# fixstars/cuda-bundle-adjustment

Hardware: AMD Instinct MI355X
Metric: edges/sec (edge-iterations/s = E x LM iterations / wall, graph resident in HBM, every timed 10-iteration run from its own perturbed start) + 10-iter LM wall-clock (contract_wall: initialize()+optimize(10) after warm-up, C++ API) on KITTI-00-shaped graph; per-iter chi2 vs g2o-faithful oracle (higher is better)
Workload: dtype f64

## Files before the change

cuda-bundle-adjustment_amd/capi.py:

```python
from __future__ import annotations

import atexit
import ctypes as C
import os
import subprocess
import weakref

import numpy as np

_HERE = os.path.dirname(os.path.abspath(__file__))
CSRC = os.path.join(_HERE, "csrc")
LIB_PATH = os.path.join(CSRC, "libcuba_hip.so")
LIB_PATH_F32 = os.path.join(CSRC, "libcuba_hip_f32.so")
HEADER = os.path.join(os.path.dirname(_HERE), "include", "cuba_hip.h")

_dp = C.POINTER(C.c_double)
_ip = C.POINTER(C.c_int32)
_u8p = C.POINTER(C.c_uint8)

ARRAY_IDS = dict(bp=0, bsc=1, xp=2, xl=3, lm_sys=4, hsc=5, state=6)
PROFILE_KEYS = (
    "0: Initialize Optimizer", "1: Build Structure", "2: Compute Error", "3: Build System",
    "4: Schur Complement", "5: Symbolic Decomposition", "6: Numerical Decomposition", "7: Update Solution")


class CubaHipError(RuntimeError):
    pass


def build_library(force=False):
    srcs = [os.path.join(CSRC, f) for f in os.listdir(CSRC) if f.endswith((".hip", ".hpp"))] + [HEADER]
    stale = not os.path.exists(LIB_PATH) or any(os.path.getmtime(s) > os.path.getmtime(LIB_PATH) for s in srcs)
    if force or stale or not os.path.exists(LIB_PATH_F32):
        subprocess.check_call(["make", "-C", CSRC, "-s", "all"])
    return LIB_PATH


_libs = {}


def load_library(precision="f64"):
    path = {"f64": LIB_PATH, "f32": LIB_PATH_F32}[precision]
    path = os.environ.get("CUBA_HIP_LIB_" + precision.upper(), path)
    if path in _libs:
        return _libs[path]
    if not os.path.exists(path):
        raise CubaHipError(f"{path} is missing: run __graft_entry__.build() (hipcc --offload-arch=gfx950)")
    if os.environ.get("CUBA_HIP_NO_TORCH") != "1":
        try:
            import torch
        except Exception:
            pass
    lib = C.CDLL(path)
    H = C.c_void_p
    sig = {
        "cuba_hip_create": [C.c_int, C.POINTER(H)],
        "cuba_hip_destroy": [H],
        "cuba_hip_set_stream": [H, C.c_void_p],
        "cuba_hip_set_option": [H, C.c_char_p, C.c_double],
        "cuba_hip_set_graph": [H, C.c_int, C.c_int, C.c_int, C.c_int, _dp, _dp, _dp, _dp, C.c_int, _ip, _ip, _u8p, _dp, _dp],
        "cuba_hip_set_graph_begin": [H, C.c_int, C.c_int, C.c_int, C.c_int, _dp, _dp, _dp, _dp, C.c_int, _ip, _ip, _u8p, _dp, _dp],
        "cuba_hip_set_graph_end": [H],
        "cuba_hip_set_graph_partition": [H, C.c_int, C.c_int, C.c_int, C.c_int, _dp, _dp, _dp, _dp, C.c_int, _ip, _ip, _u8p, _dp, _dp, C.c_int, C.c_int],
        "cuba_hip_set_robust_kernel": [H, C.c_int, C.c_int, C.c_double],
        "cuba_hip_build_structure": [H],
        "cuba_hip_compute_errors": [H, _dp],
        "cuba_hip_build_system": [H],
        "cuba_hip_max_diagonal": [H, _dp],
        "cuba_hip_set_lambda": [H, C.c_double],
        "cuba_hip_restore_diagonal": [H],
        "cuba_hip_schur": [H],
        "cuba_hip_schur_parts": [H, C.POINTER(C.c_int)],
        "cuba_hip_schur_part": [H, C.c_int, C.POINTER(C.c_size_t)],
# ... 721 lines not shown
```

cuda-bundle-adjustment_amd/csrc/ba_kernels.hpp:

```cpp
#pragma once

#include <hip/hip_runtime.h>
#include <cstdint>
#include <vector>

#include "ba_math.hpp"

namespace cubahip
{

constexpr int PCG_SETUP_POSES = 64;
constexpr int NSLOT = 16;
constexpr int WAVE = 64;
constexpr int LIN_BLOCK = 256;
constexpr int STEREO_BIT = 0x40000000;

struct DeviceGraph
{
	int Pt = 0, Pf = 0, Lt = 0, Lf = 0, E = 0;
	int e_begin = 0, e_end = 0;
	Scalar *q = nullptr, *t = nullptr, *cam = nullptr, *Xw = nullptr;
	int *e_pose = nullptr, *e_lm = nullptr;
	Scalar *e_mu = nullptr, *e_mv = nullptr, *e_mr = nullptr, *e_w = nullptr;
	int* lm_ptr = nullptr;
	RobustKernel rk[2] = { { 0, 0 }, { 0, 0 } };
};

constexpr int BP_HEAVY = 64;

struct DeviceStructure
{
	int nWaves = 0;
	int* wave_lm = nullptr;
	int nBig = 0;
	int* big_lm = nullptr;
	int nblk = 0;
	int *hsc_rowptr = nullptr, *hsc_colind = nullptr;
	int *adj_ptr = nullptr, *adj_blk = nullptr, *adj_col = nullptr;
	int2* ell = nullptr;
	int ell_m = 0, ell_over = 0;
	int* hsc_blkrow = nullptr;
	int nOd = 0;
	int nDiagProd = 0;
	int* od_blocks = nullptr;
	int inv_rows8 = 1;
	int nHeavy = 0;
	int *prod_ea = nullptr, *prod_eb = nullptr;
	const int *prod_beg = nullptr, *prod_end = nullptr, *pe_beg = nullptr, *pe_end = nullptr;
	int* prod_lm = nullptr;
	int* pe_edge = nullptr;
	int nCb = 0;
	int *cb_I = nullptr, *cb_J = nullptr, *cb_ptr = nullptr, *cb_blk = nullptr;
	Scalar *cb_wi = nullptr, *cb_wj = nullptr;
	Scalar* e_rec = nullptr;
	int mixed = 0;
};

int spmv_rows_for(int Pf);

struct DeviceSystem
{
	Scalar* hsc = nullptr;
	Scalar* bsc = nullptr;
	Scalar* bp = nullptr;
	Scalar* lm_sys = nullptr;
	Scalar* lm_inv = nullptr;
	Scalar* xp = nullptr;
	Scalar* xl = nullptr;
	Scalar* parts = nullptr;
	Scalar* slots = nullptr;
	unsigned long long* maxdiag = nullptr;
	int* fail = nullptr;
	Scalar *minv = nullptr, *r = nullptr, *z = nullptr, *p0 = nullptr, *p1 = nullptr, *ap = nullptr;
	Scalar *rz = nullptr, *pq = nullptr;
	int rzStride = 0, pqStride = 0;
	int nrz0 = 0, nrz = 0, npq = 0;
	int* done = nullptr;
	int* iters = nullptr;
	int* host_flags = nullptr;
	int* ticket = nullptr;
	int* kbase = nullptr;
	int agg = 0;
	int nc = 0;
	Scalar inv_agg = 0;
	int cl = 1;
	Scalar* acinv = nullptr;
	float* acinv32 = nullptr;
	Scalar* gj_pivots = nullptr;
	Scalar* rc = nullptr;
	Scalar* hrow = nullptr;
	int spmv_rows = 2;
	Scalar* qpart = nullptr;
	Scalar* r2 = nullptr;
// ... 28 lines not shown
	int nActive = 0;
	int nBlocks = 0;
	int nPoses = 0;
	const int *pose_i = nullptr, *pose_j = nullptr;
	const int* blk_ptr = nullptr;
	const int* blk_id = nullptr;
	const int* blk_shared = nullptr;
	const int* pose_ptr = nullptr;
	const int* pose_id = nullptr;
	const int* pose_item = nullptr;
	const Scalar* info = nullptr;
	Scalar* rec = nullptr;
	Scalar* chi = nullptr;
	const int* rk_kind = nullptr;
	const Scalar* rk_delta = nullptr;
};
constexpr int REL_REC = 90;
struct DeviceRelPoses : DevicePosePairs { const Scalar *q = nullptr, *t = nullptr; };
constexpr int PRNG_REC = 14;
struct DevicePoseRanges : DevicePosePairs
{
	const Scalar *arm_i = nullptr, *arm_j = nullptr;
	const Scalar* range = nullptr;
};

struct DeviceLandmarkPriors
{
	int n = 0;
	const int* lm_ptr = nullptr;
	const int* lm = nullptr;
	const Scalar* xbar = nullptr;
	const Scalar* info = nullptr;
	const int* rk_kind = nullptr;
	const Scalar* rk_delta = nullptr;
	Scalar* chi = nullptr;
};

enum { FACTOR_PRIORS = 0, FACTOR_REL, FACTOR_LMP, FACTOR_POS, FACTOR_DIR, FACTOR_RNG, FACTOR_PRNG, FACTOR_KINDS };
struct DeviceFactors
{
	DevicePriors priors; DeviceRelPoses rel; DeviceLandmarkPriors lmp; DevicePositionFactors pos; DeviceDirectionFactors dir; DeviceRangeFactors rng;
	DevicePoseRanges prng;
	template <class F> void each(F&& f) const { f(priors); f(rel); f(lmp); f(pos); f(dir); f(rng); f(prng); }
};
void launch_pose_factor_linearize(const DeviceGraph& g, const DeviceStructure& st, const DeviceSystem& sys, const DeviceFactors& pf, int mode, hipStream_t s);
void launch_factor_chi2(const DeviceGraph& g, const DeviceFactors& pf, Scalar* parts, hipStream_t s, int only = -1);
int factor_chi2_parts(const DeviceFactors* pf);

void launch_residual_chi2(const DeviceGraph& g, Scalar* parts, Scalar* slots, Scalar* per_edge, hipStream_t st, const DeviceFactors* pf = nullptr);

struct BlockPassRange { int begin, end, heavy; };
void launch_linearize_dm(const DeviceGraph& g, const DeviceStructure& st, const DeviceSystem& sys, int mode, Scalar lambda, hipStream_t s,
	Scalar* backupSrc = nullptr, Scalar* backupDst = nullptr, size_t backupCount = 0, const BlockPassRange* range = nullptr, const double* restoreFlag = nullptr,
	const DeviceLandmarkPriors* lp = nullptr);
void launch_block_pass(const DeviceGraph& g, const DeviceStructure& st, const DeviceSystem& sys, const BlockPassRange& range, hipStream_t s);

void launch_pose_maxdiag(const DeviceGraph& g, const DeviceStructure& st, const DeviceSystem& sys, hipStream_t s);

void launch_back_substitute(const DeviceGraph& g, const DeviceStructure& st, const DeviceSystem& sys, Scalar lambda, hipStream_t s);

void launch_pose_scale(const DeviceGraph& g, const DeviceSystem& sys, Scalar lambda, Scalar* slots, hipStream_t s);
struct LmDevice;
void launch_trial_tail_fused(const DeviceGraph& g, const DeviceStructure& st, const DeviceSystem& sys, Scalar lambda, const Scalar* old, hipStream_t s,
	const LmDevice* decide = nullptr, const DeviceFactors* pf = nullptr, int publish = 1);
size_t trial_tail_parts(const DeviceGraph& g, const DeviceStructure& st, int factorParts = 0);
constexpr int LM_REC = 8, LM_RING = 64;
struct LmDevice { double* state = nullptr; Scalar* lam = nullptr; double* ring = nullptr; };
void launch_lm_run_init(const Scalar* chiSlots, const unsigned long long* maxdiag, const LmDevice& lm, double tau, double tagBase, int maxq, hipStream_t s);
void launch_lm_decide_failed(const DeviceSystem& sys, const LmDevice& lm, hipStream_t s);
void launch_reduce_report(const DeviceSystem& sys, const Scalar* pA, int nA, Scalar* oA, const Scalar* pB, int nB, Scalar* oB, const Scalar* pC, int nC, Scalar* oC,
	const LmDevice* decide, int publish, hipStream_t s);
void launch_restore_if_rejected(Scalar* state, const Scalar* backup, size_t count, const LmDevice& lm, hipStream_t s);
void launch_landmark_scale(const DeviceGraph& g, const DeviceSystem& sys, Scalar lambda, Scalar* slots, hipStream_t s);

void launch_update_state(const DeviceGraph& g, const DeviceSystem& sys, hipStream_t s);

void launch_pcg_setup(const DeviceGraph& g, const DeviceStructure& st, const DeviceSystem& sys, Scalar lambda, hipStream_t s);
void launch_pcg_spmv(const DeviceGraph& g, const DeviceStructure& st, const DeviceSystem& sys, int k, int maxIter, Scalar tol2, hipStream_t s);
void launch_pcg_update(const DeviceGraph& g, const DeviceStructure& st, const DeviceSystem& sys, int k, int maxIter, Scalar tol2, hipStream_t s);
Scalar* launch_coarse_setup(const DeviceGraph& g, const DeviceStructure& st, const DeviceSystem& sys, Scalar* work0, Scalar* work1, hipStream_t s, hipEvent_t assembled = nullptr);
Scalar* launch_dense_inverse(Scalar* work0, Scalar* work1, int n, Scalar* pivots, hipStream_t s);
void launch_coarse_finish(const Scalar* swept, Scalar* dst, int n, hipStream_t s);
struct GjJob { Scalar* buf[2]; Scalar* piv[2]; int n, tiles; };
void launch_coarse_assemble(const DeviceGraph& g, const DeviceStructure& st, const DeviceSystem& sys, Scalar* work0, hipStream_t s);
void launch_dense_inverse_batch(const GjJob* jobs, int m, int nMax, hipStream_t s);
void launch_pcg2_fused(const DeviceGraph& g, const DeviceSystem& sys, int k, int kOut, int maxIter, Scalar tol2, int doUpdate, hipStream_t s);
int spmv_upper_grid(int Pf);
int pcg_rows_max_aggregate();
int pcg_rows_entries_per_thread(const DeviceSystem& sys);
void launch_build_lowpos(const DeviceGraph& g, const DeviceStructure& st, int* lowpos, hipStream_t s);
void launch_pcg_upper_iteration(const DeviceGraph& g, const DeviceStructure& st, const DeviceSystem& sys, int k, int maxIter, Scalar tol2, hipStream_t s, int which = 7);
void launch_pcg_advance(const DeviceSystem& sys, int n, hipStream_t s, Scalar tol2 = Scalar(-1));
void launch_coarse_to_fp32(const Scalar* swept, float* dst, int n, hipStream_t s);
void launch_pcg_iteration(const DeviceGraph& g, const DeviceStructure& st, const DeviceSystem& sys, int k, int maxIter, Scalar tol2, hipStream_t s);

struct LmDevice;
struct BatchTrial
{
	unsigned lmGroups = 0, lmGrid = 0; const Scalar* backupSrc = nullptr; Scalar* backupDst = nullptr; size_t backupCount = 0;
	int poseGroups = 0; unsigned schurGrid = 0;
	int nSetup = 0; size_t expandTotal = 0; unsigned nExpand = 0; const Scalar* copySrc = nullptr; Scalar* copyDst = nullptr; size_t copyPairs = 0; unsigned setupGrid = 0;
	int fusedOn = 0;
	const Scalar* old = nullptr; Scalar *scParts = nullptr, *chiParts = nullptr, *scaleParts = nullptr; int nLm = 0, poseBlocks = 0, nScale = 0; unsigned tailGrid = 0; int nA = 0;
	double* lmState = nullptr; Scalar* lmLam = nullptr; double* lmRing = nullptr; int reportOn = 0;
	Scalar* state = nullptr; size_t stateCount = 0; unsigned restoreGrid = 0;
};
struct BatchEntry
{
	DeviceGraph g; DeviceStructure st; DeviceSystem sys;
	int maxIter = 0;
	int gridSpmv = 0;
	BatchTrial t;
};
void batch_fill_linearize(const DeviceGraph& g, const DeviceStructure& st, const Scalar* backupSrc, Scalar* backupDst, size_t backupCount, BatchTrial& t);
void launch_batch_linearize(const BatchEntry* tab, int n, unsigned lmGridMax, unsigned schurGridMax, bool mixed, hipStream_t s);
void batch_fill_setup(const DeviceGraph& g, const DeviceStructure& st, const DeviceSystem& sys, const Scalar* copySrc, Scalar* copyDst, size_t copyCount, BatchTrial& t);
void launch_batch_setup(const BatchEntry* tab, int n, unsigned gridMax, hipStream_t s);
void launch_batch_first_precond(const BatchEntry* tab, int n, const DeviceSystem& sys0, int ncMax, size_t ldsMax, Scalar tol2, hipStream_t s);
void batch_fill_tail(const DeviceGraph& g, const DeviceStructure& st, const DeviceSystem& sys, const Scalar* old, const LmDevice& lm, Scalar* state, size_t stateCount, BatchTrial& t);
void launch_batch_tail(const BatchEntry* tab, int n, unsigned tailGridMax, unsigned restoreGridMax, hipStream_t s);
int batch_kernel_class(const DeviceGraph& g, const DeviceSystem& sys);
size_t batch_pcg2_lds_bytes(const DeviceSystem& sys);
void launch_pcg_batch_iteration(const BatchEntry* tab, int n, const DeviceGraph& g0, const DeviceSystem& sys0, int gridSpmvMax, int ncMax, size_t ldsMax, int k, Scalar tol2, hipStream_t s);
void launch_pcg_batch_advance(const BatchEntry* tab, int n, int iters, hipStream_t s, Scalar tol2);

hipError_t graph_add_pcg_chunk(hipGraph_t graph, const DeviceGraph& g, const DeviceStructure& st, const DeviceSystem& sys, int chunk, int maxIter, Scalar tol2, int report);

void launch_hsc_expand(const DeviceGraph& g, const DeviceStructure& st, const DeviceSystem& sys, hipStream_t s);
void launch_pcg_setup_expand(const DeviceGraph& g, const DeviceStructure& st, const DeviceSystem& sys, Scalar lambda, hipStream_t s,
	const Scalar* copySrc = nullptr, Scalar* copyDst = nullptr, size_t copyCount = 0);

constexpr int SC_T = 32;
constexpr int SC_TP = 5;
constexpr int SC_TT = SC_T * SC_T;

struct SparseCholPlan
{
	int Pf = 0, T = 0, nTiles = 0, nLevels = 0, slack = 0;
	std::vector<int> posOfSeg, segOfPos;
	std::vector<int> colPtr;
	std::vector<int> rowIdx, colOfTile;
	std::vector<int> gPtr;
	std::vector<int> gather;
	std::vector<int> wgRec;
	std::vector<int> lvlPtr, lvlTiles;
	std::vector<int> lvlColPtr, lvlCols;
	std::vector<int> blkTile;
	long long entries = 0;
	size_t tileBytes() const { return sizeof(Scalar) * (size_t)SC_TT * ((size_t)2 * nTiles + 1); }
	double secondsEstimate() const;
};
bool sparse_chol_plan(int Pf, const int* rowptr, const int* colind, int slack, size_t maxTiles, SparseCholPlan& out);

struct SparseChol
{
	Scalar* tiles = nullptr;
	Scalar* tilesT = nullptr;
	Scalar* y = nullptr;
	Scalar* rinv = nullptr;
	const int *colPtr = nullptr, *rowIdx = nullptr, *colOfTile = nullptr, *gPtr = nullptr, *gather = nullptr;
	const int *wgRec = nullptr, *lvlCols = nullptr, *blkTile = nullptr, *posOfSeg = nullptr;
	int* fail = nullptr;
	int T = 0, Pf = 0, nTiles = 0;
};
void launch_sparse_chol_fill(const DeviceStructure& st, const DeviceSystem& sys, const SparseChol& d, hipStream_t s);
void launch_sparse_chol_solve(const SparseChol& d, const SparseCholPlan& plan, Scalar* x, hipStream_t s);
void launch_sparse_chol_factor(const SparseChol& d, const SparseCholPlan& plan, hipStream_t s);

struct SelInvPlan
{
	int nLevels = 0;
	std::vector<int> stepPtr;
	std::vector<int> offRec;
	std::vector<int> colStepPtr, cols;
	std::vector<int> gather;
	long long products = 0;
	size_t sigmaBytes() const;
	int nTiles = 0;
};
bool selinv_plan(const SparseCholPlan& p, SelInvPlan& out);

struct SelInv
// ... 70 lines not shown
```

cuda-bundle-adjustment_amd/csrc/ba_linearize.hip:

```cpp

#include "ba_device.hpp"

namespace cubahip
{

constexpr int REC = 8;

__device__ __forceinline__ double tag_encode(int tag, double) { return __longlong_as_double((long long)tag); }
__device__ __forceinline__ float tag_encode(int tag, float) { return __int_as_float(tag); }
__device__ __forceinline__ int tag_decode(double v) { return (int)__double_as_longlong(v); }
__device__ __forceinline__ int tag_decode(float v) { return __float_as_int(v); }
__device__ __forceinline__ bool sign_flag(double v) { return __double_as_longlong(v) < 0; }
__device__ __forceinline__ bool sign_flag(float v) { return __float_as_int(v) < 0; }
__device__ __forceinline__ double abs_value(double v) { return __builtin_fabs(v); }
__device__ __forceinline__ float abs_value(float v) { return __builtin_fabsf(v); }

template <typename ET>
__device__ __forceinline__ void write_record(Scalar* base, size_t e, const Scalar Xc[3], Scalar wr, const Scalar r[3], int il, bool stereo)
{
	ET* rec = reinterpret_cast<ET*>(base) + REC * e;
	const ET w = (ET)wr;
	rec[0] = (ET)Xc[0]; rec[1] = (ET)Xc[1]; rec[2] = (ET)Xc[2]; rec[3] = stereo ? -w : w;
	rec[4] = (ET)r[0]; rec[5] = (ET)r[1]; rec[6] = (ET)r[2];
	rec[7] = tag_encode(il, ET());
// ... 342 lines not shown
template <int MODE, typename ET>
__global__ __launch_bounds__(256) void pose_pass_kernel(DeviceGraph g, DeviceStructure st, DeviceSystem sys)
{
	pose_pass_body<MODE, ET>(g, st, sys, blockIdx.x);
}

template <typename ET>
struct ProductOperand { ET X[3]; ET M[3][3]; };

template <typename ET>
__device__ __forceinline__ void product_operand(const ET* rec, const Rot3T<ET>& R, const ET cam[5], ProductOperand<ET>& o)
{
	CameraFrameEdge<ET> c;
	camera_frame_edge<ET>(rec, cam, c);
	o.X[0] = c.X[0]; o.X[1] = c.X[1]; o.X[2] = c.X[2];
	camera_frame_m<ET>(c, R, o.M);
}

template <typename ET>
__device__ __forceinline__ void product_accumulate(const ProductOperand<ET>& A, const ProductOperand<ET>& B, const ET inv[6], ET (&T)[6][6])
{
	ET P[3][3], W[3][6];
#pragma unroll
	for (int i = 0; i < 3; i++)
#pragma unroll
		for (int k = 0; k < 3; k++)
			P[i][k] = A.M[i][0] * inv[sym3_idx(0, k)] + A.M[i][1] * inv[sym3_idx(1, k)] + A.M[i][2] * inv[sym3_idx(2, k)];
#pragma unroll
	for (int i = 0; i < 3; i++)
	{
#pragma unroll
		for (int j = 0; j < 3; j++) W[i][3 + j] = P[i][0] * B.M[j][0] + P[i][1] * B.M[j][1] + P[i][2] * B.M[j][2];
		W[i][0] = B.X[1] * W[i][5] - B.X[2] * W[i][4];
		W[i][1] = B.X[2] * W[i][3] - B.X[0] * W[i][5];
		W[i][2] = B.X[0] * W[i][4] - B.X[1] * W[i][3];
	}
#pragma unroll
	for (int c = 0; c < 6; c++)
	{
		T[0][c] += A.X[1] * W[2][c] - A.X[2] * W[1][c];
		T[1][c] += A.X[2] * W[0][c] - A.X[0] * W[2][c];
		T[2][c] += A.X[0] * W[1][c] - A.X[1] * W[0][c];
		T[3][c] += W[0][c]; T[4][c] += W[1][c]; T[5][c] += W[2][c];
	}
}

template <typename ET, int GROUP>
__device__ __forceinline__ void block_pass_group(const DeviceGraph& g, const DeviceStructure& st, const DeviceSystem& sys, int grp, int gl)
{
	const int blk0 = grp >= 0 ? st.od_blocks[grp] : -1;
	const bool on = blk0 >= 0;
	const int blk = on ? blk0 : 0;
	const int a = on ? st.hsc_blkrow[blk] : 0, b = on ? st.hsc_colind[blk] : 0;
	ET qa[4], cama[5], qb[4], camb[5];
	load_pose_as<ET>(g, a, qa, cama);
	load_pose_as<ET>(g, b, qb, camb);
	const Rot3T<ET> Ra = quat_to_rot(qa[0], qa[1], qa[2], qa[3]);
	const Rot3T<ET> Rb = quat_to_rot(qb[0], qb[1], qb[2], qb[3]);
	ET T[6][6];
#pragma unroll
	for (int r = 0; r < 6; r++)
#pragma unroll
		for (int c = 0; c < 6; c++) T[r][c] = 0;
	const ET* recs = reinterpret_cast<const ET*>(st.e_rec);
	const int p1 = on ? st.prod_end[blk] : 0;
	for (int p = (on ? st.prod_beg[blk] : 0) + gl; p < p1; p += GROUP)
	{
		const ET* ra = recs + REC * (size_t)st.prod_ea[p];
		const ET* rb = recs + REC * (size_t)st.prod_eb[p];
		const Scalar* li = st.inv_rows8 ? sys.lm_inv + 8 * (size_t)st.prod_lm[p] : sys.lm_sys + 9 * (size_t)st.prod_lm[p];
		ET inv[6];
#pragma unroll
		for (int k = 0; k < 6; k++) inv[k] = (ET)li[k];
		ProductOperand<ET> A, B;
		product_operand<ET>(ra, Ra, cama, A);
		product_operand<ET>(rb, Rb, camb, B);
		product_accumulate<ET>(A, B, inv, T);
	}
	Scalar Ts[6][6];
#pragma unroll
	for (int r = 0; r < 6; r++)
#pragma unroll
		for (int c = 0; c < 6; c++)
		{
			Scalar v = (Scalar)T[r][c];
			if (GROUP == 64) v = wave_sum(v);
			else { v += __shfl_xor(v, 1); v += __shfl_xor(v, 2); v += __shfl_xor(v, 4); v += __shfl_xor(v, 8); }
			Ts[r][c] = v;
		}
	if (!on) return;
	Scalar* dst = sys.hsc + 36 * (size_t)blk;
	if (a != b)
	{
#pragma unroll
		for (int c = 0; c < 6; c++)
#pragma unroll
			for (int r = 0; r < 6; r++)
				if (GROUP == 64 ? (c * 6 + r) == gl : (c * 6 + r) % GROUP == gl) dst[c * 6 + r] = -Ts[r][c];
	}
	else if (gl == 0)
	{
#pragma unroll
		for (int c = 0; c < 6; c++)
#pragma unroll
			for (int r = 0; r <= c; r++) dst[c * 6 + r] -= Ts[r][c] + Ts[c][r];
	}
}

__host__ __device__ __forceinline__ int block_pass_heavy_groups(int nHeavy) { return (nHeavy + 3) / 4; }
__host__ __device__ __forceinline__ int block_pass_groups(int nOd, int nHeavy) { return block_pass_heavy_groups(nHeavy) + ((nOd - nHeavy) * BP_GROUP + 255) / 256; }

template <typename ET>
__device__ __forceinline__ void block_pass_body(const DeviceGraph& g, const DeviceStructure& st, const DeviceSystem& sys, int bid)
{
	const int nh = block_pass_heavy_groups(st.nHeavy);
	if (bid < nh)
	{
		const int grp = bid * 4 + (threadIdx.x >> 6);
		block_pass_group<ET, 64>(g, st, sys, grp < st.nHeavy ? grp : -1, threadIdx.x & 63);
	}
	else
	{
		const int grp = st.nHeavy + ((bid - nh) * 256 + threadIdx.x) / BP_GROUP;
		block_pass_group<ET, BP_GROUP>(g, st, sys, grp < st.nOd ? grp : -1, threadIdx.x & (BP_GROUP - 1));
	}
}

template <typename ET>
__global__ __launch_bounds__(256) void block_pass_kernel(DeviceGraph g, DeviceStructure st, DeviceSystem sys)
{
	block_pass_body<ET>(g, st, sys, blockIdx.x);
}

template <typename ET>
__global__ __launch_bounds__(256) void schur_pass_kernel(DeviceGraph g, DeviceStructure st, DeviceSystem sys, int nPoseGroups)
{
	if ((int)blockIdx.x < nPoseGroups) pose_pass_body<1, ET>(g, st, sys, blockIdx.x);
	else block_pass_body<ET>(g, st, sys, blockIdx.x - nPoseGroups);
}

template <typename ET>
__global__ __launch_bounds__(256) void schur_pass_batch_kernel(const BatchEntry* __restrict__ tab)
{
	const BatchEntry& e = tab[blockIdx.y];
	if (blockIdx.x >= e.t.schurGrid) return;
	if ((int)blockIdx.x < e.t.poseGroups) pose_pass_body<1, ET>(e.g, e.st, e.sys, blockIdx.x);
	else block_pass_body<ET>(e.g, e.st, e.sys, blockIdx.x - e.t.poseGroups);
}

static DeviceStructure block_pass_view(const DeviceStructure& st, const BlockPassRange& r)
{
	DeviceStructure v = st;
	v.od_blocks = st.od_blocks + r.begin; v.nOd = r.end - r.begin; v.nHeavy = r.heavy;
	return v;
}

struct LandmarkGrid
{
	unsigned groups, nCopy;
	LandmarkGrid(const DeviceStructure& st, const Scalar* backupSrc, size_t backupCount)
		: groups((st.nWaves + (LIN_BLOCK / WAVE) - 1) / (LIN_BLOCK / WAVE)),
		nCopy(backupSrc ? (unsigned)std::min<size_t>(512, (backupCount + LIN_BLOCK - 1) / LIN_BLOCK) : 0) {}
	unsigned grid() const { return groups + nCopy; }
};

template <typename ET>
static void launch_linearize_dm_t(const DeviceGraph& g, const DeviceStructure& stAll, const DeviceSystem& sys, int mode, Scalar lambda, hipStream_t s,
	Scalar* backupSrc, Scalar* backupDst, size_t backupCount, const BlockPassRange* range, const double* restoreFlag, const DeviceLandmarkPriors* lp)
{
	const DeviceStructure st = range ? block_pass_view(stAll, *range) : stAll;
	if (st.nWaves > 0)
	{
		const LandmarkGrid L(st, backupSrc, backupCount);
		const double* flag = L.nCopy ? restoreFlag : nullptr;
		if (lp)
			hipLaunchKernelGGL((mode == 0 ? lm_pass_prior_kernel<0, ET> : lm_pass_prior_kernel<1, ET>), dim3(L.grid()), dim3(LIN_BLOCK), 0, s,
				g, st, sys, lambda, L.groups, backupSrc, backupDst, backupCount, flag, *lp);
		else
			hipLaunchKernelGGL((mode == 0 ? lm_pass_kernel<0, ET> : lm_pass_kernel<1, ET>), dim3(L.grid()), dim3(LIN_BLOCK), 0, s,
				g, st, sys, lambda, L.groups, backupSrc, backupDst, backupCount, flag);
	}
	else if (backupSrc && backupCount)
		(void)hipMemcpyAsync(backupDst, backupSrc, backupCount * sizeof(Scalar), hipMemcpyDeviceToDevice, s);
	if (st.nBig > 0)
	{
		const auto big = lp ? (mode == 0 ? big_lm_pass_kernel<0, ET, true> : big_lm_pass_kernel<1, ET, true>)
			: (mode == 0 ? big_lm_pass_kernel<0, ET, false> : big_lm_pass_kernel<1, ET, false>);
		hipLaunchKernelGGL(big, dim3(st.nBig), dim3(256), 0, s, g, st, sys, lambda, lp ? *lp : DeviceLandmarkPriors());
	}
	const int nbp = block_pass_groups(st.nOd, st.nHeavy);
	if (mode == 1 && g.Pf > 0 && st.nOd > 0 && st.nDiagProd == 0)
	{
		const int np = (g.Pf + 3) / 4;
		hipLaunchKernelGGL((schur_pass_kernel<ET>), dim3(np + nbp), dim3(256), 0, s, g, st, sys, np);
		return;
	}
	if (g.Pf > 0)
	{
		if (mode == 0) hipLaunchKernelGGL((pose_pass_kernel<0, ET>), dim3((g.Pf + 3) / 4), dim3(256), 0, s, g, st, sys);
		else hipLaunchKernelGGL((pose_pass_kernel<1, ET>), dim3((g.Pf + 3) / 4), dim3(256), 0, s, g, st, sys);
	}
	if (mode == 1 && st.nOd > 0)
		hipLaunchKernelGGL((block_pass_kernel<ET>), dim3(nbp), dim3(256), 0, s, g, st, sys);
}

void launch_linearize_dm(const DeviceGraph& g, const DeviceStructure& st, const DeviceSystem& sys, int mode, Scalar lambda, hipStream_t s,
	Scalar* backupSrc, Scalar* backupDst, size_t backupCount, const BlockPassRange* range, const double* restoreFlag, const DeviceLandmarkPriors* lp)
{
	if (lp && lp->n == 0) lp = nullptr;
	if (st.mixed && sizeof(Scalar) == 8) launch_linearize_dm_t<float>(g, st, sys, mode, lambda, s, backupSrc, backupDst, backupCount, range, restoreFlag, lp);
	else launch_linearize_dm_t<Scalar>(g, st, sys, mode, lambda, s, backupSrc, backupDst, backupCount, range, restoreFlag, lp);
}

void batch_fill_linearize(const DeviceGraph& g, const DeviceStructure& st, const Scalar* backupSrc, Scalar* backupDst, size_t backupCount, BatchTrial& t)
{
	const LandmarkGrid L(st, backupSrc, backupCount);
	t.lmGroups = L.groups;
	t.lmGrid = L.grid();
	t.backupSrc = backupSrc; t.backupDst = backupDst; t.backupCount = backupCount;
	t.poseGroups = (g.Pf + 3) / 4;
	t.schurGrid = (unsigned)(t.poseGroups + block_pass_groups(st.nOd, st.nHeavy));
}

void launch_batch_linearize(const BatchEntry* tab, int n, unsigned lmGridMax, unsigned schurGridMax, bool mixed, hipStream_t s)
{
	if (mixed && sizeof(Scalar) == 8)
	{
		hipLaunchKernelGGL((lm_pass_batch_kernel<float>), dim3(lmGridMax, n), dim3(LIN_BLOCK), 0, s, tab);
		hipLaunchKernelGGL((schur_pass_batch_kernel<float>), dim3(schurGridMax, n), dim3(256), 0, s, tab);
	}
	else
	{
		hipLaunchKernelGGL((lm_pass_batch_kernel<Scalar>), dim3(lmGridMax, n), dim3(LIN_BLOCK), 0, s, tab);
		hipLaunchKernelGGL((schur_pass_batch_kernel<Scalar>), dim3(schurGridMax, n), dim3(256), 0, s, tab);
	}
}

void launch_block_pass(const DeviceGraph& g, const DeviceStructure& stAll, const DeviceSystem& sys, const BlockPassRange& range, hipStream_t s)
{
	if (range.end <= range.begin) return;
	const DeviceStructure st = block_pass_view(stAll, range);
	const int nbp = block_pass_groups(st.nOd, st.nHeavy);
	if (st.mixed && sizeof(Scalar) == 8) hipLaunchKernelGGL((block_pass_kernel<float>), dim3(nbp), dim3(256), 0, s, g, st, sys);
	else hipLaunchKernelGGL((block_pass_kernel<Scalar>), dim3(nbp), dim3(256), 0, s, g, st, sys);
}

__global__ __launch_bounds__(256) void pose_maxdiag_kernel(DeviceGraph g, DeviceStructure st, DeviceSystem sys)
{
	const int i = blockIdx.x * 256 + threadIdx.x;
	Scalar m = 0;
	if (i < g.Pf * 6)
	{
		const int p = i / 6, k = i % 6;
		m = sys.hsc[36 * (size_t)st.hsc_rowptr[p] + k * 7];
	}
	m = wave_max(m);
	if ((threadIdx.x & 63) == 0) atomic_max_nonneg(sys.maxdiag, m);
}

void launch_pose_maxdiag(const DeviceGraph& g, const DeviceStructure& st, const DeviceSystem& sys, hipStream_t s)
{
	if (g.Pf <= 0) return;
	hipLaunchKernelGGL(pose_maxdiag_kernel, dim3((g.Pf * 6 + 255) / 256), dim3(256), 0, s, g, st, sys);
}
// ... 3 lines not shown
```

cuda-bundle-adjustment_amd/csrc/ba_lm.hip:

```cpp
#include "ba_solver.hpp"

using namespace cubahip;

void cuba_hip_solver::graphWorker()
{
	(void)hipSetDevice(device);
	std::unique_lock<std::mutex> lk(gb.m);
	for (;;)
	{
		gb.cv.wait(lk, [&] { return gb.stop || !gb.jobs.empty() || !gb.trash.empty(); });
		if (gb.stop) return;
		if (gb.jobs.empty())
		{
			std::vector<hipGraphExec_t> t; t.swap(gb.trash);
			gb.busy = true;
			lk.unlock();
			for (hipGraphExec_t e : t) (void)hipGraphExecDestroy(e);
			lk.lock();
			gb.busy = false;
			gb.cv.notify_all();
			continue;
		}
		GraphJob j = gb.jobs.front(); gb.jobs.pop_front();
		gb.busy = true;
// ... 68 lines not shown
{
	volatile int* flags = (volatile int*)((char*)h_pinned + 1024);
	{
		const auto t0 = Clock::now();
		for (long spins = 0; flags[3] != expectedTicket; spins++)
			if ((spins & 0xfff) == 0xfff && std::chrono::duration<double>(Clock::now() - t0).count() > 2.0) break;
		if (flags[3] == expectedTicket)
		{
			std::atomic_thread_fence(std::memory_order_acquire);
			return;
		}
	}
	sync();
	std::atomic_thread_fence(std::memory_order_acquire);
	expectedTicket = flags[3];
}

void cuba_hip_solver::downloadAsDouble(const Scalar* dsrc, double* hdst, size_t n)
{
	if (!n) return;
	if (sizeof(Scalar) == sizeof(double))
	{
		HIP_TRY(hipMemcpyAsync(hdst, dsrc, n * sizeof(double), hipMemcpyDeviceToHost, stream));
		sync();
		return;
	}
	std::vector<Scalar> tmp(n);
	HIP_TRY(hipMemcpyAsync(tmp.data(), dsrc, n * sizeof(Scalar), hipMemcpyDeviceToHost, stream));
	sync();
	for (size_t i = 0; i < n; i++) hdst[i] = (double)tmp[i];
}

void cuba_hip_solver::uploadFromDouble(Scalar* ddst, const double* hsrc, size_t n)
{
	if (!n) return;
	std::vector<Scalar> tmp(hsrc, hsrc + n);
	HIP_TRY(hipMemcpyAsync(ddst, tmp.data(), n * sizeof(Scalar), hipMemcpyHostToDevice, stream));
	sync();
}

double cuba_hip_solver::computeErrors()
{
	need();
	StageTimer tm(this, 2);
	launch_residual_chi2(g, d_parts.data(), slotsDev, nullptr, stream, factors());
	return readSlots(0);
}

void cuba_hip_solver::linearize(int mode, double lam, bool withBackup)
{
	waitAssembled();
	const bool parts = mode == 1 && !redParts.empty();
	launch_linearize_dm(g, st, sys, mode, lam, stream, withBackup ? d_state.data() : nullptr, d_backup.data(), d_state.size(), parts ? &redParts[0].od : nullptr,
		withBackup ? lmRestoreFlag : nullptr, landmarkPriors());
	if (parts && !partsByCaller)
		for (size_t c = 1; c < redParts.size(); c++) launch_block_pass(g, st, sys, redParts[c].od, stream);
	if (factors()) launch_pose_factor_linearize(g, st, sys, pf, mode, stream);
}

void cuba_hip_solver::schurPart(int part, size_t ranges[4])
{
	need();
	if (part < 0 || part >= schurParts()) throw ArgError{ "cuba_hip_schur_part: no such part" };
	if (part == 0)
	{
		StageTimer tm(this, 4);
		zeroReduced();
		partsByCaller = true;
		try { linearize(1, lambda, false); } catch (...) { partsByCaller = false; throw; }
		partsByCaller = false;
	}
	else
	{
		StageTimer tm(this, 4);
		launch_block_pass(g, st, sys, redParts[part].od, stream);
	}
	const size_t nblk = (size_t)st.nblk;
	ranges[0] = redParts.empty() ? 0 : 36 * redParts[part].blkBegin;
	ranges[1] = redParts.empty() ? 36 * nblk : 36 * (redParts[part].blkEnd - redParts[part].blkBegin);
	ranges[2] = part == 0 ? 36 * nblk : 0;
	ranges[3] = part == 0 ? d_red.size() - 36 * nblk : 0;
}

void cuba_hip_solver::assemble()
{
	need();
	StageTimer tm(this, 3);
	zeroReduced(true);
	d_maxdiag.zero(stream);
	linearize(0, 0.0);
}

void cuba_hip_solver::maxDiagonalParts(double* posePart, double* lmPart)
{
	need();
	const double* hD = (const double*)hostStage();
	HIP_TRY(hipMemcpyAsync(hostStage(), d_maxdiag.data(), 8 * 64, hipMemcpyDeviceToHost, stream));
	sync();
	double v = 0;
	for (int i = 0; i < 64; i++) v = std::max(v, hD[i]);
	*lmPart = v;
	d_maxdiag.zero(stream);
	launch_pose_maxdiag(g, st, sys, stream);
	HIP_TRY(hipMemcpyAsync(hostStage(), d_maxdiag.data(), 8 * 64, hipMemcpyDeviceToHost, stream));
	sync();
	v = 0;
	for (int i = 0; i < 64; i++) v = std::max(v, hD[i]);
	*posePart = v;
}

void cuba_hip_solver::scaleParts(double lam, double* posePart, double* lmPart)
{
	need();
	launch_pose_scale(g, sys, lam, slotsDev + 3 * NSLOT, stream);
	launch_landmark_scale(g, sys, lam, slotsDev + 2 * NSLOT, stream);
	sync();
	double a = 0, b = 0;
	for (int i = 0; i < NSLOT; i++) { b += slot(2 * NSLOT + i); a += slot(3 * NSLOT + i); }
	*posePart = a; *lmPart = b;
}

double cuba_hip_solver::maxDiagonal()
{
	need();
	StageTimer tm(this, 3);
	zeroReduced(true);
	d_maxdiag.zero(stream);
	linearize(0, 0.0);
	launch_pose_maxdiag(g, st, sys, stream);
	HIP_TRY(hipMemcpyAsync(hostStage(), d_maxdiag.data(), 8 * 64, hipMemcpyDeviceToHost, stream));
	sync();
	double v = 0;
	for (int i = 0; i < 64; i++) v = std::max(v, ((const double*)hostStage())[i]);
	return v;
}

void cuba_hip_solver::schur(bool withBackup)
{
	need();
	StageTimer tm(this, 4);
	zeroReduced();
	linearize(1, lambda, withBackup);
}

bool cuba_hip_solver::solveReduced() { return retryWithFp64Inverse(solveReducedOnce()); }

bool cuba_hip_solver::retryWithFp64Inverse(bool ok)
{
	if (ok || !lastSolveBrokeDown || lastFailCode != 2 || !fp32Inverse() || sys.agg <= 0) return ok;
	precondFp32 = false; sys.acinv32 = nullptr;
	dropPcgGraph();
	coarseValid = false; firstInvValid = false; firstInvPending = false;
	cntFp32Fallbacks++;
	if (std::getenv("CUBA_HIP_DEBUG")) std::fprintf(stderr, "[cuba_hip] PCG broke down with the fp32-stored coarse inverse: repeating the solve with fp64 storage\n");
	const int64_t directBefore = cntDirect;
	const bool ok2 = solveReducedOnce();
	if (!ok2 || cntDirect != directBefore)
	{
		precondFp32 = true; sys.acinv32 = d_coarse32[0].data();
		dropPcgGraph();
		coarseValid = false; firstInvValid = false; firstInvPending = false;
	}
	return ok2;
}

int cuba_hip_solver::pcgBudget(int maxIter) const
{
	const int it = directAfter > 0 ? directAfter : std::min(384, std::max(128, Pf / 4));
	return std::min(maxIter, std::max(4, it / 4 * 4));
}

bool cuba_hip_solver::ensureDirectPlan()
{
	if (directPlanValid) return !directRefused;
	const auto t0 = Clock::now();
	ensureHostPattern();
	if (!sparse_chol_plan(Pf, h_rowptr.data(), h_colind.data(), directSlack, (size_t)std::max(1, directMaxTiles), directPlan))
	{
		directPlanValid = true; directRefused = true;
		char buf[200];
		std::snprintf(buf, sizeof buf, "exact reduced solve unavailable: the factor of the %d-pose reduced matrix needs more than direct_max_tiles = %d tiles", Pf, directMaxTiles);
		lastError = buf;
		return false;
	}
	const SparseCholPlan& p = directPlan;
	{
		size_t freeB = 0, totalB = 0;
		const size_t have = sizeof(Scalar) * (d_scTiles.size() + d_scTilesT.size());
		if (hipMemGetInfo(&freeB, &totalB) == hipSuccess && p.tileBytes() > have && p.tileBytes() - have > freeB)
		{
			directPlanValid = true; directRefused = true;
			char buf[200];
			std::snprintf(buf, sizeof buf, "exact reduced solve unavailable: the factor of the %d-pose reduced matrix needs %.1f MB, %.1f MB of device memory are free",
				Pf, p.tileBytes() / 1e6, freeB / 1e6);
// ... 3 lines not shown
		(void)hipGetLastError();
	}
	std::vector<int> ints;
	auto put = [&](const std::vector<int>& v) { const size_t o = ints.size(); ints.insert(ints.end(), v.begin(), v.end()); while (ints.size() % 4) ints.push_back(0); return o; };
	const size_t oColPtr = put(p.colPtr), oRowIdx = put(p.rowIdx), oColOf = put(p.colOfTile), oGPtr = put(p.gPtr), oGather = put(p.gather),
		oWgRec = put(p.wgRec), oLvlCols = put(p.lvlCols), oBlkTile = put(p.blkTile), oPos = put(p.posOfSeg);
	d_scInts.upload(ints, stream);
	d_scTiles.resize((size_t)SC_TT * ((size_t)p.nTiles + 1)); d_scTilesT.resize((size_t)SC_TT * std::max(1, p.nTiles));
	d_scY.resize((size_t)SC_T * p.T); d_scRinv.resize((size_t)SC_T * p.T); d_scFail.resize(1);
	sync();
	SparseChol& d = directDev;
	d.tiles = d_scTiles.data(); d.tilesT = d_scTilesT.data(); d.y = d_scY.data(); d.rinv = d_scRinv.data(); d.fail = d_scFail.data();
	const int* base = d_scInts.data();
	d.colPtr = base + oColPtr; d.rowIdx = base + oRowIdx; d.colOfTile = base + oColOf; d.gPtr = base + oGPtr; d.gather = base + oGather;
	d.wgRec = base + oWgRec; d.lvlCols = base + oLvlCols; d.blkTile = base + oBlkTile; d.posOfSeg = base + oPos;
	d.T = p.T; d.Pf = Pf; d.nTiles = p.nTiles;
	directPlanValid = true;
	directPlanBuilds++;
	directPlanSeconds = std::chrono::duration<double>(Clock::now() - t0).count();
	if (std::getenv("CUBA_HIP_DEBUG"))
		std::fprintf(stderr, "[cuba_hip] exact reduced solve, symbolic phase: %d poses -> %d tile columns, %d tiles (%.1f MB), %d levels, %lld tile products, slack %d, %.2f ms\n",
			Pf, p.T, p.nTiles, p.tileBytes() / 1e6, p.nLevels, p.entries, p.slack, 1e3 * directPlanSeconds);
	return true;
}

bool cuba_hip_solver::solveDirect()
{
	if (!ensureDirectPlan()) return false;
	const auto t0 = Clock::now();
	launch_sparse_chol_fill(st, sys, directDev, stream);
	launch_sparse_chol_solve(directDev, directPlan, sys.xp, stream);
	int* hflag = (int*)hostStage();
	HIP_TRY(hipMemcpyAsync(hflag, directDev.fail, sizeof(int), hipMemcpyDeviceToHost, stream));
	sync();
	directSeconds = std::chrono::duration<double>(Clock::now() - t0).count();
	cntDirect++;
	directSticky = true;
	coarseValid = false;
	if (std::getenv("CUBA_HIP_DEBUG"))
		std::fprintf(stderr, "[cuba_hip] exact reduced solve: %d unknowns, %.3f ms, lambda %.3e%s\n", 6 * Pf, 1e3 * directSeconds, lambda, *hflag ? " -- NON-POSITIVE PIVOT" : "");
	if (*hflag)
	{
		cntDirectFailed++;
		lastError = "exact reduced solve: non-positive pivot (the damped reduced matrix is not positive definite)";
		return false;
	}
	return true;
}

bool cuba_hip_solver::solveBegin(SolveCtx& sc)
{
	lastSolveBrokeDown = false;
	need();
	if (Pf == 0) { sc.result = true; return true; }
	const int maxIter = sc.maxIter = maxIterAlloc;
	const Scalar tol2 = sc.tol2 = pcgTol * pcgTol;
	if (failDirty) { d_fail.zero(stream); failDirty = false; }
	const bool twoLevel = sc.twoLevel = sys.agg > 0;
	const bool direct = sc.direct = directUsable();
	if (direct && (directSticky || directAlways))
	{
		launch_pcg_setup(g, st, sys, lambda, stream);
		failDirty = true;
		coarseValid = false;
		notePcgHistory(0);
		sc.result = solveDirect();
		return true;
	}
	sc.budget = direct && !acceptUnconverged ? pcgBudget(maxIter) : maxIter;
	const size_t invCount = (size_t)36 * sys.cl * sys.cl * sys.nc * sys.nc;
	bool takeInverse = false;
	if (twoLevel && coarseValid && pendingInv >= 0)
	{
		HIP_TRY(hipStreamWaitEvent(stream, evInverse, 0));
		takeInverse = true; pendingInv = -1;
	}
	const bool deferred = sc.deferLaunch && twoLevel && coarseValid;
	{
		const bool f32 = fp32Inverse();
		const Scalar* cpSrc = !takeInverse ? nullptr : f32 ? reinterpret_cast<const Scalar*>(d_coarse32[1].data()) : d_coarse[0].data();
		Scalar* cpDst = f32 ? reinterpret_cast<Scalar*>(d_coarse32[0].data()) : d_coarse[2].data();
		const size_t cpCount = f32 ? inv32Count() / 2 : invCount;
		if (deferred) { sc.deferred = true; sc.copySrc = cpSrc; sc.copyDst = cpDst; sc.copyCount = cpCount; }
		else launch_pcg_setup_expand(g, st, sys, lambda, stream, cpSrc, cpDst, cpCount);
	}
	if (twoLevel)
	{
		const int gjSteps = (6 * sys.cl * sys.nc + 31) / 32, first = gjSteps & 1;
		{
			ensureOverlapObjects();
			const size_t invBytes = sizeof(Scalar) * (size_t)36 * sys.cl * sys.cl * sys.nc * sys.nc;
			if (!coarseValid && heuristics && firstInvValid)
			{
				HIP_TRY(hipStreamWaitEvent(stream, evFirstInv, 0));
				if (fp32Inverse()) HIP_TRY(hipMemcpyAsync(d_coarse32[0].data(), d_firstInv32.data(), inv32Count() * sizeof(float), hipMemcpyDeviceToDevice, stream));
				else HIP_TRY(hipMemcpyAsync(d_coarse[2].data(), d_firstInv.data(), invBytes, hipMemcpyDeviceToDevice, stream));
				pendingInv = -1;
				coarseValid = true; sideAge = overlapPeriod(); firstInvPending = true;
			}
			else if (!coarseValid)
			{
				drainInversion();
				(void)launch_coarse_setup(g, st, sys, d_coarse[first].data(), d_coarse[1 - first].data(), stream);
				if (fp32Inverse()) launch_coarse_to_fp32(d_coarse[0].data(), d_coarse32[0].data(), 6 * sys.cl * sys.nc, stream);
				else launch_coarse_finish(d_coarse[0].data(), d_coarse[2].data(), 6 * sys.cl * sys.nc, stream);
				coarseValid = true; cntCoarseRefresh++; cntCoarseInline++; sideAge = 0;
				if (heuristics)
				{
					if (fp32Inverse()) d_firstInv32.resize(inv32Count()); else d_firstInv.resize(invCount);
					sideAge = overlapPeriod(); firstInvPending = true;
				}
			}
			sys.acinv = d_coarse[2].data();
			const bool regular = ++sideAge >= overlapPeriod();
			if (regular) sideAge = 0;
			if (regular)
			{
				if (!deferred) HIP_TRY(hipEventRecord(evSetup, stream));
				if (sc.deferCoarse)
				{
					sc.deferCoarse->push_back(CoarseJob{ this, first, firstInvPending, !deferred });
					if (firstInvPending) { firstInvPending = false; firstInvValid = true; }
				}
				else if (sc.sideLater) sc.sideFirst = first;
				else enqueueCoarseSide(first);
				pendingInv = 0;
				assemblePending = true; cntCoarseRefresh++;
			}
		}
		if (!deferred) launch_pcg2_fused(g, sys, 0, 0, maxIter, tol2, 0, stream);
	}
	const bool graphs = sc.graphs = useGraph && !sc.batched && g_liveHandles.load(std::memory_order_relaxed) <= 1;
	if (useGraph && !graphs && (!pcgGraphs.empty() || graphsOrderedFor)) dropPcgGraph();
	if (graphs && pcgGraphs.empty() && graphsOrderedFor != (const void*)sys.acinv)
	{
		for (int c = 64; c >= 4; c /= 2) (void)pcgGraphIfReady(c, maxIter, tol2);
		graphsOrderedFor = (const void*)sys.acinv;
	}
	sc.hInts = (volatile int*)((char*)h_pinned + 1024);
	sc.tSolve0 = Clock::now();
	int predicted = 32;
	if (runIters.size() >= 2)
	{
		const double a = runIters[runIters.size() - 2], b = runIters.back();
		const double lin = b + std::max(0.0, b - a), geo = b * std::min(1.35, std::max(1.0, b / std::max(1.0, a)));
		predicted = (int)std::max(lin, geo) + 1;
	}
	else if (runIters.size() == 1) predicted = (int)(1.35 * runIters[0]) + 2;
	else if (firstSolveIters > 0) predicted = firstSolveIters + 1;
	{
		const size_t k = runIters.size();
		if (heuristics && k < prevRunIters.size() && std::equal(runIters.begin(), runIters.end(), prevRunIters.begin())) predicted = prevRunIters[k];
	}
	sc.predicted = predicted;
	return false;
}

void cuba_hip_solver::enqueueCoarseSide(int first)
{
	HIP_TRY(hipStreamWaitEvent(gjStream, evSetup, 0));
	(void)launch_coarse_setup(g, st, sys, d_coarse[first].data(), d_coarse[1 - first].data(), gjStream, evAssembled);
	enqueueInversionTail(gjStream, firstInvPending);
	if (firstInvPending) { firstInvPending = false; firstInvValid = true; }
}

void cuba_hip_solver::enqueueInversionTail(hipStream_t side, bool firstInvCopy)
{
	const int Nc = 6 * sys.cl * sys.nc;
	if (fp32Inverse()) launch_coarse_to_fp32(d_coarse[0].data(), d_coarse32[1].data(), Nc, side);
	else launch_coarse_finish(d_coarse[0].data(), d_coarse[0].data(), Nc, side);
	if (firstInvCopy)
	{
		if (fp32Inverse()) HIP_TRY(hipMemcpyAsync(d_firstInv32.data(), d_coarse32[1].data(), inv32Count() * sizeof(float), hipMemcpyDeviceToDevice, side));
		else HIP_TRY(hipMemcpyAsync(d_firstInv.data(), d_coarse[0].data(), sizeof(Scalar) * (size_t)Nc * Nc, hipMemcpyDeviceToDevice, side));
		HIP_TRY(hipEventRecord(evFirstInv, side));
	}
	HIP_TRY(hipEventRecord(evInverse, side));
}

bool cuba_hip_solver::solveBrokeDown(SolveCtx& sc)
{
	lastSolveBrokeDown = true; lastFailCode = sc.hInts[0];
	cntPcgIters += sc.hInts[1]; coarseValid = false; firstInvValid = false; firstInvPending = false; failDirty = true;
	if (sc.direct && lastFailCode != 1 && !(lastFailCode == 2 && fp32Inverse() && sc.twoLevel))
	{
		notePcgHistory(-sc.hInts[1]);
		d_fail.zero(stream); failDirty = false;
		return solveDirect();
	}
	return false;
}

static int pcgFirstTarget(int predicted) { return (predicted + 3) / 4 * 4; }
static int pcgNextTarget(int k0, int looks) { return k0 + ((looks == 0 && k0 <= 96) ? 4 : std::max(8, k0 / 8 / 4 * 4)); }
static int pcgBatchLength(int target, int budget, int k0) { return std::max(4, std::min(target, budget) - k0); }

bool cuba_hip_solver::solveReducedOnce()
{
	StageTimer tm(this, 6);
	SolveCtx sc;
	sc.sideLater = coarseSideLater;
	if (solveBegin(sc)) return sc.result;
	const int maxIter = sc.maxIter; const Scalar tol2 = sc.tol2; const bool graphs = sc.graphs; const int predicted = sc.predicted;
	bool converged = false;
	int k0 = 0, looks = 0, eagerIters = 0;
	int target = pcgFirstTarget(predicted);
	while (k0 < sc.budget && !converged)
	{
		int todo = pcgBatchLength(target, sc.budget, k0);
		while (todo > 0)
		{
			int c = graphs ? 256 : todo;
			for (; graphs && c > 4 && c > todo; c >>= 1) {}
			if (graphs && todo > c && todo % 4 == 0 && todo <= 128 && pcgGraphMaxIter == maxIter && pcgGraphTol2 == tol2)
			{
				if ((pcgGraphs.count(std::make_pair(todo, (const Scalar*)sys.acinv)) || ++batchRequests[todo] >= 2) && pcgGraphIfReady(todo, maxIter, tol2)) c = todo;
			}
			hipGraphExec_t exec = graphs ? pcgGraphIfReady(c, maxIter, tol2) : nullptr;
			if (exec) { HIP_TRY(hipGraphLaunch(exec, stream)); noteReport(); }
			else
			{
				for (int k = 0; k < c; k++) enqueuePcgIteration(k, maxIter, tol2, stream);
				launch_pcg_advance(sys, c, stream, tol2); noteReport();
				if (graphs) { eagerIters += c; cntPcgPlain += c; }
			}
			k0 += c; todo -= c;
			if (sc.sideFirst >= 0) { enqueueCoarseSide(sc.sideFirst); sc.sideFirst = -1; }
		}
		waitReport();
		if (sc.hInts[0] != 0) return solveBrokeDown(sc);
		if (sc.hInts[2] == 1 || sc.hInts[1] < std::min(k0, maxIter)) converged = true;
		target = pcgNextTarget(k0, looks);
		looks++; cntPcgLooks++; cntHostLooks++;
	}
	sc.converged = converged; sc.k0 = k0; sc.looks = looks; sc.eagerIters = eagerIters;
	return solveEnd(sc);
}

bool cuba_hip_solver::solveEnd(SolveCtx& sc)
{
	const int maxIter = sc.maxIter; const bool direct = sc.direct; const bool converged = sc.converged;
	const int k0 = sc.k0, looks = sc.looks, eagerIters = sc.eagerIters, predicted = sc.predicted;
	const auto tSolve1 = Clock::now();
	if (std::getenv("CUBA_HIP_DEBUG"))
	{
		std::vector<Scalar> part((size_t)std::max(1, sys.nrz0));
		HIP_TRY(hipMemcpyAsync(part.data(), sys.rz, sizeof(Scalar) * part.size(), hipMemcpyDeviceToHost, stream));
		sync();
		double rz0 = 0; for (Scalar v : part) rz0 += (double)v;
		std::fprintf(stderr, "[cuba_hip] PCG: %d iterations, %d enqueued (%d as plain launches), %d host looks (prediction %d), lambda %.3e, r0.z0 %.6e, solve %.3f ms, graphs built so far %lld\n",
			sc.hInts[1], k0, eagerIters, looks, predicted, lambda, rz0, 1e3 * std::chrono::duration<double>(tSolve1 - sc.tSolve0).count(), (long long)gb.builds.load());
	}
	const int itersDone = sc.itersDone >= 0 ? sc.itersDone : sc.hInts[1];
	cntPcgIters += itersDone; cntPcgEnqueued += k0;
	if (runIters.empty()) firstSolveIters = itersDone;
// ... 95 lines not shown
		if (!r.absorb(rec)) throw StateError{ "the device's decision record of an LM trial never arrived" };
	}
}

bool cuba_hip_solver::lmBeforeTrial(LmRun& r)
{
	if (r.stop) return false;
	if (r.enq > r.seen)
	{
		const bool safe = r.done + 1 < r.niter && r.rejRun + 1 < LmRun::maxq;
		if (!safe) { waitReport(); cntHostLooks++; lmAbsorb(r, r.enq); if (r.stop) return false; }
	}
	cntTrials++;
	lambda = -1.0;
	return true;
}

bool cuba_hip_solver::lmAfterSolveHost(LmRun& r)
{
	lmAbsorb(r, r.enq);
	if (r.stop) { cntTrials--; return false; }
	return true;
}

bool cuba_hip_solver::lmAfterSolve(LmRun& r, bool ok)
{
	if (!lmAfterSolveHost(r)) return false;
	const bool waited = !r.chain || !(r.done + 1 < r.niter && r.rejRun + 1 < LmRun::maxq);
	const bool publish = waited || !ok;
	if (ok) launch_trial_tail_fused(g, st, sys, (Scalar)-1, d_backup.data(), stream, &r.lm, factors(), publish ? 1 : 0);
	else launch_lm_decide_failed(sys, r.lm, stream);
	if (publish) noteReport();
	r.restoreInPass = !publish && st.nWaves > 0;
	if (!r.restoreInPass) launch_restore_if_rejected(d_state.data(), d_backup.data(), d_state.size(), r.lm, stream);
	r.enq++;
	(void)hipStreamQuery(stream);
	return true;
}

int cuba_hip_solver::lmRunEnd(LmRun& r)
{
	if (r.seen < r.enq) { waitReport(); cntHostLooks++; lmAbsorb(r, r.enq); }
	lambda = r.lam;
	return r.done;
}

int cuba_hip_solver::optimizeDeviceDecision(int niter, double* chi2Out)
{
	LmRun r;
	lmRunBegin(r, niter, chi2Out, true);
	while (lmBeforeTrial(r))
	{
		lmRestoreFlag = r.restoreInPass ? r.lm.state + 5 : nullptr;
		try { schur(true); } catch (...) { lmRestoreFlag = nullptr; throw; }
		lmRestoreFlag = nullptr;
		coarseSideLater = true;
		bool ok = false;
		try { ok = solveReduced(); } catch (...) { coarseSideLater = false; throw; }
		coarseSideLater = false;
		if (!lmAfterSolve(r, ok)) break;
	}
	return lmRunEnd(r);
}

bool cuba_hip_solver::fullyBatchable() const
{
	return batchable() && st.nBig == 0 && st.nDiagProd == 0 && st.nOd > 0 && st.nWaves > 0 && redParts.empty() && !factors();
}

bool cuba_hip_solver::batchable() const
{
	return !profile && partHi < 0 && Pf > 0 && Lf > 0 && E > 0 && trial_tail_parts(g, st, factorParts()) <= d_parts.size() && batch_kernel_class(g, sys) >= 0;
}

void cuba_hip_solver::launchCoarseJobs(std::vector<CoarseJob>& jobs, hipEvent_t common)
{
	if (jobs.empty()) return;
	ensureOverlapObjects();
	hipStream_t side = gjStream;
	const int m = (int)jobs.size();
	if (!h_gjTab) { HIP_TRY(hipHostMalloc((void**)&h_gjTab, sizeof(GjJob) * CUBA_HIP_BATCH_MAX, hipHostMallocDefault)); HIP_TRY(hipEventCreateWithFlags(&evGjTab, hipEventDisableTiming)); HIP_TRY(hipEventRecord(evGjTab, side)); }
	d_gjTab.resize(sizeof(GjJob) * CUBA_HIP_BATCH_MAX);
	HIP_TRY(hipEventSynchronize(evGjTab));
	int nMax = 0;
	for (int a = 0; a < m; a++)
	{
		cuba_hip_solver* h = jobs[a].h;
		const int Nc = 6 * h->sys.cl * h->sys.nc;
		HIP_TRY(hipStreamWaitEvent(side, jobs[a].ownEvent || !common ? h->evSetup : common, 0));
		launch_coarse_assemble(h->g, h->st, h->sys, h->d_coarse[jobs[a].first].data(), side);
		GjJob& j = h_gjTab[a];
		j.buf[0] = h->d_coarse[jobs[a].first].data(); j.buf[1] = h->d_coarse[1 - jobs[a].first].data();
		j.piv[0] = h->sys.gj_pivots; j.piv[1] = h->sys.gj_pivots + 32 * 32;
		j.n = Nc; j.tiles = (Nc + 31) / 32;
		nMax = std::max(nMax, Nc);
	}
	for (int a = 0; a < m; a++) HIP_TRY(hipEventRecord(jobs[a].h->evAssembled, side));
	HIP_TRY(hipMemcpyAsync(d_gjTab.data(), h_gjTab, sizeof(GjJob) * m, hipMemcpyHostToDevice, side));
	HIP_TRY(hipEventRecord(evGjTab, side));
	launch_dense_inverse_batch(reinterpret_cast<const GjJob*>(d_gjTab.data()), m, nMax, side);
	for (int a = 0; a < m; a++) jobs[a].h->enqueueInversionTail(side, jobs[a].firstInvCopy);
	jobs.clear();
}

void cuba_hip_solver::ensureBatchTables()
{
	if (!h_batchTab) HIP_TRY(hipHostMalloc((void**)&h_batchTab, sizeof(BatchEntry) * CUBA_HIP_BATCH_MAX * 3, hipHostMallocDefault));
	d_batchTab.resize(sizeof(BatchEntry) * CUBA_HIP_BATCH_MAX * 3);
// ... 71 lines not shown
};
}

static int optimizeBatch(cuba_hip_solver** hs, int n, int niter, double* chi2, int* nDone, bool full)
{
	typedef cuba_hip_solver::SolveCtx SolveCtx;
	cuba_hip_solver* lead = hs[0];
	hipStream_t bs = lead->stream;
	struct StreamGuard
	{
		cuba_hip_solver** hs; int n; std::vector<hipStream_t> own;
		StreamGuard(cuba_hip_solver** h, int m, hipStream_t s) : hs(h), n(m), own((size_t)m)
		{
			for (int i = 0; i < n; i++) { own[i] = hs[i]->stream; (void)hipStreamSynchronize(own[i]); hs[i]->stream = s; }
		}
		~StreamGuard() { if (n > 0) (void)hipStreamSynchronize(hs[0]->stream); for (int i = 0; i < n; i++) hs[i]->stream = own[i]; }
	} streamGuard(hs, full ? n : 0, bs);
	std::vector<hipEvent_t>& evJoin = lead->batchEvents;
	while (!full && (int)evJoin.size() < n + 1) { hipEvent_t e; HIP_TRY(hipEventCreateWithFlags(&e, hipEventDisableTiming)); evJoin.push_back(e); }
	const hipEvent_t evFork = full ? nullptr : evJoin[n];
	lead->ensureBatchTables();
	lead->ensureOverlapObjects();
	BatchEntry* hTab[3]; const BatchEntry* dTab[3];
	for (int k = 0; k < 3; k++) { hTab[k] = lead->h_batchTab + (size_t)k * CUBA_HIP_BATCH_MAX; dTab[k] = reinterpret_cast<const BatchEntry*>(lead->d_batchTab.data()) + (size_t)k * CUBA_HIP_BATCH_MAX; }
	auto upload = [&](int k, int m) { HIP_TRY(hipMemcpyAsync(const_cast<BatchEntry*>(dTab[k]), hTab[k], sizeof(BatchEntry) * m, hipMemcpyHostToDevice, bs)); };
	const int pcgTab = full ? 1 : 0;
	std::vector<cuba_hip_solver::LmRun> runs((size_t)n);
	std::vector<SolveCtx> ctx((size_t)n);
	std::vector<cuba_hip_solver::CoarseJob> coarseJobs;
	for (int i = 0; i < n; i++) hs[i]->lmRunBegin(runs[i], niter, chi2 ? chi2 + (size_t)i * niter : nullptr);
	const bool mixed = lead->st.mixed != 0;
	const int cls0 = batch_kernel_class(lead->g, lead->sys);
	std::vector<int> act;
	std::vector<char> okv((size_t)n);
	int batchSolves = 0;
	for (;;)
	{
		act.clear();
		for (int i = 0; i < n; i++) if (hs[i]->lmBeforeTrial(runs[i])) act.push_back(i);
		if (act.empty()) break;
		const int m = (int)act.size();
		(full ? lead->cntBatchFullTrials : lead->cntBatchIterTrials)++;
		if (full)
		{
			unsigned lmMax = 0, schurMax = 0;
			for (int a = 0; a < m; a++)
			{
				cuba_hip_solver* h = hs[act[a]];
				h->zeroReduced();
				BatchEntry& e = hTab[0][a];
				e = BatchEntry();
				e.g = h->g; e.st = h->st; e.sys = h->sys;
				batch_fill_linearize(h->g, h->st, h->d_state.data(), h->d_backup.data(), h->d_state.size(), e.t);
				lmMax = std::max(lmMax, e.t.lmGrid); schurMax = std::max(schurMax, e.t.schurGrid);
			}
			upload(0, m);
			launch_batch_linearize(dTab[0], m, lmMax, schurMax, mixed, bs);
		}
		BatchPcg pcg(hs, ctx, bs);
		unsigned setupMax = 0; int nFused = 0;
		for (int a = 0; a < m; a++)
		{
			const int i = act[a];
			cuba_hip_solver* h = hs[i];
			if (!full) h->schur(true);
			ctx[i] = SolveCtx(); ctx[i].batched = true; ctx[i].deferCoarse = &coarseJobs; ctx[i].deferLaunch = full;
			const bool alone = batch_kernel_class(h->g, h->sys) != cls0;
			const bool finished = alone || h->solveBegin(ctx[i]);
			if (finished) okv[i] = alone ? h->solveReduced() : ctx[i].result;
			BatchEntry& e = hTab[pcgTab][full ? a : pcg.count()];
			if (!finished)
			{
				pcg.add(i, e);
				if (ctx[i].deferred) { batch_fill_setup(h->g, h->st, h->sys, ctx[i].copySrc, ctx[i].copyDst, ctx[i].copyCount, e.t); e.t.fusedOn = 1; nFused++; }
				setupMax = std::max(setupMax, e.t.setupGrid);
			}
			else if (full) { e = BatchEntry(); e.g = h->g; e.st = h->st; e.sys = h->sys; }
		}
		if (!full || pcg.count() == 0) lead->launchCoarseJobs(coarseJobs);
		if (pcg.count() > 0)
		{
			const int mTab = full ? m : pcg.count();
			if (full)
			{
				upload(1, m);
				if (nFused > 0) launch_batch_setup(dTab[1], m, setupMax, bs);
				HIP_TRY(hipEventRecord(lead->evSetup, bs));
				lead->launchCoarseJobs(coarseJobs, lead->evSetup);
				if (nFused > 0) launch_batch_first_precond(dTab[1], m, pcg.kh->sys, pcg.ncMax, pcg.ldsMax, pcg.tol2, bs);
			}
			else
			{
				for (int a = 0; a < mTab; a++)
				{
					cuba_hip_solver* h = hs[pcg.who[a]];
					if (h != lead) { HIP_TRY(hipEventRecord(evJoin[a], h->stream)); HIP_TRY(hipStreamWaitEvent(bs, evJoin[a], 0)); }
				}
				upload(0, mTab);
			}
			pcg.iterate(dTab[pcgTab], mTab);
			if (!full) HIP_TRY(hipEventRecord(evFork, bs));
			pcg.finish(okv, evFork);
			batchSolves++;
		}
		if (full)
		{
// ... 218 lines not shown
```

cuda-bundle-adjustment_amd/csrc/ba_pcg.hip:

```cpp

#include "ba_device.hpp"

namespace cubahip
{

template <bool ROWCOPY>
__device__ __forceinline__ void pcg_setup_body(const DeviceGraph& g, const DeviceStructure& st, const DeviceSystem& sys, Scalar lambda, int bid, int nb)
{
	const int i = threadIdx.x < PCG_SETUP_POSES ? bid * PCG_SETUP_POSES + (int)threadIdx.x : g.Pf;
	lambda = launch_lambda(sys, lambda);
	Scalar rz = 0;
	if (i < g.Pf)
	{
		Scalar* blk = sys.hsc + 36 * (size_t)st.hsc_rowptr[i];
		Scalar A[36], Ai[36];
#pragma unroll
		for (int c = 0; c < 6; c++)
#pragma unroll
			for (int r = 0; r <= c; r++)
			{
				Scalar v = blk[c * 6 + r];
				if (r == c) v += lambda;
				A[c * 6 + r] = v;
				A[r * 6 + c] = v;
			}
#pragma unroll
		for (int k = 0; k < 36; k++) blk[k] = A[k];
		if (ROWCOPY && !sys.upper)
		{
			const int pos = (st.adj_ptr[i + 1] - st.adj_ptr[i]) - (st.hsc_rowptr[i + 1] - st.hsc_rowptr[i]);
			if (pos < 20 * st.ell_m)
			{
				Scalar* dst = sys.hrow + 36 * ((size_t)i * st.ell_m * 20 + pos);
#pragma unroll
				for (int k = 0; k < 36; k++) dst[k] = A[k];
			}
		}
		if (!spd6_inverse(A, Ai)) *sys.fail = 1;
#pragma unroll
		for (int k = 0; k < 36; k++) sys.minv[36 * (size_t)i + k] = Ai[k];
		Scalar rr[6];
#pragma unroll
		for (int k = 0; k < 6; k++) rr[k] = sys.bsc[6 * (size_t)i + k];
#pragma unroll
		for (int r = 0; r < 6; r++)
		{
			Scalar z = 0;
#pragma unroll
			for (int c = 0; c < 6; c++) z += Ai[c * 6 + r] * rr[c];
			sys.r[6 * (size_t)i + r] = rr[r];
			sys.z[6 * (size_t)i + r] = z;
			sys.xp[6 * (size_t)i + r] = 0;
			sys.p0[6 * (size_t)i + r] = 0;
			sys.p1[6 * (size_t)i + r] = 0;
			rz += rr[r] * z;
		}
	}
	rz = wave_sum(rz);
	if (sys.agg == 0)
	{
		if (threadIdx.x == 0)
		{
			const Scalar s2 = rz;
			sys.rz[bid] = s2;
			sys.rz[sys.rzStride + bid] = s2;
		}
		for (int t = nb + bid * 256 + threadIdx.x; t < sys.nrz; t += nb * 256) sys.rz[sys.rzStride + t] = 0;
	}
	if (bid == 0 && threadIdx.x == 0) { *sys.iters = 0; *sys.done = 0; *sys.kbase = 0; }
}

__global__ __launch_bounds__(256) void pcg_setup_kernel(DeviceGraph g, DeviceStructure st, DeviceSystem sys, Scalar lambda)
{
	pcg_setup_body<false>(g, st, sys, lambda, blockIdx.x, gridDim.x);
}

void launch_pcg_setup(const DeviceGraph& g, const DeviceStructure& st, const DeviceSystem& sys, Scalar lambda, hipStream_t s)
{
	if (g.Pf > 0) hipLaunchKernelGGL(pcg_setup_kernel, dim3((g.Pf + PCG_SETUP_POSES - 1) / PCG_SETUP_POSES), dim3(256), 0, s, g, st, sys, lambda);
}

__device__ __forceinline__ void pcg_raise_done(const DeviceSystem& sys, bool atLimit, Scalar rzk)
{
	if (*sys.done == 0) *sys.done = atLimit ? 2 : 1;
	if (!(rzk == rzk)) *sys.fail = 3;
}

__device__ __forceinline__ bool pcg_active(const DeviceSystem& sys, int k, int maxIter, Scalar tol2, int lane, Scalar& rzk)
{
	if (*sys.done) return false;
	rzk = wave_sum(load_parts(rz_slot(sys, k), rz_count(sys, k), lane));
	const Scalar rz0 = wave_sum(load_parts(sys.rz, sys.nrz0, lane));
	const bool on = k < maxIter && *sys.fail == 0 && rzk > tol2 * rz0 && rzk == rzk;
	if (!on && blockIdx.x == 0 && threadIdx.x == 0) pcg_raise_done(sys, k >= maxIter, rzk);
	return on;
}

__device__ __forceinline__ void spmv_entry(const DeviceStructure& st, const DeviceSystem& sys, const Scalar* pold, int a, int rr,
	Scalar& accz, Scalar& accp)
{
	const int bi = st.adj_blk[a];
	const int j = st.adj_col[a];
	const Scalar* B = sys.hsc + 36 * (size_t)(bi & 0x7fffffff);
	const int sr = bi < 0 ? 6 : 1, sc = bi < 0 ? 1 : 6;
	Scalar av[6], zv[6], pv[6];
#pragma unroll
	for (int c = 0; c < 6; c++)
	{
		av[c] = B[rr * sr + c * sc];
		zv[c] = sys.z[6 * (size_t)j + c];
		pv[c] = pold[6 * (size_t)j + c];
	}
#pragma unroll
	for (int c = 0; c < 6; c++) { accz += av[c] * zv[c]; accp += av[c] * pv[c]; }
}

typedef Scalar Scalar2 __attribute__((ext_vector_type(2)));

template <bool FUSED>
__device__ __forceinline__ void hsc_expand_body(const DeviceStructure& st, const DeviceSystem& sys, size_t total, size_t bid)
{
	const size_t t = bid * 256 + threadIdx.x;
	if (t >= total) return;
	const size_t slot = t / 36;
	const int e = (int)(t - 36 * slot);
	const int2 en = st.ell[slot];
	if (en.y < 0) return;
	const int rr = e / 6, c = e - 6 * rr;
	const Scalar* B = sys.hsc + 36 * (size_t)(en.x & 0x7fffffff);
	if (FUSED && en.y == (int)(slot / ((size_t)st.ell_m * 20))) return;
	sys.hrow[t] = B[en.x < 0 ? rr * 6 + c : c * 6 + rr];
}

__global__ __launch_bounds__(256) void hsc_expand_kernel(DeviceStructure st, DeviceSystem sys, size_t total)
{
	hsc_expand_body<false>(st, sys, total, blockIdx.x);
}

__global__ __launch_bounds__(256) void pcg_setup_expand_kernel(DeviceGraph g, DeviceStructure st, DeviceSystem sys, Scalar lambda, int nSetup, size_t total,
	unsigned nExpand, const Scalar2* __restrict__ copySrc, Scalar2* __restrict__ copyDst, size_t copyPairs)
{
	if ((int)blockIdx.x < nSetup) pcg_setup_body<true>(g, st, sys, lambda, blockIdx.x, nSetup);
	else if (blockIdx.x < nSetup + nExpand) hsc_expand_body<true>(st, sys, total, blockIdx.x - nSetup);
	else
	{
		const size_t stride = (size_t)(gridDim.x - nSetup - nExpand) * 256;
		for (size_t i = (size_t)(blockIdx.x - nSetup - nExpand) * 256 + threadIdx.x; i < copyPairs; i += stride) copyDst[i] = copySrc[i];
	}
}

__global__ __launch_bounds__(256) void pcg_setup_expand_batch_kernel(const BatchEntry* __restrict__ tab)
{
	const BatchEntry& e = tab[blockIdx.y];
	const BatchTrial& t = e.t;
	if (blockIdx.x >= t.setupGrid) return;
	if ((int)blockIdx.x < t.nSetup) pcg_setup_body<true>(e.g, e.st, e.sys, Scalar(-1), blockIdx.x, t.nSetup);
	else if (blockIdx.x < t.nSetup + t.nExpand) hsc_expand_body<true>(e.st, e.sys, t.expandTotal, blockIdx.x - t.nSetup);
	else
	{
		const Scalar2* __restrict__ src = reinterpret_cast<const Scalar2*>(t.copySrc);
		Scalar2* __restrict__ dst = reinterpret_cast<Scalar2*>(t.copyDst);
		const size_t stride = (size_t)(t.setupGrid - t.nSetup - t.nExpand) * 256;
		for (size_t i = (size_t)(blockIdx.x - t.nSetup - t.nExpand) * 256 + threadIdx.x; i < t.copyPairs; i += stride) dst[i] = src[i];
	}
}

void launch_hsc_expand(const DeviceGraph& g, const DeviceStructure& st, const DeviceSystem& sys, hipStream_t s)
{
	const size_t total = (size_t)g.Pf * st.ell_m * 20 * 36;
	if (total) hipLaunchKernelGGL(hsc_expand_kernel, dim3((unsigned)((total + 255) / 256)), dim3(256), 0, s, st, sys, total);
}

void launch_pcg_setup_expand(const DeviceGraph& g, const DeviceStructure& st, const DeviceSystem& sys, Scalar lambda, hipStream_t s,
	const Scalar* copySrc, Scalar* copyDst, size_t copyCount)
{
	if (g.Pf <= 0) return;
	const size_t total = sys.upper ? 0 : (size_t)g.Pf * st.ell_m * 20 * 36;
	const int nSetup = (g.Pf + PCG_SETUP_POSES - 1) / PCG_SETUP_POSES;
	const unsigned nExpand = (unsigned)((total + 255) / 256);
	const size_t pairs = copySrc ? copyCount / 2 : 0;
	const unsigned nCopy = pairs ? (unsigned)std::min<size_t>(1024, (pairs + 255) / 256) : 0;
	hipLaunchKernelGGL(pcg_setup_expand_kernel, dim3(nSetup + nExpand + nCopy), dim3(256), 0, s, g, st, sys, lambda, nSetup, total, nExpand,
		reinterpret_cast<const Scalar2*>(copySrc), reinterpret_cast<Scalar2*>(copyDst), pairs);
}

void batch_fill_setup(const DeviceGraph& g, const DeviceStructure& st, const DeviceSystem& sys, const Scalar* copySrc, Scalar* copyDst, size_t copyCount, BatchTrial& t)
{
	t.expandTotal = sys.upper ? 0 : (size_t)g.Pf * st.ell_m * 20 * 36;
	t.nSetup = (g.Pf + PCG_SETUP_POSES - 1) / PCG_SETUP_POSES;
	t.nExpand = (unsigned)((t.expandTotal + 255) / 256);
	t.copyPairs = copySrc ? copyCount / 2 : 0;
	const unsigned nCopy = t.copyPairs ? (unsigned)std::min<size_t>(1024, (t.copyPairs + 255) / 256) : 0;
	t.copySrc = copySrc; t.copyDst = copyDst;
	t.setupGrid = t.nSetup + t.nExpand + nCopy;
}

void launch_batch_setup(const BatchEntry* tab, int n, unsigned gridMax, hipStream_t s)
{
	if (gridMax) hipLaunchKernelGGL(pcg_setup_expand_batch_kernel, dim3(gridMax, n), dim3(256), 0, s, tab);
}

template <int N>
__device__ __forceinline__ void spmv_batch(const DeviceSystem& sys, const Scalar* pold, const int2 (&e)[3], const Scalar* Arow, int rr, Scalar& accz, Scalar& accp)
{
	Scalar2 av[N][3], zv[N][3], pv[N][3];
#pragma unroll
	for (int n = 0; n < N; n++)
	{
		const size_t j = e[n].y >= 0 ? e[n].y : 0;
		const Scalar2* A2 = reinterpret_cast<const Scalar2*>(Arow + (size_t)n * (20 * 36) + 6 * rr);
		const Scalar2* z2 = reinterpret_cast<const Scalar2*>(sys.z + 6 * j);
		const Scalar2* p2 = reinterpret_cast<const Scalar2*>(pold + 6 * j);
		const bool on = e[n].y >= 0;
#pragma unroll
		for (int c = 0; c < 3; c++) { av[n][c] = on ? A2[c] : Scalar2{ 0, 0 }; zv[n][c] = z2[c]; pv[n][c] = p2[c]; }
	}
#pragma unroll
	for (int n = 0; n < N; n++)
	{
#pragma unroll
		for (int c = 0; c < 3; c++)
		{
			const Scalar a0 = av[n][c].x, a1 = av[n][c].y;
			accz += a0 * zv[n][c].x; accp += a0 * pv[n][c].x;
			accz += a1 * zv[n][c].y; accp += a1 * pv[n][c].y;
		}
	}
}

template <int ROWS>
// ... 555 lines not shown
		Scalar s2 = 0;
#pragma unroll
		for (int w = 0; w < PCG2_T / 64; w++) s2 += wsum[24 + w];
		rz_slot_w(sys, kOut)[blockIdx.x] = s2;
		if (!doUpdate) sys.rz[blockIdx.x] = s2;
		if (doUpdate && blockIdx.x == 0) *sys.iters = kabs + 1;
	}
	TRACE_MARK();
	if (doUpdate) TRACE_FLUSH(1, blockIdx.x * (PCG2_T / 64) + wv);
}

template <int CL, int AC, int AC2, int W, bool PRE = false>
__global__ __launch_bounds__(PCG2_T) void pcg2_fused_kernel(DeviceGraph g, DeviceSystem sys, int k, int kOut, int maxIter, Scalar tol2, int doUpdate)
{
	pcg2_fused_body<CL, AC, AC2, W, PRE>(g, sys, k, kOut, maxIter, tol2, doUpdate);
}

template <int CL, int AC, int AC2, int W>
__global__ __launch_bounds__(PCG2_T) void pcg2_fused_batch_kernel(const BatchEntry* __restrict__ tab, int k, int kOut, Scalar tol2, int doUpdate)
{
	const BatchEntry& e = tab[blockIdx.y];
	if ((int)blockIdx.x >= e.sys.nc || e.gridSpmv == 0 || (doUpdate == 0 && e.t.fusedOn == 0)) return;
	pcg2_fused_body<CL, AC, AC2, W, false>(e.g, e.sys, k, kOut, e.maxIter, tol2, doUpdate);
}

template <bool PRE>
static void* pcg2_kernel_sel(const DeviceSystem& sys)
{
	const int Nc = 6 * sys.cl * sys.nc;
	if (sys.acinv32 && sizeof(Scalar) == 8)
	{
		if (sys.cl == 2) return Nc <= 768 ? (void*)pcg2_fused_kernel<2, 3, 0, 4, PRE> : Nc <= 1536 ? (void*)pcg2_fused_kernel<2, 6, 0, 4, PRE> : (void*)pcg2_fused_kernel<2, 6, 3, 4, PRE>;
		return Nc <= 768 ? (void*)pcg2_fused_kernel<1, 3, 0, 4, PRE> : Nc <= 1536 ? (void*)pcg2_fused_kernel<1, 6, 0, 4, PRE> : (void*)pcg2_fused_kernel<1, 6, 3, 4, PRE>;
	}
	const bool small = Nc <= 768;
	if (sys.cl == 2) return small ? (void*)pcg2_fused_kernel<2, 6, 0, 2, PRE> : (void*)pcg2_fused_kernel<2, 12, 6, 2, PRE>;
	return small ? (void*)pcg2_fused_kernel<1, 6, 0, 2, PRE> : (void*)pcg2_fused_kernel<1, 12, 6, 2, PRE>;
}
static void* pcg2_kernel_for(const DeviceSystem& sys, bool precondOnly = false) { return precondOnly ? pcg2_kernel_sel<true>(sys) : pcg2_kernel_sel<false>(sys); }

static size_t pcg2_lds_bytes(const DeviceSystem& sys)
{
	const size_t cd = 6 * (size_t)sys.cl;
	const size_t ncp = (cd * sys.nc + 3) & ~(size_t)3;
	return sizeof(Scalar) * (2 * ncp + 8 * cd + cd + 32 + 12 * (size_t)sys.agg);
}

void launch_pcg2_fused(const DeviceGraph& g, const DeviceSystem& sys, int k, int kOut, int maxIter, Scalar tol2, int doUpdate, hipStream_t s)
{
	const size_t lds = pcg2_lds_bytes(sys);
	hipLaunchKernelGGL((void (*)(DeviceGraph, DeviceSystem, int, int, int, Scalar, int))pcg2_kernel_for(sys), dim3(sys.nc), dim3(PCG2_T), lds, s, g, sys, k, kOut, maxIter, tol2, doUpdate);
}

__device__ __forceinline__ Scalar half_wave_sum(Scalar v, bool upperHalf)
{
	v += dpp_shift<0x111, 0xf>(v);
	v += dpp_shift<0x112, 0xf>(v);
	v += dpp_shift<0x114, 0xf>(v);
	v += dpp_shift<0x118, 0xf>(v);
	v += dpp_shift<0x142, 0xa>(v);
	union { Scalar s; int w[sizeof(Scalar) / 4]; } u, lo, hi;
	u.s = v;
#pragma unroll
	for (int i = 0; i < (int)(sizeof(Scalar) / 4); i++) { lo.w[i] = __builtin_amdgcn_readlane(u.w[i], 31); hi.w[i] = __builtin_amdgcn_readlane(u.w[i], 63); }
	return upperHalf ? hi.s : lo.s;
}

template <int NS>
__device__ __forceinline__ void upper_steps(const DeviceStructure& st, const DeviceSystem& sys, const Scalar* pold, int s0, int b0, int b1, int grp, int c,
	Scalar beta, const Scalar (&pi)[6], Scalar (&acc)[6], Scalar& dotT)
{
	int bb[NS], j[NS], lp[NS]; bool on[NS];
	Scalar2 v[NS][3]; Scalar zj[NS], pjo[NS];
#pragma unroll
	for (int s = 0; s < NS; s++)
	{
		const int b = s0 + 5 * s + grp;
		on[s] = grp < 5 && b < b1;
		bb[s] = on[s] ? b : b0;
	}
#pragma unroll
	for (int s = 0; s < NS; s++) { j[s] = st.hsc_colind[bb[s]]; lp[s] = sys.lowpos[bb[s]]; }
#pragma unroll
	for (int s = 0; s < NS; s++)
	{
		const Scalar2* B2 = reinterpret_cast<const Scalar2*>(sys.hsc + (36 * (size_t)bb[s] + 6 * c));
		v[s][0] = B2[0]; v[s][1] = B2[1]; v[s][2] = B2[2];
	}
#pragma unroll
	for (int s = 0; s < NS; s++) { zj[s] = sys.z[6 * (size_t)j[s] + c]; pjo[s] = pold[6 * (size_t)j[s] + c]; }
#pragma unroll
	for (int s = 0; s < NS; s++)
	{
		const Scalar pj = on[s] ? zj[s] + beta * pjo[s] : Scalar(0);
		const Scalar Bc[6] = { v[s][0].x, v[s][0].y, v[s][1].x, v[s][1].y, v[s][2].x, v[s][2].y };
		Scalar t = 0;
#pragma unroll
		for (int r = 0; r < 6; r++) { acc[r] += Bc[r] * pj; t += Bc[r] * pi[r]; }
		if (on[s] && bb[s] != b0)
		{
			sys.tq[6 * (size_t)lp[s] + c] = t;
			dotT += pj * t;
		}
	}
}

// ... 396 lines not shown
```

cuda-bundle-adjustment_amd/csrc/ba_setup.hip:

```cpp
#include "ba_solver.hpp"

using namespace cubahip;

void cuba_hip_solver::finishValues()
{
	if (!valuesPending) return;
	valuesPending = false;
	HIP_TRY(hipStreamWaitEvent(stream, evValues, 0));
	gatherSortedValues();
	valuesStamp++;
}

void cuba_hip_solver::gatherSortedValues()
{
	sizeSortedValues();
	topo::launch_gather_edges(d_perm.data(), d_rawEp.data(), d_rawEl.data(), d_rawDim.data(), d_rawMeas.data(), d_rawOmega.data(), E,
		nullptr, nullptr, d_mu.data(), d_mv.data(), d_mr.data(), d_w.data(), stream);
	sortedValuesValid = true;
}

UploadFacts cuba_hip_solver::uploadFacts() const
{
	static const bool noCache = std::getenv("CUBA_HIP_NO_STRUCTURE_CACHE") != nullptr;
	UploadFacts f{};
// ... 419 lines not shown
		int maxCnt = 0;
		for (int k = 0; k < nblk; k++) maxCnt = std::max(maxCnt, prodPtr[k + 1] - prodPtr[k]);
		std::vector<int> start(maxCnt + 2, 0);
		for (int k = 0; k < nblk; k++) { const int c = prodPtr[k + 1] - prodPtr[k]; if (c > 0) start[maxCnt - c + 1]++; }
		for (int c = 0; c <= maxCnt; c++) start[c + 1] += start[c];
		odBlocks.resize(start[maxCnt + 1]);
		for (int k = 0; k < nblk; k++) { const int c = prodPtr[k + 1] - prodPtr[k]; if (c > 0) odBlocks[start[maxCnt - c]++] = k; }
		if (rowGroupedBlocks(nprodLocal))
		{
			std::vector<int> cntOf(nblk);
			for (int k = 0; k < nblk; k++) cntOf[k] = prodPtr[k + 1] - prodPtr[k];
			odBlocks = rowGroupedOrder(blkRow.data(), h_colind.data(), cntOf.data(), nblk);
		}
	}
	lap("structure: product lists");
	std::vector<int> pePtr(Pf + 1, 0), peEdge;
	const bool wholeGraph = g.e_begin == 0 && g.e_end == E;
	if (!wholeGraph)
	{
		for (int i = g.e_begin; i < g.e_end; i++) if (h_epose[i] < Pf) pePtr[h_epose[i] + 1]++;
		for (int i = 0; i < Pf; i++) pePtr[i + 1] += pePtr[i];
		peEdge.resize(pePtr[Pf]);
		std::vector<int> cur(pePtr.begin(), pePtr.end() - 1);
		for (int i = g.e_begin; i < g.e_end; i++) if (h_epose[i] < Pf) peEdge[cur[h_epose[i]]++] = i;
	}
	lap("structure: pose edge lists");
	std::vector<int> waveLm, bigLm;
	{
		int start = -1, cnt = 0;
		auto flush = [&](int end) { if (start >= 0 && cnt > 0) { waveLm.push_back(start); waveLm.push_back(end); } start = -1; cnt = 0; };
		for (int l = lo; l < hi; l++)
		{
			if ((l - lo) % topo::WAVE_CHUNK == 0) flush(l);
			const int n = h_lmptr[l + 1] - h_lmptr[l];
			if (n > WAVE)
			{
				flush(l);
				bigLm.push_back(l);
				continue;
			}
			if (n == 0) continue;
			if (start >= 0 && cnt + n > WAVE) flush(l);
			if (start < 0) start = l;
			cnt += n;
		}
		flush(hi);
	}

	lap("structure: wave list");
	d_waveLm.upload(waveLm, stream); d_bigLm.upload(bigLm, stream);
	d_rowptr.upload(h_rowptr, stream); d_colind.upload(h_colind, stream);
	d_adjPtr.upload(adjPtr, stream); d_adjBlk.upload(adjBlk, stream); d_adjCol.upload(adjCol, stream);
	int ellM = 0, ellOver = 0;
	{
		int maxRow = 0;
		for (int i = 0; i < Pf; i++) maxRow = std::max(maxRow, adjPtr[i + 1] - adjPtr[i]);
		const int M = std::min(3, (maxRow + 19) / 20);
		ellM = M; ellOver = maxRow > 20 * M;
		std::vector<int2> ell((size_t)Pf * M * 20, int2{ 0, -1 });
		for (int i = 0; i < Pf; i++)
		{
			const int n = std::min(adjPtr[i + 1] - adjPtr[i], 20 * M);
			for (int e = 0; e < n; e++) ell[(size_t)i * M * 20 + e] = int2{ adjBlk[adjPtr[i] + e], adjCol[adjPtr[i] + e] };
		}
		d_ell.upload(ell, stream);
	}
	d_blkrow.upload(blkRow, stream); d_odBlocks.upload(odBlocks, stream); d_prodPtr.upload(prodPtr, stream);
	d_prodEa.upload(prodEa, stream); d_prodEb.upload(prodEb, stream); d_pePtr.upload(wholeGraph ? peAllPtr : pePtr, stream); d_peEdge.upload(wholeGraph ? peAll : peEdge, stream);
	const CoarseCfg cc = coarseConfig();
	allocSystem(nblk, cc);
	const int agg = cc.agg, cl = cc.cl, nc = cc.nc;
	lap("structure: uploads + allocs");
	std::vector<int> cbI, cbJ, cbPtr(1, 0), cbBlk, adjRow(adjBlk.size());
	std::vector<Scalar> cbWi, cbWj;
	auto weight = [&](int pose) {
		if (pose == Pf - 1 && Pf % agg == 1) return Scalar(0);
		return Scalar(2 * (pose % agg) + 1 - agg) / Scalar(agg);
	};
	for (int i = 0; i < Pf; i++) for (int a = adjPtr[i]; a < adjPtr[i + 1]; a++) adjRow[a] = i;
	if (nc > 0)
	{
		std::vector<uint64_t> ck; ck.reserve(adjBlk.size());
		for (int i = 0; i < Pf; i++)
			for (int a = adjPtr[i]; a < adjPtr[i + 1]; a++)
				ck.push_back(((uint64_t)((size_t)(i / agg) * nc + adjCol[a] / agg) << 32) | (uint32_t)a);
		std::sort(ck.begin(), ck.end());
		for (size_t x = 0; x < ck.size(); x++)
		{
			const int cbid = (int)(ck[x] >> 32);
			if (x == 0 || cbid != (int)(ck[x - 1] >> 32))
			{
				if (x) cbPtr.push_back((int)cbBlk.size());
				cbI.push_back(cbid / nc); cbJ.push_back(cbid % nc);
			}
			cbBlk.push_back(adjBlk[(uint32_t)ck[x]]);
			if (cl == 2) { cbWi.push_back(weight(adjRow[(uint32_t)ck[x]])); cbWj.push_back(weight(adjCol[(uint32_t)ck[x]])); }
		}
		cbPtr.push_back((int)cbBlk.size());
	}
	d_cbI.upload(cbI, stream); d_cbJ.upload(cbJ, stream); d_cbPtr.upload(cbPtr, stream); d_cbBlk.upload(cbBlk, stream); d_cbWi.upload(cbWi, stream); d_cbWj.upload(cbWj, stream);
	sync();
	lap("structure: coarse lists + sync");
	diagProdBlocks = 0; for (int k : odBlocks) diagProdBlocks += k >= 0 && blkRow[k] == h_colind[k];
	heavyBlocks = 0;
	if (!rowGroupedBlocks(nprodLocal))
		for (int k : odBlocks) heavyBlocks += prodPtr[k + 1] - prodPtr[k] > BP_HEAVY;
	publishStructure(nblk, (int)waveLm.size() / 2, (int)bigLm.size(), (int)odBlocks.size(), (int)cbI.size(), ellM, ellOver, cc);
	hostPatternValid = true;
	const double dt = std::chrono::duration<double>(Clock::now() - t0).count();
	prof[1] += 0.5 * dt; prof[5] += 0.5 * dt;
}

cuba_hip_solver::CoarseCfg cuba_hip_solver::coarseConfig() const
{
	int agg = pcgAggregate;
	const int cl = coarseLinear ? 2 : 1;
	const int ncMax = std::min(180, std::max(115, (Pf + 31) / 32));
	if (agg < 0) agg = cl == 2 ? (Pf >= 1320 ? std::max(16, (Pf + ncMax - 1) / ncMax) : std::max(6, (Pf + 27) / 55)) : std::max(12, (Pf + 159) / 160);
	const int spmvRows = spmv_rows_for(Pf);
	if (agg > 0) agg = (agg + spmvRows - 1) / spmvRows * spmvRows;
	int nc = agg > 0 ? (Pf + agg - 1) / agg : 0;
	int clOut = cl;
	const int aggMax = 600 / spmvRows * spmvRows;
	auto ncOf = [&](int a) { return (Pf + a - 1) / a; };
	auto fits = [&](int c, int a) { const int n = ncOf(a); return c * n <= 600 && sizeof(Scalar) * (12 * (size_t)c * n + 12 * (size_t)a + 200) <= 60 * 1024; };
	if (agg > aggMax) agg = aggMax;
	if (agg > 0)
	{
		bool ok = false;
		for (int c = cl; c >= 1 && !ok; c--)
		{
			int a = agg;
			while (a < aggMax && !fits(c, a)) a = std::min(aggMax, 2 * a);
			if (!fits(c, a))
			{
				int m = ((int)std::ceil(std::sqrt((double)c * Pf)) + spmvRows - 1) / spmvRows * spmvRows;
				m = std::min(aggMax, std::max(agg, m));
				if (fits(c, m)) a = m;
			}
			if (fits(c, a)) { agg = a; clOut = c; ok = true; }
		}
		if (!ok) agg = 0;
	}
	nc = agg > 0 ? ncOf(agg) : 0;
	if (nc < 2) { agg = 0; nc = 0; }
	return CoarseCfg{ agg, agg > 0 ? clOut : cl, nc, spmvRows };
}

void cuba_hip_solver::allocSystem(int nblk, const CoarseCfg& c)
{
	directRefused = false; directSticky = false; directPlanValid = false;
	d_red.resize((size_t)36 * nblk + (size_t)12 * Pf);
	d_lmSys.resize((size_t)9 * Lf); d_lmInv.resize((size_t)8 * std::max(Lf, 1)); d_erec.resize((size_t)8 * E); d_xp.resize((size_t)6 * Pf); d_xl.resize((size_t)3 * Lf);
	d_minv.resize((size_t)36 * Pf);
	d_r.resize((size_t)6 * Pf); d_z.resize((size_t)6 * Pf); d_p0.resize((size_t)6 * Pf); d_p1.resize((size_t)6 * Pf); d_ap.resize((size_t)6 * Pf);
	d_red.zero(stream); d_lmSys.zero(stream); d_lmInv.zero(stream); d_xp.zero(stream); d_xl.zero(stream);
	reducedZeroed = true;
	for (auto& b : d_coarse) b.resize((size_t)36 * c.cl * c.cl * c.nc * c.nc);
	{
		const size_t n = (size_t)6 * c.cl * c.nc;
		for (auto& b : d_coarse32) b.resize(fp32Inverse() ? n * ((n + 3) & ~(size_t)3) : 0);
	}
	d_rc.resize((size_t)12 * c.cl * c.nc); d_r2.resize((size_t)6 * Pf);
// ... 60 lines not shown
	std::stable_sort(byLen.begin(), byLen.end(), [](const std::pair<int, int>& x, const std::pair<int, int>& y) { return x.first < y.first; });
	std::vector<int> od(nChunks * 16, -1);
	for (size_t o = 0; o < nChunks; o++)
	{
		const size_t c = (size_t)byLen[o].second;
		if (c < nWhole) for (int x = 0; x < 16; x++) od[o * 16 + x] = val[chunkStart[c] + x];
		else
		{
			const size_t b = (size_t)chunkStart[c] - n, e = std::min(rest.size(), b + 16);
			for (size_t x = b; x < e; x++) od[o * 16 + (x - b)] = rest[x];
		}
	}
	return od;
}

void cuba_hip_solver::publishStructure(int nblk, int nWaves, int nBig, int nOd, int nCb, int ellM, int ellOver, const CoarseCfg& c)
{
	const int agg = c.agg, cl = c.cl, nc = c.nc, spmvRows = c.spmvRows;
	const int gridSetup = (Pf + PCG_SETUP_POSES - 1) / PCG_SETUP_POSES, gridUpd = (Pf + 39) / 40, gridSpmv = (Pf + spmvRows - 1) / spmvRows;
	st = DeviceStructure();
	st.nWaves = nWaves; st.wave_lm = d_waveLm.data();
	st.nBig = nBig; st.big_lm = d_bigLm.data();
	st.nblk = nblk; st.hsc_rowptr = d_rowptr.data(); st.hsc_colind = d_colind.data();
	st.adj_ptr = d_adjPtr.data(); st.adj_blk = d_adjBlk.data(); st.adj_col = d_adjCol.data();
	st.ell = d_ell.data(); st.ell_m = ellM; st.ell_over = ellOver;
	st.hsc_blkrow = d_blkrow.data(); st.nOd = nOd; st.nDiagProd = diagProdBlocks; st.od_blocks = d_odBlocks.data(); st.nHeavy = std::min(heavyBlocks, nOd);
	if (d_prodEa.size() > ((size_t)1 << 19)) st.nHeavy = 0;
	st.inv_rows8 = Lf >= 250000;
	st.prod_ea = d_prodEa.data(); st.prod_eb = d_prodEb.data();
	if (!localRanges) fillProdLm();
	st.prod_lm = d_prodLm.data();
	st.prod_beg = localRanges ? d_prodBeg.data() : d_prodPtr.data(); st.prod_end = localRanges ? d_prodEnd.data() : d_prodPtr.data() + 1;
	st.pe_beg = localRanges ? d_peBeg.data() : d_pePtr.data(); st.pe_end = localRanges ? d_peEnd.data() : d_pePtr.data() + 1;
	st.pe_edge = d_peEdge.data(); st.e_rec = d_erec.data();
	st.nCb = nCb; st.cb_I = d_cbI.data(); st.cb_J = d_cbJ.data(); st.cb_ptr = d_cbPtr.data(); st.cb_blk = d_cbBlk.data(); st.cb_wi = d_cbWi.data(); st.cb_wj = d_cbWj.data();
	sys = DeviceSystem();
	sys.hsc = d_red.data(); sys.bsc = d_red.data() + (size_t)36 * nblk; sys.bp = sys.bsc + (size_t)6 * Pf;
	sys.lm_sys = d_lmSys.data(); sys.lm_inv = d_lmInv.data(); sys.xp = d_xp.data(); sys.xl = d_xl.data(); sys.slots = slotsDev; sys.host_flags = flagsDev; sys.parts = d_parts.data();
	sys.maxdiag = d_maxdiag.data(); sys.fail = d_fail.data();
	sys.minv = d_minv.data(); sys.r = d_r.data(); sys.z = d_z.data(); sys.p0 = d_p0.data(); sys.p1 = d_p1.data(); sys.ap = d_ap.data();
	sys.rz = d_rz.data(); sys.pq = d_pq.data(); sys.iters = d_iters.data(); sys.kbase = d_kbase.data(); sys.ticket = d_ticket.data();
	dropPcgGraph();
	firstInvValid = false; firstInvPending = false; prevRunIters.clear();
	sys.rzStride = rzStrideCfg; sys.pqStride = pqStrideCfg; sys.npq = gridSpmv;
	sys.nrz0 = agg > 0 ? nc : gridSetup; sys.nrz = agg > 0 ? nc : gridUpd; sys.done = d_done.data();
	coarseValid = false;
	d_qpart.resize(agg > 0 ? (size_t)(agg / spmvRows) * 6 * cl * nc : 1); d_gjPivots.resize(2 * 32 * 32); sys.gj_pivots = d_gjPivots.data();
	sys.qpart = d_qpart.data();
	d_qpart.zero(stream);
	d_lamS.resize(1); d_lmState.resize(32); sys.lam_dev = d_lamS.data();
	sys.upper = agg > 0 && agg <= pcg_rows_max_aggregate() && (spmvUpper < 0 ? spmvRows == 4 : spmvUpper != 0) ? 1 : 0;
	if (sys.upper)
	{
		d_tq.resize((size_t)6 * nblk); sys.tq = d_tq.data(); d_hrow.release(); sys.hrow = nullptr;
		d_lowpos.resize((size_t)nblk); sys.lowpos = d_lowpos.data();
		DeviceGraph gg; gg.Pf = Pf;
		launch_build_lowpos(gg, st, d_lowpos.data(), stream);
		sys.npq = spmv_upper_grid(Pf);
	}
	else
	{
		d_hrow.resize((size_t)36 * 20 * ellM * Pf); sys.hrow = d_hrow.data();
		d_hrow.zero(stream);
	}
	sys.spmv_rows = spmvRows;
	sys.agg = agg; sys.nc = nc; sys.cl = agg > 0 ? cl : 1; sys.inv_agg = agg > 0 ? Scalar(1) / Scalar(agg) : Scalar(0); sys.acinv = d_coarse[0].data(); sys.rc = d_rc.data(); sys.r2 = d_r2.data();
	sys.acinv32 = fp32Inverse() && agg > 0 ? d_coarse32[0].data() : nullptr;
	cutReductionParts();
	haveStructure = true;
	structRelPairs = h_relPairs; cntStructureBuilds++;
}

void cuba_hip_solver::cutReductionParts()
{
	redParts.clear();
	if (partHi < 0 || st.nblk <= 0 || st.nOd <= 0 || Pf <= 0) return;
	const size_t matrixBytes = (size_t)36 * st.nblk * sizeof(Scalar);
	const int want = redChunks > 0 ? redChunks : (int)std::min<size_t>(8, matrixBytes >> 23);
	if (want <= 1) return;
	std::vector<int> rowptr((size_t)Pf + 1), od((size_t)st.nOd);
	HIP_TRY(hipMemcpyAsync(rowptr.data(), d_rowptr.data(), sizeof(int) * rowptr.size(), hipMemcpyDeviceToHost, stream));
	HIP_TRY(hipMemcpyAsync(od.data(), d_odBlocks.data(), sizeof(int) * od.size(), hipMemcpyDeviceToHost, stream));
	sync();
	std::vector<int> cut{ 0 };
	for (int c = 1; c < want; c++)
	{
		const int target = (int)((long long)st.nblk * c / want);
		const int b = *std::lower_bound(rowptr.begin(), rowptr.end(), target);
		if (b > cut.back() && b < st.nblk) cut.push_back(b);
	}
	if (cut.size() < 2) return;
	cut.push_back(st.nblk);
	const int C = (int)cut.size() - 1;
	std::vector<std::vector<int>> lists(C);
	std::vector<int> heavy(C, 0);
	int c = 0;
	for (int i = 0; i < st.nOd; i++)
	{
		if (od[i] >= 0) c = (int)(std::upper_bound(cut.begin() + 1, cut.end(), od[i]) - (cut.begin() + 1));
		lists[c].push_back(od[i]);
		if (i < st.nHeavy) heavy[c]++;
	}
	od.clear();
	for (int k = 0; k < C; k++)
	{
		RedPart p;
		p.od.begin = (int)od.size(); od.insert(od.end(), lists[k].begin(), lists[k].end()); p.od.end = (int)od.size(); p.od.heavy = heavy[k];
// ... 322 lines not shown
	d_k32a.resize(n32); d_k32b.resize(n32); d_v32a.resize(n32); d_v32b.resize(n32);
	sortTemp(n32);
	d_odBlocks.resize(nblk);
	if (localRanges)
	{
		fillProdLm();
		d_prodBeg.resize(nblk); d_prodEnd.resize(nblk);
		topo::launch_segment_subrange(d_prodPtr.data(), nblk, d_prodLm.data(), lo, hi, d_prodBeg.data(), d_prodEnd.data(), stream);
	}
	topo::launch_od_keys(localRanges ? d_prodBeg.data() : d_prodPtr.data(), localRanges ? d_prodEnd.data() : d_prodPtr.data() + 1,
		d_blkrow.data(), d_colind.data(), nblk, farOffset(), BP_HEAVY, d_k32a.data(), d_v32a.data(), cnt, stream);
	if (nblk) HIP_TRY(topo::sort_u32_u32(d_topoTemp.data(), d_topoTemp.size(), d_k32a.data(), d_k32b.data(), d_v32a.data(), d_v32b.data(), nblk, 32, stream));
	topo::launch_copy_u32_to_int(d_v32b.data(), d_odBlocks.data(), nblk, stream);
	const int nAdj = std::max(0, 2 * nblk - Pf);
	d_lowerPtr.resize((size_t)Pf + 1); d_adjPtr.resize((size_t)Pf + 1); d_adjBlk.resize(nAdj); d_adjCol.resize(nAdj); d_adjRow.resize(nAdj);
	d_tmpI0.resize(std::max(std::max((size_t)nblk, (size_t)nAdj), d_tmpI0.size())); d_tmpI1.resize(std::max((size_t)nAdj, d_tmpI1.size()));
	d_k64a.resize(std::max((size_t)nblk, d_k64a.size())); d_k64b.resize(std::max((size_t)nblk, d_k64b.size()));
	topo::launch_transpose_keys(d_colind.data(), d_blkrow.data(), nblk, d_k64a.data(), d_v32a.data(), stream);
	if (nblk) HIP_TRY(topo::sort_u64_u32(d_topoTemp.data(), d_topoTemp.size(), d_k64a.data(), d_k64b.data(), d_v32a.data(), d_v32b.data(), nblk, 64, stream));
	topo::launch_keys_hi(d_k64b.data(), nblk, Pf, d_tmpI0.data(), stream);
	topo::launch_segment_ptr(d_tmpI0.data(), nblk, Pf, d_lowerPtr.data(), stream);
	topo::launch_adj_ptr(d_rowptr.data(), d_lowerPtr.data(), Pf, d_adjPtr.data(), cnt, stream);
	topo::launch_adj_fill(d_rowptr.data(), d_colind.data(), d_blkrow.data(), d_lowerPtr.data(), d_k64b.data(), d_v32b.data(), nblk, d_adjPtr.data(),
		d_adjBlk.data(), d_adjCol.data(), d_adjRow.data(), stream);
	const CoarseCfg cc = coarseConfig();
	d_cbI.resize(nAdj); d_cbJ.resize(nAdj); d_cbPtr.resize((size_t)nAdj + 1); d_cbBlk.resize(nAdj);
	d_cbWi.resize(cc.cl == 2 ? nAdj : 0); d_cbWj.resize(cc.cl == 2 ? nAdj : 0);
	if (cc.nc > 0 && nAdj > 0)
	{
		topo::launch_coarse_keys(d_adjRow.data(), d_adjCol.data(), nAdj, cc.agg, cc.nc, d_k32a.data(), d_v32a.data(), stream);
		HIP_TRY(topo::sort_u32_u32(d_topoTemp.data(), d_topoTemp.size(), d_k32a.data(), d_k32b.data(), d_v32a.data(), d_v32b.data(), nAdj, bitsFor((long long)cc.nc * cc.nc), stream));
		topo::launch_heads_u32(d_k32b.data(), nAdj, d_tmpI0.data(), stream);
		HIP_TRY(topo::inclusive_scan_i32(d_topoTemp.data(), d_topoTemp.size(), d_tmpI0.data(), d_tmpI1.data(), nAdj, stream));
		topo::launch_coarse_lists(d_k32b.data(), d_v32b.data(), d_tmpI1.data(), d_adjBlk.data(), d_adjRow.data(), d_adjCol.data(), nAdj, cc.agg, cc.nc, Pf, cc.cl,
			d_cbI.data(), d_cbJ.data(), d_cbPtr.data(), d_cbBlk.data(), d_cbWi.data(), d_cbWj.data(), cnt, stream);
	}
	allocSystem(nblk, cc);
	HIP_TRY(hipMemcpyAsync(hc, cnt, sizeof hc, hipMemcpyDeviceToHost, stream));
	std::vector<int> earlyOd;
	if (earlyTiles)
	{
		HIP_TRY(hipEventSynchronize(evTileInputs));
		const int* pp = h_tileStage + 2 * (size_t)nblk;
		std::vector<int> len(nblk);
		for (int k = 0; k < nblk; k++) len[k] = pp[k + 1] - pp[k];
		earlyOd = rowGroupedOrder(h_tileStage, h_tileStage + nblk, len.data(), nblk);
	}
	sync();
	lap("structure (device): adjacency, coarse lists, allocations");
	const int maxRow = hc[topo::CNT_MAXROW];
	const int ellM = std::min(3, (maxRow + 19) / 20), ellOver = maxRow > 20 * ellM;
	d_ell.resize((size_t)Pf * ellM * 20);
	topo::launch_ell(d_adjPtr.data(), d_adjBlk.data(), d_adjCol.data(), Pf, ellM, d_ell.data(), stream);
	if (!reorderActive && !reorderTried && tryReorder(nblk, hc[topo::CNT_FARBLOCKS]))
	{
		reorderTried = true;
		buildStructureDevice();
		return;
	}
	reorderTried = false;
	diagProdBlocks = hc[topo::CNT_DIAGPROD]; heavyBlocks = hc[topo::CNT_NHEAVY];
	int nOdList = hc[topo::CNT_NOD];
	if (earlyTiles)
	{
		d_odBlocks.upload(earlyOd, stream);
		sync();
		nOdList = (int)earlyOd.size(); heavyBlocks = 0;
	}
	else if (rowGroupedBlocks(npairs) && nblk > 0)
	{
		std::vector<int> hRow(nblk), hBeg(nblk), hEnd(nblk), hCol;
		hCol.resize(nblk); HIP_TRY(hipMemcpyAsync(hCol.data(), d_colind.data(), sizeof(int) * nblk, hipMemcpyDeviceToHost, stream));
		HIP_TRY(hipMemcpyAsync(hRow.data(), d_blkrow.data(), sizeof(int) * nblk, hipMemcpyDeviceToHost, stream));
		HIP_TRY(hipMemcpyAsync(hBeg.data(), localRanges ? d_prodBeg.data() : d_prodPtr.data(), sizeof(int) * nblk, hipMemcpyDeviceToHost, stream));
		HIP_TRY(hipMemcpyAsync(hEnd.data(), localRanges ? d_prodEnd.data() : d_prodPtr.data() + 1, sizeof(int) * nblk, hipMemcpyDeviceToHost, stream));
		sync();
		for (int k = 0; k < nblk; k++) hEnd[k] -= hBeg[k];
		const std::vector<int> od = rowGroupedOrder(hRow.data(), hCol.data(), hEnd.data(), nblk);
		d_odBlocks.upload(od, stream);
		sync();
		nOdList = (int)od.size(); heavyBlocks = 0;
	}
	lap("structure (device): block order of the Schur pass");
	publishStructure(nblk, nWaves, nBig, nOdList, cc.nc > 0 ? hc[topo::CNT_NCB] : 0, ellM, ellOver, cc);
	hostPatternValid = false;
	lap("structure (device): published");
	if (std::getenv("CUBA_HIP_DEBUG")) std::fprintf(stderr, "[cuba_hip] structure (device): nblk %d products %lld waves %d big %d od %d coarse blocks %d max row %d\n",
		nblk, npairs, nWaves, nBig, hc[topo::CNT_NOD], hc[topo::CNT_NCB], maxRow);
	const double dt = std::chrono::duration<double>(Clock::now() - t0).count();
	prof[1] += 0.5 * dt; prof[5] += 0.5 * dt;
}

std::vector<cuba_hip_solver::CallerBlock> cuba_hip_solver::callerBlocks()
{
	ensureHostPattern();
	std::vector<CallerBlock> b; b.reserve(h_colind.size());
	for (int i = 0; i < Pf; i++)
		for (int k = h_rowptr[i]; k < h_rowptr[i + 1]; k++)
		{
			int r = poseOldOfNew[i], c = poseOldOfNew[h_colind[k]];
			const bool tr = r > c;
			if (tr) std::swap(r, c);
			b.push_back(CallerBlock{ ((uint64_t)(uint32_t)r << 32) | (uint32_t)c, k, tr });
		}
	std::sort(b.begin(), b.end(), [](const CallerBlock& x, const CallerBlock& y) { return x.key < y.key; });
	return b;
// ... 12 lines not shown
```

cuda-bundle-adjustment_amd/csrc/ba_solver.hip:

```cpp
#include "ba_solver.hpp"

using namespace cubahip;


namespace cubahip_host
{
std::atomic<int> g_liveHandles{ 0 };
}

namespace
{
std::string g_createError;

template <typename F>
int guarded(cuba_hip_solver* s, F&& f)
{
	if (!s) return CUBA_HIP_ERR_INVALID_ARGUMENT;
	try
	{
		if (hipSetDevice(s->device) != hipSuccess) { s->lastError = "hipSetDevice failed"; return CUBA_HIP_ERR_RUNTIME; }
		f();
		return CUBA_HIP_OK;
	}
	catch (const HipError& e)
// ... 72 lines not shown
	g_liveHandles.fetch_sub(1, std::memory_order_relaxed);
	return CUBA_HIP_OK;
}

const char* cuba_hip_last_error(const cuba_hip_solver* s) { return s ? s->lastError.c_str() : "null solver handle"; }

int cuba_hip_set_stream(cuba_hip_solver* s, void* hip_stream)
{
	return guarded(s, [&] {
		s->sync();
		if (s->ownStream && s->stream) { HIP_TRY(hipStreamDestroy(s->stream)); s->ownStream = false; }
		s->stream = (hipStream_t)hip_stream;
	});
}

int cuba_hip_set_option(cuba_hip_solver* s, const char* key, double value)
{
	return guarded(s, [&] {
		if (!key) throw ArgError{ "null key" };
		const std::string k(key);
		if (k == "pcg_tol") s->pcgTol = value;
		else if (k == "pcg_max_iter") { s->pcgMaxIter = (int)value; s->haveStructure = false; }
		else if (k == "heuristics") { s->heuristics = value != 0; s->firstInvValid = false; s->firstInvPending = false; }
		else if (k == "precond_fp32") { s->precondFp32 = value != 0; s->haveStructure = false; s->coarseValid = false; s->dropPcgGraph(); }
		else if (k == "pose_reorder") { s->poseReorder = value != 0; s->haveStructure = false; }
		else if (k == "device_setup") { s->deviceSetup = value != 0; s->haveStructure = false; }
		else if (k == "mixed_precision") s->mixedPrecision = value != 0 && sizeof(Scalar) == 8;
		else if (k == "pcg_accept_unconverged") s->acceptUnconverged = value != 0;
		else if (k == "direct_fallback") { s->directFallback = value != 0; s->directSticky = false; }
		else if (k == "direct_after") s->directAfter = (int)value;
		else if (k == "direct_max_tiles") { s->directMaxTiles = (int)value; s->directRefused = false; s->directPlanValid = false; }
		else if (k == "direct_slack") { s->directSlack = (int)value; s->directRefused = false; s->directPlanValid = false; }
		else if (k == "reduced_solver")
		{
			if (value != 0 && value != 1) throw ArgError{ "reduced_solver: 0 = block PCG with the exact solver as fallback, 1 = exact sparse Cholesky for every solve" };
			s->directAlways = value != 0;
		}
		else if (k == "pcg_aggregate") { s->pcgAggregate = (int)value; s->haveStructure = false; }
		else if (k == "coarse_linear") { s->coarseLinear = value != 0; s->haveStructure = false; }
		else if (k == "covariance_workspace_mb")
		{
			if (value < 0 || value > (double)(1 << 30)) throw ArgError{ "covariance_workspace_mb must lie in 0 .. 2^30 (0 = automatic)" };
			s->covWorkspaceMb = value;
		}
		else if (k == "landmark_reorder") s->lmReorder = value != 0;
		else if (k == "reduction_chunks")
		{
			if (value < 0 || value > 64) throw ArgError{ "reduction_chunks must lie in 0 .. 64" };
			s->redChunks = (int)value; s->haveStructure = false;
		}
		else if (k == "spmv_upper") { s->spmvUpper = (int)value; s->haveStructure = false; s->dropPcgGraph(); }
		else if (k == "pcg_graph") { s->useGraph = value != 0; s->dropPcgGraph(); }
		else if (k == "profile") s->profile = value != 0;
		else throw ArgError{ "unknown option: " + k };
	});
}


int cuba_hip_hint_unchanged(cuba_hip_solver* s, int same_edges, int same_values)
{
	return guarded(s, [&] { s->hintSameEdges = same_edges != 0; s->hintSameValues = same_edges != 0 && same_values != 0; });
}

int cuba_hip_set_graph(cuba_hip_solver* s, int Pt, int Pf, int Lt, int Lf, const double* q, const double* t, const double* cam,
	const double* Xw, int E, const int32_t* edge_pose, const int32_t* edge_landmark, const uint8_t* edge_dim,
	const double* meas, const double* omega)
{
	return guarded(s, [&] { s->setGraph(Pt, Pf, Lt, Lf, q, t, cam, Xw, E, edge_pose, edge_landmark, edge_dim, meas, omega); });
}

int cuba_hip_set_graph_begin(cuba_hip_solver* s, int Pt, int Pf, int Lt, int Lf, const double* q, const double* t, const double* cam,
	const double* Xw, int E, const int32_t* edge_pose, const int32_t* edge_landmark, const uint8_t* edge_dim,
	const double* meas, const double* omega)
{
	return guarded(s, [&] { s->setGraph(Pt, Pf, Lt, Lf, q, t, cam, Xw, E, edge_pose, edge_landmark, edge_dim, meas, omega, true); });
}

int cuba_hip_set_graph_partition(cuba_hip_solver* s, int Pt, int Pf, int Lt, int Lf,
	const double* q, const double* t, const double* cam, const double* Xw,
	int E, const int32_t* edge_pose, const int32_t* edge_landmark, const uint8_t* edge_dim,
	const double* meas, const double* omega, int landmark_begin, int landmark_end)
{
	return guarded(s, [&] {
		if (landmark_end < 0) throw ArgError{ "bad landmark range" };
		s->setGraph(Pt, Pf, Lt, Lf, q, t, cam, Xw, E, edge_pose, edge_landmark, edge_dim, meas, omega, false, landmark_begin, landmark_end);
	});
}

int cuba_hip_set_graph_end(cuba_hip_solver* s)
{
	return guarded(s, [&] {
		if (!s->haveGraph) throw StateError{ "set_graph_begin must be called first" };
		if (s->upStream) HIP_TRY(hipStreamSynchronize(s->upStream));
		s->finishValues();
	});
}

int cuba_hip_set_robust_kernel(cuba_hip_solver* s, int edge_type, int kind, double delta)
{
	return guarded(s, [&] {
		if (edge_type < 0 || edge_type > 1 || kind < 0 || kind > 2) throw ArgError{ "bad robust kernel" };
		s->rk[edge_type] = RobustKernel{ kind, (Scalar)delta };
	});
}

int cuba_hip_build_structure(cuba_hip_solver* s) { return guarded(s, [&] { s->buildStructure(); s->sync(); }); }
// ... 137 lines not shown

int cuba_hip_chi_squares_end(cuba_hip_solver* s)
{
	return guarded(s, [&] { s->sync(); });
}

int cuba_hip_gate_edges(cuba_hip_solver* s, const double chi2_max[2], int require_positive_depth, int mode, int64_t counts[6], double* chi2_per_edge)
{
	return guarded(s, [&] { s->gateEdges(chi2_max, require_positive_depth != 0, mode, counts, chi2_per_edge); });
}

int cuba_hip_set_edge_active(cuba_hip_solver* s, const uint8_t* active) { return guarded(s, [&] { s->setEdgeActive(active); }); }
int cuba_hip_get_edge_active(cuba_hip_solver* s, uint8_t* active) { return guarded(s, [&] { s->getEdgeActive(active); }); }
int cuba_hip_landmark_active_edges(cuba_hip_solver* s, int32_t* per_landmark) { return guarded(s, [&] { s->landmarkActiveEdges(per_landmark); }); }

int cuba_hip_get_profile(cuba_hip_solver* s, double seconds[CUBA_HIP_PROFILE_ITEMS])
{
	return guarded(s, [&] { for (int i = 0; i < CUBA_HIP_PROFILE_ITEMS; i++) seconds[i] = s->prof[i]; });
}

int cuba_hip_get_counters(cuba_hip_solver* s, int64_t c[8])
{
	return guarded(s, [&] {
		c[0] = s->cntPcgIters; c[1] = s->cntTrials; c[2] = s->st.nblk; c[3] = s->nmul;
		c[4] = s->cntCoarseRefresh; c[5] = s->cntPcgLooks; c[6] = s->cntPcgEnqueued; c[7] = 6 * (int64_t)s->sys.cl * s->sys.nc;
	});
}

int cuba_hip_get_counter(cuba_hip_solver* s, const char* name, int64_t* value)
{
	return guarded(s, [&] {
		if (!name || !value) throw ArgError{ "null argument" };
		const std::string k(name);
		if (k == "pcg_iterations") *value = s->cntPcgIters;
		else if (k == "lm_trials") *value = s->cntTrials;
		else if (k == "coarse_refreshes") *value = s->cntCoarseRefresh;
		else if (k == "coarse_inline_inversions") *value = s->cntCoarseInline;
		else if (k == "pcg_host_looks") *value = s->cntPcgLooks;
		else if (k == "pcg_iterations_enqueued") *value = s->cntPcgEnqueued;
		else if (k == "pcg_unconverged_solves") *value = s->cntPcgUnconverged;
		else if (k == "pcg_graph_instantiations") *value = s->gb.builds.load();
		else if (k == "precond_fp32_fallbacks") *value = s->cntFp32Fallbacks;
		else if (k == "pcg_iterations_plain_launches") *value = s->cntPcgPlain;
		else if (k == "batch_full_trials") *value = s->cntBatchFullTrials;
		else if (k == "batch_iteration_trials") *value = s->cntBatchIterTrials;
		else if (k == "host_looks") *value = s->cntHostLooks;
		else if (k == "exact_solve_fallbacks") *value = s->cntDirect;
		else if (k == "exact_solve_failures") *value = s->cntDirectFailed;
		else if (k == "graph_uploads") *value = s->cntUploads;
		else if (k == "structure_builds") *value = s->cntStructureBuilds;
		else if (k == "value_bytes_uploaded") *value = s->cntValueBytes;
		else if (k == "edge_sorts") *value = s->cntEdgeSorts;
		else if (k == "late_decision_records") *value = s->cntLateRecords;
		else if (k == "covariance_ns") *value = (int64_t)(1e9 * s->covSeconds);
		else if (k == "covariance_pairs_ns") *value = (int64_t)(1e9 * s->covPairsSeconds);
		else if (k == "covariance_pairs_chunks") *value = s->covPairChunks;
		else throw ArgError{ "unknown counter: " + k };
	});
}

int cuba_hip_get_pcg_history(cuba_hip_solver* s, int32_t* iterations, int capacity, int* n_solves, int64_t* n_unconverged)
{
	return guarded(s, [&] {
		const int n = (int)s->pcgHistory.size();
		if (n_solves) *n_solves = n;
		if (n_unconverged) *n_unconverged = s->cntPcgUnconverged;
		if (iterations) for (int i = 0; i < std::min(n, capacity); i++) iterations[i] = s->pcgHistory[i];
	});
}

int cuba_hip_get_hsc_structure(cuba_hip_solver* s, int32_t* row_ptr, int32_t* col_ind, int* nblk)
{
	return guarded(s, [&] {
		s->need();
		s->ensureHostPattern();
		if (nblk) *nblk = (int)s->h_colind.size();
		if (!s->reorderActive)
		{
			if (row_ptr) std::memcpy(row_ptr, s->h_rowptr.data(), sizeof(int) * s->h_rowptr.size());
			if (col_ind) std::memcpy(col_ind, s->h_colind.data(), sizeof(int) * s->h_colind.size());
			return;
		}
		const auto blocks = s->callerBlocks();
		if (row_ptr)
		{
			for (int i = 0; i <= s->Pf; i++) row_ptr[i] = 0;
			for (const auto& b : blocks) row_ptr[(int)(b.key >> 32) + 1]++;
			for (int i = 0; i < s->Pf; i++) row_ptr[i + 1] += row_ptr[i];
		}
		if (col_ind) for (size_t k = 0; k < blocks.size(); k++) col_ind[k] = (int)(uint32_t)blocks[k].key;
	});
}

int cuba_hip_get_array(cuba_hip_solver* s, int which, double* out, size_t* count)
{
	return guarded(s, [&] {
		s->need();
		const Scalar* src = nullptr; size_t n = 0;
		switch (which)
		{
		case CUBA_HIP_ARRAY_BP: src = s->sys.bp; n = (size_t)6 * s->Pf; break;
		case CUBA_HIP_ARRAY_BSC: src = s->sys.bsc; n = (size_t)6 * s->Pf; break;
		case CUBA_HIP_ARRAY_XP: src = s->sys.xp; n = (size_t)6 * s->Pf; break;
		case CUBA_HIP_ARRAY_XL: src = s->sys.xl; n = (size_t)3 * s->Lf; break;
		case CUBA_HIP_ARRAY_LM_SYS: src = s->sys.lm_sys; n = (size_t)9 * s->Lf; break;
		case CUBA_HIP_ARRAY_HSC: src = s->sys.hsc; n = (size_t)36 * s->st.nblk; break;
		default: throw ArgError{ "unknown array id" };
		}
		if (count) *count = n;
		if (out && n)
		{
			if (which == CUBA_HIP_ARRAY_XL) src = s->landmarkRowsForCaller(src, s->Lf, 3);
			else if (which == CUBA_HIP_ARRAY_LM_SYS) src = s->landmarkRowsForCaller(src, s->Lf, 9);
			s->downloadAsDouble(src, out, n);
			if (s->reorderActive)
			{
				if (which == CUBA_HIP_ARRAY_BP || which == CUBA_HIP_ARRAY_BSC || which == CUBA_HIP_ARRAY_XP) s->permutePoseArray(out, 6, false);
				else if (which == CUBA_HIP_ARRAY_HSC)
				{
					const std::vector<double> v(out, out + n);
					const auto blocks = s->callerBlocks();
					for (size_t k = 0; k < blocks.size(); k++)
					{
						const double* src36 = v.data() + 36 * (size_t)blocks[k].src;
						double* dst = out + 36 * k;
						for (int c = 0; c < 6; c++)
							for (int r = 0; r < 6; r++) dst[c * 6 + r] = blocks[k].transposed ? src36[r * 6 + c] : src36[c * 6 + r];
					}
				}
			}
		}
	});
}

int cuba_hip_compute_covariance(cuba_hip_solver* s, double* pose_cov, double* landmark_cov, int* not_positive_definite)
{
	return guarded(s, [&] {
		const bool ok = s->computeCovariance(pose_cov, landmark_cov);
		if (!ok) s->lastError = "marginal covariances: non-positive pivot (the undamped reduced matrix is not positive definite)";
		if (not_positive_definite) *not_positive_definite = ok ? 0 : 1;
	});
}

int cuba_hip_get_covariance_blocks(cuba_hip_solver* s, double* values)
{
	return guarded(s, [&] { s->covarianceBlocks(values); });
}

int cuba_hip_compute_covariance_pairs(cuba_hip_solver* s, int n, const int32_t* kind_a, const int32_t* index_a, const int32_t* kind_b,
	const int32_t* index_b, double* out, int* not_positive_definite)
{
	return guarded(s, [&] {
		const bool ok = s->computeCovariancePairs(n, kind_a, index_a, kind_b, index_b, out);
		if (!ok) s->lastError = "covariance pairs: non-positive pivot (the undamped reduced matrix is not positive definite)";
		if (not_positive_definite) *not_positive_definite = ok ? 0 : 1;
	});
}

static int factor_chi_squares(cuba_hip_solver* s, int kind, double* out)
{
	return guarded(s, [&] {
		if (!s->haveGraph) throw StateError{ "set_graph must be called first" };
// ... 630 lines not shown
```

cuda-bundle-adjustment_amd/csrc/ba_solver.hpp:

```cpp
#pragma once

#include <algorithm>
#include <chrono>
#include <cmath>
#include <cstdarg>
#include <cstdio>
#include <cstdlib>
#include <cstring>
#include <numeric>
#include <string>
#include <thread>
#include <atomic>
#include <functional>
#include <condition_variable>
#include <deque>
#include <map>
#include <mutex>
#include <vector>

#include "../../include/cuba_hip.h"
#include "ba_kernels.hpp"
#include "host_pool.hpp"
#include "ba_structure.hpp"
#include "ba_upload_plan.hpp"

using namespace cubahip;
static_assert(UPLOAD_POSE_LIMIT == STEREO_BIT, "the upload plan refuses the poses a sorted edge cannot name");

namespace cubahip_host
{

struct HipError { hipError_t code; const char* what; const char* file; int line; };

#define HIP_TRY(expr)                                                    \
	do {                                                                 \
		hipError_t err__ = (expr);                                       \
		if (err__ != hipSuccess) throw HipError{ err__, #expr, __FILE__, __LINE__ }; \
	} while (0)

struct StateError { std::string msg; };
struct ArgError { std::string msg; };

template <typename T>
class DevBuf
{
public:
	DevBuf() = default;
	DevBuf(const DevBuf&) = delete;
	DevBuf& operator=(const DevBuf&) = delete;
	~DevBuf() { release(); }
	void release()
	{
		if (ptr_) (void)hipFree(ptr_);
		ptr_ = nullptr; size_ = cap_ = 0;
	}
	void resize(size_t n)
// ... 562 lines not shown
	bool directRefused = false;
	bool directPlanValid = false;
	double directSeconds = 0, directPlanSeconds = 0;
	SparseCholPlan directPlan;
	SparseChol directDev;
	DevBuf<Scalar> d_scTiles, d_scTilesT, d_scY, d_scRinv;
	DevBuf<int> d_scInts, d_scFail;
	int64_t cntDirect = 0, cntDirectFailed = 0;
	int64_t directPlanBuilds = 0;
	bool directUsable() const { return directFallback && !directRefused && Pf > 0; }
	int pcgBudget(int maxIter) const;
	bool ensureDirectPlan();
	bool solveDirect();

	SelInvPlan selPlan;
	int64_t selPlanFor = -1;
	SelInv selDev;
	DevBuf<int> d_selInts;
	DevBuf<Scalar> d_sigma, d_covW, d_covPose, d_covBlk, d_covLm;
	bool covBlocksValid = false;
	double covSeconds = 0;
	bool computeCovariance(double* poseCov, double* lmCov);
	void covarianceBlocks(double* out);
	double covWorkspaceMb = 0;
	double covPairsSeconds = 0;
	int covPairChunks = 0;
	PairWork covPairWork;
	DevBuf<Scalar> d_pairOut;
	bool computeCovariancePairs(int n, const int32_t* kindA, const int32_t* indexA, const int32_t* kindB, const int32_t* indexB, double* out);

	struct CoarseJob { cuba_hip_solver* h; int first; bool firstInvCopy; bool ownEvent; };
	void launchCoarseJobs(std::vector<CoarseJob>& jobs, hipEvent_t common = nullptr);
	GjJob* h_gjTab = nullptr; DevBuf<unsigned char> d_gjTab; hipEvent_t evGjTab = nullptr;
	struct SolveCtx
	{
		int maxIter = 0, budget = 0, predicted = 32, k0 = 0, looks = 0, eagerIters = 0;
		int itersDone = -1;
		Scalar tol2 = 0;
		bool twoLevel = false, direct = false, graphs = false, converged = false, result = false;
		bool batched = false;
		std::vector<CoarseJob>* deferCoarse = nullptr;
		bool deferLaunch = false;
		bool deferred = false;
		bool sideLater = false;
		int sideFirst = -1;
		const Scalar* copySrc = nullptr; Scalar* copyDst = nullptr; size_t copyCount = 0;
		volatile int* hInts = nullptr;
		Clock::time_point tSolve0;
	};
	bool solveBegin(SolveCtx& sc);
	void enqueueCoarseSide(int first);
	void enqueueInversionTail(hipStream_t side, bool firstInvCopy);
	bool coarseSideLater = false;
	bool solveBrokeDown(SolveCtx& sc);
	bool solveEnd(SolveCtx& sc);
	bool solveReducedOnce();
	bool retryWithFp64Inverse(bool ok);

	void backSubstitute();

	bool solve();

	void update();

	double computeScale(double lam);

	void push() { need(); HIP_TRY(hipMemcpyAsync(d_backup.data(), d_state.data(), d_state.size() * sizeof(Scalar), hipMemcpyDeviceToDevice, stream)); }
	void pop() { need(); HIP_TRY(hipMemcpyAsync(d_state.data(), d_backup.data(), d_state.size() * sizeof(Scalar), hipMemcpyDeviceToDevice, stream)); }

	int optimize(int niter, double* chi2Out);
	int optimizeDeviceDecision(int niter, double* chi2Out);
	struct LmRun
	{
		static constexpr int maxq = 10;
		int niter = 0, enq = 0, seen = 0, done = 0, rejRun = 0;
		bool stop = false;
		bool chain = false;
		bool restoreInPass = false;
		double lam = 0, F = 0, tagBase = 0;
		double* chi2Out = nullptr;
		LmDevice lm;
		bool absorb(const volatile double* rec)
		{
			if (rec[7] != tagBase + (double)(seen + 1)) return false;
			const bool acc = rec[5] != 0.0;
			const double rho = rec[2];
			lam = rec[3]; F = rec[4];
			seen++;
			if (acc) rejRun = 0; else rejRun++;
			const bool iterationEnds = acc || rejRun == maxq || !(rho < 0);
			if (!iterationEnds) return true;
			if (chi2Out) chi2Out[done] = F;
			done++;
			if (done == niter || rejRun == maxq || rho <= 0 || !std::isfinite(lam)) stop = true;
			rejRun = 0;
			return true;
		}
	};
	void lmRunBegin(LmRun& r, int niter, double* chi2Out, bool chain = false);
	const double* lmRestoreFlag = nullptr;
	void lmAbsorb(LmRun& r, int upto);
	bool lmBeforeTrial(LmRun& r);
	bool lmAfterSolveHost(LmRun& r);
	bool lmAfterSolve(LmRun& r, bool ok);
	bool fullyBatchable() const;
	int lmRunEnd(LmRun& r);
// ... 19 lines not shown
```

cuda-bundle-adjustment_amd/csrc/ba_structure.hip:

```cpp
#include "ba_structure.hpp"

#include <cstring>

#include <rocprim/rocprim.hpp>

#include "ba_kernels.hpp"

namespace cubahip
{
namespace topo
{

size_t sort_temp_bytes(size_t n)
{
	size_t b = 0;
	(void)rocprim::radix_sort_pairs(nullptr, b, (const uint64_t*)nullptr, (uint64_t*)nullptr, (const uint64_t*)nullptr, (uint64_t*)nullptr, n, 0, 64, (hipStream_t)0);
	return b + 256;
}

size_t scan_temp_bytes(size_t n)
{
	size_t b = 0;
	(void)rocprim::exclusive_scan(nullptr, b, (const long long*)nullptr, (long long*)nullptr, 0LL, n, rocprim::plus<long long>(), (hipStream_t)0);
	return b + 256;
// ... 231 lines not shown
{
	const int k = blockIdx.x * T + threadIdx.x;
	if (k >= nblk) return;
	const int r = blkrow[k], c = colind[k];
	keys[k] = r == c ? KEY_MAX : (((uint64_t)(uint32_t)c << 32) | (uint32_t)r);
	vals[k] = (uint32_t)k;
}

__global__ __launch_bounds__(T) void keys_hi_kernel(const uint64_t* keys, int n, int limit, int* hi)
{
	const int i = blockIdx.x * T + threadIdx.x;
	if (i < n) hi[i] = (int)min((uint64_t)limit, keys[i] >> 32);
}

__global__ __launch_bounds__(T) void adj_ptr_kernel(const int* rowptr, const int* lowerPtr, int Pf, int* adjPtr, int* counters)
{
	const int i = blockIdx.x * T + threadIdx.x;
	int len = 0;
	if (i <= Pf)
	{
		adjPtr[i] = lowerPtr[i] + rowptr[i];
		if (i < Pf) len = (lowerPtr[i + 1] + rowptr[i + 1]) - (lowerPtr[i] + rowptr[i]);
	}
#pragma unroll
	for (int o = 32; o > 0; o >>= 1) len = max(len, __shfl_xor(len, o));
	if ((threadIdx.x & 63) == 0 && len) atomicMax(&counters[CNT_MAXROW], len);
}

__global__ __launch_bounds__(T) void adj_fill_kernel(const int* rowptr, const int* colind, const int* blkrow, const int* lowerPtr, const uint64_t* tKeys,
	const uint32_t* tBlk, int nblk, const int* adjPtr, int* adjBlk, int* adjCol, int* adjRow)
{
	const int t = blockIdx.x * T + threadIdx.x;
	if (t >= nblk) return;
	const uint64_t key = tKeys[t];
	if (key != KEY_MAX)
	{
		const int c = (int)(key >> 32), r = (int)(uint32_t)key;
		const int a = adjPtr[c] + (t - lowerPtr[c]);
		adjBlk[a] = (int)tBlk[t] | (int)0x80000000; adjCol[a] = r; adjRow[a] = c;
	}
	const int i = blkrow[t];
	const int a = adjPtr[i] + (lowerPtr[i + 1] - lowerPtr[i]) + (t - rowptr[i]);
	adjBlk[a] = t; adjCol[a] = colind[t]; adjRow[a] = i;
}

__global__ __launch_bounds__(T) void ell_kernel(const int* adjPtr, const int* adjBlk, const int* adjCol, int Pf, int M, int2* ell)
{
	const size_t x = (size_t)blockIdx.x * T + threadIdx.x;
	const int W = 20 * M;
	if (x >= (size_t)Pf * W) return;
	const int i = (int)(x / W), e = (int)(x - (size_t)i * W);
	const int a0 = adjPtr[i], n = adjPtr[i + 1] - a0;
	ell[x] = e < n ? int2{ adjBlk[a0 + e], adjCol[a0 + e] } : int2{ 0, -1 };
}

__global__ __launch_bounds__(T) void coarse_keys_kernel(const int* adjRow, const int* adjCol, int nAdj, int agg, int nc, uint32_t* keys, uint32_t* vals)
{
	const int a = blockIdx.x * T + threadIdx.x;
	if (a >= nAdj) return;
	keys[a] = (uint32_t)((adjRow[a] / agg) * nc + adjCol[a] / agg);
	vals[a] = (uint32_t)a;
}

__global__ __launch_bounds__(T) void heads_u32_kernel(const uint32_t* keys, int n, int* head)
{
	const int j = blockIdx.x * T + threadIdx.x;
	if (j < n) head[j] = (j == 0 || keys[j] != keys[j - 1]) ? 1 : 0;
}

__device__ __forceinline__ Scalar coarse_weight(int pose, int agg, int Pf)
{
	if (pose == Pf - 1 && Pf % agg == 1) return Scalar(0);
	return Scalar(2 * (pose % agg) + 1 - agg) / Scalar(agg);
}

__global__ __launch_bounds__(T) void coarse_lists_kernel(const uint32_t* keys, const uint32_t* order, const int* cbOfEntry, const int* adjBlk, const int* adjRow,
	const int* adjCol, int nAdj, int agg, int nc, int Pf, int cl, int* cbI, int* cbJ, int* cbPtr, int* cbBlk, Scalar* cbWi, Scalar* cbWj, int* counters)
{
	const int x = blockIdx.x * T + threadIdx.x;
	if (x >= nAdj) return;
	const uint32_t key = keys[x];
	const int a = (int)order[x], cb = cbOfEntry[x] - 1;
	if (x == 0 || keys[x - 1] != key) { cbI[cb] = (int)(key / (uint32_t)nc); cbJ[cb] = (int)(key % (uint32_t)nc); cbPtr[cb] = x; }
	cbBlk[x] = adjBlk[a];
	if (cl == 2) { cbWi[x] = coarse_weight(adjRow[a], agg, Pf); cbWj[x] = coarse_weight(adjCol[a], agg, Pf); }
	if (x == nAdj - 1) { cbPtr[cb + 1] = nAdj; counters[CNT_NCB] = cb + 1; }
}

template <bool WRITE>
__global__ __launch_bounds__(64) void wave_list_kernel(const int* lm_ptr, int lo, int hi, const int* chunkOfs, int* chunkCounts,
	int* wave_lm, int* big_lm)
{
	const int c = blockIdx.x * 64 + threadIdx.x;
	const int l0 = lo + c * WAVE_CHUNK;
	if (l0 >= hi) return;
	const int l1 = min(hi, l0 + WAVE_CHUNK);
	int nW = 0, nB = 0;
	int w = 0, bI = 0;
	if (WRITE) { w = chunkOfs[2 * c]; bI = chunkOfs[2 * c + 1]; }
	int start = -1, cnt = 0;
	int prev = lm_ptr[l0];
	for (int l = l0; l < l1; l++)
	{
		const int next = lm_ptr[l + 1];
		const int n = next - prev;
		prev = next;
// ... 179 lines not shown
{
	if (E > 0) hipLaunchKernelGGL(remap_landmarks_kernel, grid_for((size_t)E), dim3(T), 0, s, elIn, newOfOld, E, elOut);
}
void launch_permute_rows(const Scalar* src, Scalar* dst, const int* newOfOld, int nrows, int width, bool toInternal, hipStream_t s)
{
	const size_t total = (size_t)nrows * width;
	if (total) hipLaunchKernelGGL(permute_rows_kernel, grid_for(total), dim3(T), 0, s, src, dst, newOfOld, total, width, toInternal ? 1 : 0);
}

void launch_entry_heads(const uint64_t* keys, size_t n, int* head, hipStream_t s)
{
	if (n > 0) hipLaunchKernelGGL(entry_heads_kernel, grid_for(n), dim3(T), 0, s, keys, n, head);
}

void launch_blocks_from_entries(const uint64_t* keys, const uint64_t* vals, const int* blkOfEntry, size_t n, int nSeeds, const int* seedScan, int* colind,
	int* blkrow, int* prod_ptr, int* prod_ea, int* prod_eb, hipStream_t s)
{
	if (n == 0) return;
	if (!seedScan) hipLaunchKernelGGL(blocks_from_entries_kernel, grid_for(n), dim3(T), 0, s, keys, vals, blkOfEntry, n, nSeeds, colind, blkrow, prod_ptr, prod_ea, prod_eb);
	else hipLaunchKernelGGL(blocks_from_entries_seeded_kernel, grid_for(n), dim3(T), 0, s, keys, vals, blkOfEntry, n, nSeeds, seedScan, colind, blkrow, prod_ptr, prod_ea, prod_eb);
}

void launch_segment_subrange(const int* ptr, int nseg, const int* vals, int vlo, int vhi, int* beg, int* end, hipStream_t s)
{
	if (nseg > 0) hipLaunchKernelGGL(segment_subrange_kernel, grid_for(nseg), dim3(T), 0, s, ptr, nseg, vals, vlo, vhi, beg, end);
}

void launch_od_keys(const int* prod_beg, const int* prod_end, const int* blkrow, const int* colind, int nblk, int farOffset, int heavy, uint32_t* keys, uint32_t* vals, int* counters, hipStream_t s)
{
	if (nblk > 0) hipLaunchKernelGGL(od_keys_kernel, grid_for(nblk), dim3(T), 0, s, prod_beg, prod_end, blkrow, colind, nblk, farOffset, heavy, keys, vals, counters);
}

void launch_remap_poses(const int* epIn, const int* newOfOld, int E, int Pf, int* epOut, hipStream_t s)
{
	if (E > 0) hipLaunchKernelGGL(remap_poses_kernel, grid_for(E), dim3(T), 0, s, epIn, newOfOld, E, Pf, epOut);
}

void launch_transpose_keys(const int* colind, const int* blkrow, int nblk, uint64_t* keys, uint32_t* vals, hipStream_t s)
{
	if (nblk > 0) hipLaunchKernelGGL(transpose_keys_kernel, grid_for(nblk), dim3(T), 0, s, colind, blkrow, nblk, keys, vals);
}

void launch_keys_hi(const uint64_t* keys, int n, int limit, int* hi, hipStream_t s)
{
	if (n > 0) hipLaunchKernelGGL(keys_hi_kernel, grid_for(n), dim3(T), 0, s, keys, n, limit, hi);
}

void launch_ell(const int* adjPtr, const int* adjBlk, const int* adjCol, int Pf, int M, int2* ell, hipStream_t s)
{
	const size_t n = (size_t)Pf * 20 * M;
	if (n > 0) hipLaunchKernelGGL(ell_kernel, grid_for(n), dim3(T), 0, s, adjPtr, adjBlk, adjCol, Pf, M, ell);
}

void launch_coarse_keys(const int* adjRow, const int* adjCol, int nAdj, int agg, int nc, uint32_t* keys, uint32_t* vals, hipStream_t s)
{
	if (nAdj > 0) hipLaunchKernelGGL(coarse_keys_kernel, grid_for(nAdj), dim3(T), 0, s, adjRow, adjCol, nAdj, agg, nc, keys, vals);
}

void launch_heads_u32(const uint32_t* keys, int n, int* head, hipStream_t s)
{
	if (n > 0) hipLaunchKernelGGL(heads_u32_kernel, grid_for(n), dim3(T), 0, s, keys, n, head);
}

void launch_coarse_lists(const uint32_t* keys, const uint32_t* order, const int* cbOfEntry, const int* adjBlk, const int* adjRow, const int* adjCol, int nAdj,
	int agg, int nc, int Pf, int cl, int* cbI, int* cbJ, int* cbPtr, int* cbBlk, Scalar* cbWi, Scalar* cbWj, int* counters, hipStream_t s)
{
	if (nAdj > 0) hipLaunchKernelGGL(coarse_lists_kernel, grid_for(nAdj), dim3(T), 0, s, keys, order, cbOfEntry, adjBlk, adjRow, adjCol, nAdj, agg, nc, Pf, cl,
		cbI, cbJ, cbPtr, cbBlk, cbWi, cbWj, counters);
}

void launch_wave_count(const int* lm_ptr, int lo, int hi, int* chunkCounts, hipStream_t s)
{
	const int nChunks = (hi - lo + WAVE_CHUNK - 1) / WAVE_CHUNK;
	if (nChunks > 0) hipLaunchKernelGGL(wave_list_kernel<false>, dim3((nChunks + 63) / 64), dim3(64), 0, s, lm_ptr, lo, hi, (const int*)nullptr, chunkCounts,
		(int*)nullptr, (int*)nullptr);
}

void launch_wave_scan(int* chunkCounts, int nChunks, int* counters, hipStream_t s)
{
	hipLaunchKernelGGL(wave_scan_kernel, dim3(1), dim3(1024), 0, s, chunkCounts, nChunks, counters);
}

void launch_wave_write(const int* lm_ptr, int lo, int hi, const int* chunkOfs, int* wave_lm, int* big_lm, hipStream_t s)
{
	const int nChunks = (hi - lo + WAVE_CHUNK - 1) / WAVE_CHUNK;
	if (nChunks > 0) hipLaunchKernelGGL(wave_list_kernel<true>, dim3((nChunks + 63) / 64), dim3(64), 0, s, lm_ptr, lo, hi, chunkOfs, (int*)nullptr, wave_lm, big_lm);
}

void launch_unsort(const uint32_t* perm, const Scalar* sorted, int E, double* callerOrder, hipStream_t s)
{
	if (E > 0) hipLaunchKernelGGL(unsort_kernel, grid_for(E), dim3(T), 0, s, perm, sorted, E, callerOrder);
}

void launch_adj_ptr(const int* rowptr, const int* lowerPtr, int Pf, int* adjPtr, int* counters, hipStream_t s)
{
	hipLaunchKernelGGL(adj_ptr_kernel, grid_for((size_t)Pf + 1), dim3(T), 0, s, rowptr, lowerPtr, Pf, adjPtr, counters);
}

void launch_adj_fill(const int* rowptr, const int* colind, const int* blkrow, const int* lowerPtr, const uint64_t* tKeys, const uint32_t* tBlk, int nblk,
	const int* adjPtr, int* adjBlk, int* adjCol, int* adjRow, hipStream_t s)
{
	if (nblk > 0) hipLaunchKernelGGL(adj_fill_kernel, grid_for(nblk), dim3(T), 0, s, rowptr, colind, blkrow, lowerPtr, tKeys, tBlk, nblk, adjPtr, adjBlk, adjCol, adjRow);
}

}
}
// ... 1 lines not shown
```

cuda-bundle-adjustment_amd/csrc/ba_structure.hpp:

```cpp
#pragma once

#include <cstddef>
#include <cstdint>

#include <hip/hip_runtime.h>

#include "ba_math.hpp"

namespace cubahip
{
namespace topo
{

size_t sort_temp_bytes(size_t n);
size_t scan_temp_bytes(size_t n);
hipError_t sort_u64_u32(void* temp, size_t tempBytes, const uint64_t* kin, uint64_t* kout, const uint32_t* vin, uint32_t* vout, size_t n, int endBit, hipStream_t s);
hipError_t sort_u64_u64(void* temp, size_t tempBytes, const uint64_t* kin, uint64_t* kout, const uint64_t* vin, uint64_t* vout, size_t n, int endBit, hipStream_t s);
hipError_t sort_u32_u32(void* temp, size_t tempBytes, const uint32_t* kin, uint32_t* kout, const uint32_t* vin, uint32_t* vout, size_t n, int endBit, hipStream_t s);
hipError_t exclusive_scan_i64(void* temp, size_t tempBytes, const long long* in, long long* out, size_t n, hipStream_t s);
hipError_t inclusive_scan_i32(void* temp, size_t tempBytes, const int* in, int* out, size_t n, hipStream_t s);

enum { CNT_BAD = 0, CNT_FREE_EDGES, CNT_NOD, CNT_MAXROW, CNT_NCB, CNT_NWAVES, CNT_NBIG, CNT_FARBLOCKS, CNT_DIAGPROD, CNT_NHEAVY, CNT_COUNT = 16 };

void launch_edge_keys(const int* ep, const int* el, const uint8_t* dim, int E, int Pt, int Pf, int Lt, int Lf,
	uint64_t* keys, uint32_t* vals, int* counters, hipStream_t s);
void launch_gather_edges(const uint32_t* perm, const int* ep, const int* el, const uint8_t* dim, const double* meas, const double* omega, int E,
	int* e_pose, int* e_lm, Scalar* mu, Scalar* mv, Scalar* mr, Scalar* w, hipStream_t s);
void launch_scatter_values(const int* ids, const double* packed, int n, double* meas, double* omega, hipStream_t s);
void launch_segment_ptr(const int* keys, int n, int nSeg, int* ptr, hipStream_t s);

void launch_lm_pairs(const int* lm_ptr, const int* e_pose, int Lf, int Pf, int* nfree, long long* pairCount, long long* freeCount, hipStream_t s);
void launch_pose_keys(const int* e_pose, int E, int Pf, uint32_t* keys, uint32_t* vals, hipStream_t s);
void launch_copy_u32_to_int(const uint32_t* in, int* out, int n, hipStream_t s);
void launch_gather_int(const int* idx, const int* src, size_t n, int* dst, hipStream_t s);
void launch_pattern_entries(const int* lm_ptr, const int* e_pose, const int* e_lm, const int* nfree, const long long* pairBase,
	int E, int Lf, int Pf, uint64_t* keys, uint64_t* vals, const uint64_t* extraSeeds, int nExtra, hipStream_t s);
void launch_seed_flags(const uint64_t* vals, size_t n, int* flag, hipStream_t s);
void launch_entry_heads(const uint64_t* keys, size_t n, int* head, hipStream_t s);
void launch_blocks_from_entries(const uint64_t* keys, const uint64_t* vals, const int* blkOfEntry, size_t n, int nSeeds, const int* seedScan,
	int* colind, int* blkrow, int* prod_ptr, int* prod_ea, int* prod_eb, hipStream_t s);
void launch_od_keys(const int* prod_beg, const int* prod_end, const int* blkrow, const int* colind, int nblk, int farOffset, int heavy, uint32_t* keys, uint32_t* vals, int* counters, hipStream_t s);
void launch_segment_subrange(const int* ptr, int nseg, const int* vals, int vlo, int vhi, int* beg, int* end, hipStream_t s);
void launch_remap_poses(const int* epIn, const int* newOfOld, int E, int Pf, int* epOut, hipStream_t s);
void launch_transpose_keys(const int* colind, const int* blkrow, int nblk, uint64_t* keys, uint32_t* vals, hipStream_t s);
void launch_keys_hi(const uint64_t* keys, int n, int limit, int* hi, hipStream_t s);
void launch_adj_ptr(const int* rowptr, const int* lowerPtr, int Pf, int* adjPtr, int* counters, hipStream_t s);
void launch_adj_fill(const int* rowptr, const int* colind, const int* blkrow, const int* lowerPtr, const uint64_t* tKeys, const uint32_t* tBlk, int nblk,
	const int* adjPtr, int* adjBlk, int* adjCol, int* adjRow, hipStream_t s);
void launch_ell(const int* adjPtr, const int* adjBlk, const int* adjCol, int Pf, int M, int2* ell, hipStream_t s);
void launch_coarse_keys(const int* adjRow, const int* adjCol, int nAdj, int agg, int nc, uint32_t* keys, uint32_t* vals, hipStream_t s);
void launch_heads_u32(const uint32_t* keys, int n, int* head, hipStream_t s);
void launch_coarse_lists(const uint32_t* keys, const uint32_t* order, const int* cbOfEntry, const int* adjBlk, const int* adjRow, const int* adjCol,
	int nAdj, int agg, int nc, int Pf, int cl, int* cbI, int* cbJ, int* cbPtr, int* cbBlk, Scalar* cbWi, Scalar* cbWj, int* counters, hipStream_t s);
constexpr int WAVE_CHUNK = 256;
void launch_wave_count(const int* lm_ptr, int lo, int hi, int* chunkCounts, hipStream_t s);
void launch_wave_scan(int* chunkCounts, int nChunks, int* counters, hipStream_t s);
void launch_wave_write(const int* lm_ptr, int lo, int hi, const int* chunkCounts, int* wave_lm, int* big_lm, hipStream_t s);
void launch_lm_first_last(const int* ep, const int* el, int E, int Lt, int* first, int* last, hipStream_t s);
void launch_lm_order_keys(const int* first, const int* last, int Lf, uint64_t* keys, uint32_t* vals, hipStream_t s);
void launch_lm_order_map(const uint32_t* order, int Lf, int Lt, int* newOfOld, hipStream_t s);
void launch_remap_landmarks(const int* elIn, const int* newOfOld, int E, int* elOut, hipStream_t s);
void launch_permute_rows(const Scalar* src, Scalar* dst, const int* newOfOld, int nrows, int width, bool toInternal, hipStream_t s);

void launch_unsort(const uint32_t* perm, const Scalar* sorted, int E, double* callerOrder, hipStream_t s);

}
}
```

include/cuba_hip.h:

```cpp
#ifndef CUBA_HIP_H_
#define CUBA_HIP_H_

#include <stddef.h>
#include <stdint.h>

#ifdef __cplusplus
extern "C" {
#endif

typedef struct cuba_hip_solver cuba_hip_solver;

typedef enum cuba_hip_status
{
	CUBA_HIP_OK = 0,
	CUBA_HIP_ERR_INVALID_ARGUMENT = 1,
	CUBA_HIP_ERR_RUNTIME = 2,
	CUBA_HIP_ERR_STATE = 3,
	CUBA_HIP_ERR_NO_DEVICE = 4
} cuba_hip_status;

enum { CUBA_HIP_ROBUST_NONE = 0, CUBA_HIP_ROBUST_HUBER = 1, CUBA_HIP_ROBUST_TUKEY = 2 };
enum { CUBA_HIP_EDGE_MONOCULAR = 0, CUBA_HIP_EDGE_STEREO = 1 };
enum { CUBA_HIP_VERTEX_POSE = 0, CUBA_HIP_VERTEX_LANDMARK = 1 };

enum { CUBA_HIP_PROFILE_ITEMS = 8 };

enum
{
	CUBA_HIP_ARRAY_BP = 0,
	CUBA_HIP_ARRAY_BSC = 1,
	CUBA_HIP_ARRAY_XP = 2,
	CUBA_HIP_ARRAY_XL = 3,
	CUBA_HIP_ARRAY_LM_SYS = 4,
	CUBA_HIP_ARRAY_HSC = 5,
	CUBA_HIP_ARRAY_STATE = 6
};


int cuba_hip_create(int device, cuba_hip_solver** out);
int cuba_hip_destroy(cuba_hip_solver* s);
const char* cuba_hip_last_error(const cuba_hip_solver* s);
const char* cuba_hip_version(void);
int cuba_hip_scalar_size(void);

void* cuba_hip_host_alloc(size_t bytes);
void cuba_hip_host_free(void* p);

int cuba_hip_set_stream(cuba_hip_solver* s, void* hip_stream);

int cuba_hip_set_option(cuba_hip_solver* s, const char* key, double value);


int cuba_hip_set_graph(cuba_hip_solver* s, int Pt, int Pf, int Lt, int Lf,
	const double* q, const double* t, const double* cam, const double* Xw,
	int E, const int32_t* edge_pose, const int32_t* edge_landmark, const uint8_t* edge_dim,
	const double* meas, const double* omega);

int cuba_hip_set_graph_begin(cuba_hip_solver* s, int Pt, int Pf, int Lt, int Lf,
	const double* q, const double* t, const double* cam, const double* Xw,
	int E, const int32_t* edge_pose, const int32_t* edge_landmark, const uint8_t* edge_dim,
	const double* meas, const double* omega);
int cuba_hip_set_graph_end(cuba_hip_solver* s);

int cuba_hip_hint_unchanged(cuba_hip_solver* s, int same_edges, int same_values);

int cuba_hip_set_robust_kernel(cuba_hip_solver* s, int edge_type, int kind, double delta);

int cuba_hip_build_structure(cuba_hip_solver* s);


int cuba_hip_compute_errors(cuba_hip_solver* s, double* chi2);

int cuba_hip_build_system(cuba_hip_solver* s);

int cuba_hip_max_diagonal(cuba_hip_solver* s, double* max_diag);

int cuba_hip_set_lambda(cuba_hip_solver* s, double lambda);
int cuba_hip_restore_diagonal(cuba_hip_solver* s);

int cuba_hip_schur(cuba_hip_solver* s);
int cuba_hip_solve_reduced(cuba_hip_solver* s, int* ok);
int cuba_hip_back_substitute(cuba_hip_solver* s);
int cuba_hip_solve(cuba_hip_solver* s, int* ok);

int cuba_hip_update(cuba_hip_solver* s);

int cuba_hip_compute_scale(cuba_hip_solver* s, double lambda, double* scale);

// ... 127 lines not shown
```

Before: 837.6 million.

## Fold row-ordered Hsc copy into Schur launch and fuse PCG setup with first iteration

The Schur linearize kernel now writes each off-diagonal block directly into the row-ordered (ELL) hrow layout through a precomputed block-to-slot map, so the separate expand pass can be skipped. The PCG setup is also fused with the first two-level preconditioner application and first fused PCG iteration in one kernel, with the first-inverse carry-over copy done beforehand. This removes a full pass over the Schur blocks and a few kernel launches per LM iteration, at the cost of extra scattered writes in the Schur kernel, a more complex setup kernel that may limit occupancy, and new gating logic and debug options.

```diff
diff --git a/cuda-bundle-adjustment_amd/capi.py b/cuda-bundle-adjustment_amd/capi.py
--- a/cuda-bundle-adjustment_amd/capi.py
+++ b/cuda-bundle-adjustment_amd/capi.py
@@ -18,7 +18,7 @@
 _ip = C.POINTER(C.c_int32)
 _u8p = C.POINTER(C.c_uint8)
 
-ARRAY_IDS = dict(bp=0, bsc=1, xp=2, xl=3, lm_sys=4, hsc=5, state=6)
+ARRAY_IDS = dict(bp=0, bsc=1, xp=2, xl=3, lm_sys=4, hsc=5, state=6, hrow=7, minv=8, z=9, r=10, rc=11, rz=12, hrow_slot=13)
 PROFILE_KEYS = (
     "0: Initialize Optimizer", "1: Build Structure", "2: Compute Error", "3: Build System",
     "4: Schur Complement", "5: Symbolic Decomposition", "6: Numerical Decomposition", "7: Update Solution")
diff --git a/cuda-bundle-adjustment_amd/csrc/ba_kernels.hpp b/cuda-bundle-adjustment_amd/csrc/ba_kernels.hpp
--- a/cuda-bundle-adjustment_amd/csrc/ba_kernels.hpp
+++ b/cuda-bundle-adjustment_amd/csrc/ba_kernels.hpp
@@ -39,6 +39,7 @@
 	int *adj_ptr = nullptr, *adj_blk = nullptr, *adj_col = nullptr;
 	int2* ell = nullptr;
 	int ell_m = 0, ell_over = 0;
+	const int2* hrow_slot = nullptr;
 	int* hsc_blkrow = nullptr;
 	int nOd = 0;
 	int nDiagProd = 0;
@@ -173,7 +174,7 @@
 struct BlockPassRange { int begin, end, heavy; };
 void launch_linearize_dm(const DeviceGraph& g, const DeviceStructure& st, const DeviceSystem& sys, int mode, Scalar lambda, hipStream_t s,
 	Scalar* backupSrc = nullptr, Scalar* backupDst = nullptr, size_t backupCount = 0, const BlockPassRange* range = nullptr, const double* restoreFlag = nullptr,
-	const DeviceLandmarkPriors* lp = nullptr);
+	const DeviceLandmarkPriors* lp = nullptr, const int2* hrowSlot = nullptr);
 void launch_block_pass(const DeviceGraph& g, const DeviceStructure& st, const DeviceSystem& sys, const BlockPassRange& range, hipStream_t s);
 
 void launch_pose_maxdiag(const DeviceGraph& g, const DeviceStructure& st, const DeviceSystem& sys, hipStream_t s);
@@ -249,6 +250,9 @@
 
 void launch_hsc_expand(const DeviceGraph& g, const DeviceStructure& st, const DeviceSystem& sys, hipStream_t s);
 void launch_pcg_setup_expand(const DeviceGraph& g, const DeviceStructure& st, const DeviceSystem& sys, Scalar lambda, hipStream_t s,
+	const Scalar* copySrc = nullptr, Scalar* copyDst = nullptr, size_t copyCount = 0, bool expand = true);
+constexpr int PCG2_SETUP_FIRST_MAX_AGG = 512;
+void launch_pcg2_setup_first(const DeviceGraph& g, const DeviceStructure& st, const DeviceSystem& sys, Scalar lambda, int maxIter, Scalar tol2, hipStream_t s,
 	const Scalar* copySrc = nullptr, Scalar* copyDst = nullptr, size_t copyCount = 0);
 
 constexpr int SC_T = 32;
diff --git a/cuda-bundle-adjustment_amd/csrc/ba_linearize.hip b/cuda-bundle-adjustment_amd/csrc/ba_linearize.hip
--- a/cuda-bundle-adjustment_amd/csrc/ba_linearize.hip
+++ b/cuda-bundle-adjustment_amd/csrc/ba_linearize.hip
@@ -418,6 +418,7 @@
 	const bool on = blk0 >= 0;
 	const int blk = on ? blk0 : 0;
 	const int a = on ? st.hsc_blkrow[blk] : 0, b = on ? st.hsc_colind[blk] : 0;
+	const int2 hs = on && st.hrow_slot ? st.hrow_slot[blk] : int2{ -1, -1 };
 	ET qa[4], cama[5], qb[4], camb[5];
 	load_pose_as<ET>(g, a, qa, cama);
 	load_pose_as<ET>(g, b, qb, camb);
@@ -463,6 +464,24 @@
 #pragma unroll
 			for (int r = 0; r < 6; r++)
 				if (GROUP == 64 ? (c * 6 + r) == gl : (c * 6 + r) % GROUP == gl) dst[c * 6 + r] = -Ts[r][c];
+		if (hs.x >= 0)
+		{
+			Scalar* ha = sys.hrow + 36 * (size_t)hs.x;
+#pragma unroll
+			for (int r = 0; r < 6; r++)
+#pragma unroll
+				for (int c = 0; c < 6; c++)
+					if (GROUP == 64 ? (r * 6 + c) == gl : (r * 6 + c) % GROUP == gl) ha[r * 6 + c] = -Ts[r][c];
+		}
+		if (hs.y >= 0)
+		{
+			Scalar* hb = sys.hrow + 36 * (size_t)hs.y;
+#pragma unroll
+			for (int c = 0; c < 6; c++)
+#pragma unroll
+				for (int r = 0; r < 6; r++)
+					if (GROUP == 64 ? (c * 6 + r) == gl : (c * 6 + r) % GROUP == gl) hb[c * 6 + r] = -Ts[r][c];
+		}
 	}
 	else if (gl == 0)
 	{
@@ -532,9 +551,11 @@
 
 template <typename ET>
 static void launch_linearize_dm_t(const DeviceGraph& g, const DeviceStructure& stAll, const DeviceSystem& sys, int mode, Scalar lambda, hipStream_t s,
-	Scalar* backupSrc, Scalar* backupDst, size_t backupCount, const BlockPassRange* range, const double* restoreFlag, const DeviceLandmarkPriors* lp)
-{
-	const DeviceStructure st = range ? block_pass_view(stAll, *range) : stAll;
+	Scalar* backupSrc, Scalar* backupDst, size_t backupCount, const BlockPassRange* range, const double* restoreFlag, const DeviceLandmarkPriors* lp,
+	const int2* hrowSlot)
+{
+	DeviceStructure st = range ? block_pass_view(stAll, *range) : stAll;
+	st.hrow_slot = mode == 1 && !range && g.Pf > 0 && st.nOd > 0 && st.nDiagProd == 0 && sys.hrow ? hrowSlot : nullptr;
 	if (st.nWaves > 0)
 	{
 		const LandmarkGrid L(st, backupSrc, backupCount);
@@ -571,11 +592,12 @@
 }
 
 void launch_linearize_dm(const DeviceGraph& g, const DeviceStructure& st, const DeviceSystem& sys, int mode, Scalar lambda, hipStream_t s,
-	Scalar* backupSrc, Scalar* backupDst, size_t backupCount, const BlockPassRange* range, const double* restoreFlag, const DeviceLandmarkPriors* lp)
+	Scalar* backupSrc, Scalar* backupDst, size_t backupCount, const BlockPassRange* range, const double* restoreFlag, const DeviceLandmarkPriors* lp,
+	const int2* hrowSlot)
 {
 	if (lp && lp->n == 0) lp = nullptr;
-	if (st.mixed && sizeof(Scalar) == 8) launch_linearize_dm_t<float>(g, st, sys, mode, lambda, s, backupSrc, backupDst, backupCount, range, restoreFlag, lp);
-	else launch_linearize_dm_t<Scalar>(g, st, sys, mode, lambda, s, backupSrc, backupDst, backupCount, range, restoreFlag, lp);
+	if (st.mixed && sizeof(Scalar) == 8) launch_linearize_dm_t<float>(g, st, sys, mode, lambda, s, backupSrc, backupDst, backupCount, range, restoreFlag, lp, hrowSlot);
+	else launch_linearize_dm_t<Scalar>(g, st, sys, mode, lambda, s, backupSrc, backupDst, backupCount, range, restoreFlag, lp, hrowSlot);
 }
 
 void batch_fill_linearize(const DeviceGraph& g, const DeviceStructure& st, const Scalar* backupSrc, Scalar* backupDst, size_t backupCount, BatchTrial& t)
diff --git a/cuda-bundle-adjustment_amd/csrc/ba_lm.hip b/cuda-bundle-adjustment_amd/csrc/ba_lm.hip
--- a/cuda-bundle-adjustment_amd/csrc/ba_lm.hip
+++ b/cuda-bundle-adjustment_amd/csrc/ba_lm.hip
@@ -144,7 +144,7 @@
 	waitAssembled();
 	const bool parts = mode == 1 && !redParts.empty();
 	launch_linearize_dm(g, st, sys, mode, lam, stream, withBackup ? d_state.data() : nullptr, d_backup.data(), d_state.size(), parts ? &redParts[0].od : nullptr,
-		withBackup ? lmRestoreFlag : nullptr, landmarkPriors());
+		withBackup ? lmRestoreFlag : nullptr, landmarkPriors(), mode == 1 && hrowFromSchur ? d_hrowSlot.data() : nullptr);
 	if (parts && !partsByCaller)
 		for (size_t c = 1; c < redParts.size(); c++) launch_block_pass(g, st, sys, redParts[c].od, stream);
 	if (factors()) launch_pose_factor_linearize(g, st, sys, pf, mode, stream);
@@ -158,6 +158,7 @@
 	{
 		StageTimer tm(this, 4);
 		zeroReduced();
+		hrowFromSchur = false;
 		partsByCaller = true;
 		try { linearize(1, lambda, false); } catch (...) { partsByCaller = false; throw; }
 		partsByCaller = false;
@@ -227,11 +228,28 @@
 	return v;
 }
 
+bool cuba_hip_solver::foldUsable()
+{
+	if (foldSetup == 0 || profile || partHi >= 0 || Pf <= 0 || sys.upper || sys.agg <= 0 || !sys.hrow || !redParts.empty() || st.nDiagProd != 0 || st.nOd <= 0
+		|| factors() || d_hrowSlot.size() != (size_t)st.nblk) return false;
+	if (!hrowSlotChecked)
+	{
+		std::vector<int2> map(d_hrowSlot.size());
+		HIP_TRY(hipMemcpyAsync(map.data(), d_hrowSlot.data(), sizeof(int2) * map.size(), hipMemcpyDeviceToHost, stream));
+		sync();
+		checkHrowSlot(map, (size_t)Pf * 20 * st.ell_m);
+		hrowSlotChecked = true;
+	}
+	return true;
+}
+
 void cuba_hip_solver::schur(bool withBackup)
 {
 	need();
 	StageTimer tm(this, 4);
 	zeroReduced();
+	hrowFromSchur = (foldChain || foldStageCalls) && foldUsable();
+	if (hrowFromSchur) cntFoldRows++;
 	linearize(1, lambda, withBackup);
 }
 
@@ -341,6 +359,8 @@
 {
 	lastSolveBrokeDown = false;
 	need();
+	const bool rowsStored = hrowFromSchur;
+	hrowFromSchur = false;
 	if (Pf == 0) { sc.result = true; return true; }
 	const int maxIter = sc.maxIter = maxIterAlloc;
 	const Scalar tol2 = sc.tol2 = pcgTol * pcgTol;
@@ -365,13 +385,28 @@
 		takeInverse = true; pendingInv = -1;
 	}
 	const bool deferred = sc.deferLaunch && twoLevel && coarseValid;
+	const bool carryOver = twoLevel && !coarseValid && heuristics && firstInvValid;
+	const bool foldFirst = rowsStored && foldSetup == 1 && twoLevel && sys.agg <= PCG2_SETUP_FIRST_MAX_AGG && !deferred && (coarseValid || carryOver);
 	{
 		const bool f32 = fp32Inverse();
 		const Scalar* cpSrc = !takeInverse ? nullptr : f32 ? reinterpret_cast<const Scalar*>(d_coarse32[1].data()) : d_coarse[0].data();
 		Scalar* cpDst = f32 ? reinterpret_cast<Scalar*>(d_coarse32[0].data()) : d_coarse[2].data();
 		const size_t cpCount = f32 ? inv32Count() / 2 : invCount;
 		if (deferred) { sc.deferred = true; sc.copySrc = cpSrc; sc.copyDst = cpDst; sc.copyCount = cpCount; }
-		else launch_pcg_setup_expand(g, st, sys, lambda, stream, cpSrc, cpDst, cpCount);
+		else if (foldFirst)
+		{
+			ensureOverlapObjects();
+			if (carryOver)
+			{
+				HIP_TRY(hipStreamWaitEvent(stream, evFirstInv, 0));
+				if (f32) HIP_TRY(hipMemcpyAsync(d_coarse32[0].data(), d_firstInv32.data(), inv32Count() * sizeof(float), hipMemcpyDeviceToDevice, stream));
+				else HIP_TRY(hipMemcpyAsync(d_coarse[2].data(), d_firstInv.data(), sizeof(Scalar) * invCount, hipMemcpyDeviceToDevice, stream));
+			}
+			sys.acinv = d_coarse[2].data();
+			cntFoldFirst++;
+			launch_pcg2_setup_first(g, st, sys, lambda, maxIter, tol2, stream, cpSrc, cpDst, cpCount);
+		}
+		else launch_pcg_setup_expand(g, st, sys, lambda, stream, cpSrc, cpDst, cpCount, !rowsStored);
 	}
 	if (twoLevel)
 	{
@@ -381,9 +416,12 @@
 			const size_t invBytes = sizeof(Scalar) * (size_t)36 * sys.cl * sys.cl * sys.nc * sys.nc;
 			if (!coarseValid && heuristics && firstInvValid)
 			{
-				HIP_TRY(hipStreamWaitEvent(stream, evFirstInv, 0));
-				if (fp32Inverse()) HIP_TRY(hipMemcpyAsync(d_coarse32[0].data(), d_firstInv32.data(), inv32Count() * sizeof(float), hipMemcpyDeviceToDevice, stream));
-				else HIP_TRY(hipMemcpyAsync(d_coarse[2].data(), d_firstInv.data(), invBytes, hipMemcpyDeviceToDevice, stream));
+				if (!foldFirst)
+				{
+					HIP_TRY(hipStreamWaitEvent(stream, evFirstInv, 0));
+					if (fp32Inverse()) HIP_TRY(hipMemcpyAsync(d_coarse32[0].data(), d_firstInv32.data(), inv32Count() * sizeof(float), hipMemcpyDeviceToDevice, stream));
+					else HIP_TRY(hipMemcpyAsync(d_coarse[2].data(), d_firstInv.data(), invBytes, hipMemcpyDeviceToDevice, stream));
+				}
 				pendingInv = -1;
 				coarseValid = true; sideAge = overlapPeriod(); firstInvPending = true;
 			}
@@ -417,7 +455,7 @@
 				assemblePending = true; cntCoarseRefresh++;
 			}
 		}
-		if (!deferred) launch_pcg2_fused(g, sys, 0, 0, maxIter, tol2, 0, stream);
+		if (!deferred && !foldFirst) launch_pcg2_fused(g, sys, 0, 0, maxIter, tol2, 0, stream);
 	}
 	const bool graphs = sc.graphs = useGraph && !sc.batched && g_liveHandles.load(std::memory_order_relaxed) <= 1;
 	if (useGraph && !graphs && (!pcgGraphs.empty() || graphsOrderedFor)) dropPcgGraph();
@@ -490,6 +528,12 @@
 	SolveCtx sc;
 	sc.sideLater = coarseSideLater;
 	if (solveBegin(sc)) return sc.result;
+	if (debugSetupOnly)
+	{
+		if (sc.sideFirst >= 0) { enqueueCoarseSide(sc.sideFirst); sc.sideFirst = -1; }
+		sync();
+		return true;
+	}
 	const int maxIter = sc.maxIter; const Scalar tol2 = sc.tol2; const bool graphs = sc.graphs; const int predicted = sc.predicted;
 	bool converged = false;
 	int k0 = 0, looks = 0, eagerIters = 0;
@@ -691,8 +735,9 @@
 	while (lmBeforeTrial(r))
 	{
 		lmRestoreFlag = r.restoreInPass ? r.lm.state + 5 : nullptr;
-		try { schur(true); } catch (...) { lmRestoreFlag = nullptr; throw; }
-		lmRestoreFlag = nullptr;
+		foldChain = true;
+		try { schur(true); } catch (...) { lmRestoreFlag = nullptr; foldChain = false; throw; }
+		lmRestoreFlag = nullptr; foldChain = false;
 		coarseSideLater = true;
 		bool ok = false;
 		try { ok = solveReduced(); } catch (...) { coarseSideLater = false; throw; }
@@ -870,6 +915,7 @@
 				e = BatchEntry();
 				e.g = h->g; e.st = h->st; e.sys = h->sys;
 				batch_fill_linearize(h->g, h->st, h->d_state.data(), h->d_backup.data(), h->d_state.size(), e.t);
+				h->hrowFromSchur = false;
 				lmMax = std::max(lmMax, e.t.lmGrid); schurMax = std::max(schurMax, e.t.schurGrid);
 			}
 			upload(0, m);
diff --git a/cuda-bundle-adjustment_amd/csrc/ba_pcg.hip b/cuda-bundle-adjustment_amd/csrc/ba_pcg.hip
--- a/cuda-bundle-adjustment_amd/csrc/ba_pcg.hip
+++ b/cuda-bundle-adjustment_amd/csrc/ba_pcg.hip
@@ -4,10 +4,14 @@
 namespace cubahip
 {
 
+__device__ __forceinline__ int pcg_setup_pose_of(const DeviceGraph& g, int bid)
+{
+	return threadIdx.x < PCG_SETUP_POSES ? bid * PCG_SETUP_POSES + (int)threadIdx.x : g.Pf;
+}
+
 template <bool ROWCOPY>
-__device__ __forceinline__ void pcg_setup_body(const DeviceGraph& g, const DeviceStructure& st, const DeviceSystem& sys, Scalar lambda, int bid, int nb)
-{
-	const int i = threadIdx.x < PCG_SETUP_POSES ? bid * PCG_SETUP_POSES + (int)threadIdx.x : g.Pf;
+__device__ __forceinline__ void pcg_setup_body(const DeviceGraph& g, const DeviceStructure& st, const DeviceSystem& sys, Scalar lambda, int bid, int nb, int i)
+{
 	lambda = launch_lambda(sys, lambda);
 	Scalar rz = 0;
 	if (i < g.Pf)
@@ -72,7 +76,7 @@
 
 __global__ __launch_bounds__(256) void pcg_setup_kernel(DeviceGraph g, DeviceStructure st, DeviceSystem sys, Scalar lambda)
 {
-	pcg_setup_body<false>(g, st, sys, lambda, blockIdx.x, gridDim.x);
+	pcg_setup_body<false>(g, st, sys, lambda, blockIdx.x, gridDim.x, pcg_setup_pose_of(g, blockIdx.x));
 }
 
 void launch_pcg_setup(const DeviceGraph& g, const DeviceStructure& st, const DeviceSystem& sys, Scalar lambda, hipStream_t s)
@@ -140,7 +144,7 @@
 __global__ __launch_bounds__(256) void pcg_setup_expand_kernel(DeviceGraph g, DeviceStructure st, DeviceSystem sys, Scalar lambda, int nSetup, size_t total,
 	unsigned nExpand, const Scalar2* __restrict__ copySrc, Scalar2* __restrict__ copyDst, size_t copyPairs)
 {
-	if ((int)blockIdx.x < nSetup) pcg_setup_body<true>(g, st, sys, lambda, blockIdx.x, nSetup);
+	if ((int)blockIdx.x < nSetup) pcg_setup_body<true>(g, st, sys, lambda, blockIdx.x, nSetup, pcg_setup_pose_of(g, blockIdx.x));
 	else if (blockIdx.x < nSetup + nExpand) hsc_expand_body<true>(st, sys, total, blockIdx.x - nSetup);
 	else
 	{
@@ -154,7 +158,7 @@
 	const BatchEntry& e = tab[blockIdx.y];
 	const BatchTrial& t = e.t;
 	if (blockIdx.x >= t.setupGrid) return;
-	if ((int)blockIdx.x < t.nSetup) pcg_setup_body<true>(e.g, e.st, e.sys, Scalar(-1), blockIdx.x, t.nSetup);
+	if ((int)blockIdx.x < t.nSetup) pcg_setup_body<true>(e.g, e.st, e.sys, Scalar(-1), blockIdx.x, t.nSetup, pcg_setup_pose_of(e.g, blockIdx.x));
 	else if (blockIdx.x < t.nSetup + t.nExpand) hsc_expand_body<true>(e.st, e.sys, t.expandTotal, blockIdx.x - t.nSetup);
 	else
 	{
@@ -172,10 +176,10 @@
 }
 
 void launch_pcg_setup_expand(const DeviceGraph& g, const DeviceStructure& st, const DeviceSystem& sys, Scalar lambda, hipStream_t s,
-	const Scalar* copySrc, Scalar* copyDst, size_t copyCount)
+	const Scalar* copySrc, Scalar* copyDst, size_t copyCount, bool expand)
 {
 	if (g.Pf <= 0) return;
-	const size_t total = sys.upper ? 0 : (size_t)g.Pf * st.ell_m * 20 * 36;
+	const size_t total = sys.upper || !expand ? 0 : (size_t)g.Pf * st.ell_m * 20 * 36;
 	const int nSetup = (g.Pf + PCG_SETUP_POSES - 1) / PCG_SETUP_POSES;
 	const unsigned nExpand = (unsigned)((total + 255) / 256);
 	const size_t pairs = copySrc ? copyCount / 2 : 0;
@@ -837,6 +841,55 @@
 	hipLaunchKernelGGL((void (*)(DeviceGraph, DeviceSystem, int, int, int, Scalar, int))pcg2_kernel_for(sys), dim3(sys.nc), dim3(PCG2_T), lds, s, g, sys, k, kOut, maxIter, tol2, doUpdate);
 }
 
+template <int CL, int AC, int AC2, int W>
+__global__ __launch_bounds__(PCG2_T) void pcg2_setup_first_kernel(DeviceGraph g, DeviceStructure st, DeviceSystem sys, Scalar lambda, int maxIter, Scalar tol2,
+	const Scalar2* __restrict__ copySrc, Scalar2* __restrict__ copyDst, size_t copyPairs)
+{
+	if ((int)blockIdx.x >= sys.nc)
+	{
+		const size_t stride = (size_t)(gridDim.x - sys.nc) * PCG2_T;
+		for (size_t i = (size_t)(blockIdx.x - sys.nc) * PCG2_T + threadIdx.x; i < copyPairs; i += stride) copyDst[i] = copySrc[i];
+		return;
+	}
+	const int i0 = (int)blockIdx.x * sys.agg, i1 = min(g.Pf, i0 + sys.agg);
+	const int il = (int)(threadIdx.x >> 6) + 8 * (int)(threadIdx.x & 63);
+	pcg_setup_body<true>(g, st, sys, lambda, blockIdx.x, sys.nc, i0 + il < i1 ? i0 + il : g.Pf);
+	__syncthreads();
+	DeviceSystem s0 = sys;
+	s0.r = sys.bsc;
+	if (copySrc)
+	{
+		if (W == 4) s0.acinv32 = reinterpret_cast<float*>(const_cast<Scalar2*>(copySrc));
+		else s0.acinv = reinterpret_cast<Scalar*>(const_cast<Scalar2*>(copySrc));
+	}
+	pcg2_fused_body<CL, AC, AC2, W, false>(g, s0, 0, 0, maxIter, tol2, 0);
+}
+
+static void* pcg2_setup_first_kernel_for(const DeviceSystem& sys)
+{
+	const int Nc = 6 * sys.cl * sys.nc;
+	if (sys.acinv32 && sizeof(Scalar) == 8)
+	{
+		if (sys.cl == 2) return Nc <= 768 ? (void*)pcg2_setup_first_kernel<2, 3, 0, 4> : Nc <= 1536 ? (void*)pcg2_setup_first_kernel<2, 6, 0, 4> : (void*)pcg2_setup_first_kernel<2, 6, 3, 4>;
+		return Nc <= 768 ? (void*)pcg2_setup_first_kernel<1, 3, 0, 4> : Nc <= 1536 ? (void*)pcg2_setup_first_kernel<1, 6, 0, 4> : (void*)pcg2_setup_first_kernel<1, 6, 3, 4>;
+	}
+	const bool small = Nc <= 768;
+	if (sys.cl == 2) return small ? (void*)pcg2_setup_first_kernel<2, 6, 0, 2> : (void*)pcg2_setup_first_kernel<2, 12, 6, 2>;
+	return small ? (void*)pcg2_setup_first_kernel<1, 6, 0, 2> : (void*)pcg2_setup_first_kernel<1, 12, 6, 2>;
+}
+
+void launch_pcg2_setup_first(const DeviceGraph& g, const DeviceStructure& st, const DeviceSystem& sys, Scalar lambda, int maxIter, Scalar tol2, hipStream_t s,
+	const Scalar* copySrc, Scalar* copyDst, size_t copyCount)
+{
+	static_assert(PCG2_SETUP_FIRST_MAX_AGG == PCG2_T, "one pose of the aggregate per thread");
+	if (g.Pf <= 0 || sys.nc <= 0) return;
+	const size_t pairs = copySrc ? copyCount / 2 : 0;
+	const unsigned nCopy = pairs ? (unsigned)std::min<size_t>(512, (pairs + PCG2_T - 1) / PCG2_T) : 0;
+	hipLaunchKernelGGL((void (*)(DeviceGraph, DeviceStructure, DeviceSystem, Scalar, int, Scalar, const Scalar2*, Scalar2*, size_t))pcg2_setup_first_kernel_for(sys),
+		dim3(sys.nc + nCopy), dim3(PCG2_T), pcg2_lds_bytes(sys), s, g, st, sys, lambda, maxIter, tol2,
+		pairs ? reinterpret_cast<const Scalar2*>(copySrc) : nullptr, reinterpret_cast<Scalar2*>(copyDst), pairs);
+}
+
 __device__ __forceinline__ Scalar half_wave_sum(Scalar v, bool upperHalf)
 {
 	v += dpp_shift<0x111, 0xf>(v);
diff --git a/cuda-bundle-adjustment_amd/csrc/ba_setup.hip b/cuda-bundle-adjustment_amd/csrc/ba_setup.hip
--- a/cuda-bundle-adjustment_amd/csrc/ba_setup.hip
+++ b/cuda-bundle-adjustment_amd/csrc/ba_setup.hip
@@ -495,6 +495,7 @@
 	d_rowptr.upload(h_rowptr, stream); d_colind.upload(h_colind, stream);
 	d_adjPtr.upload(adjPtr, stream); d_adjBlk.upload(adjBlk, stream); d_adjCol.upload(adjCol, stream);
 	int ellM = 0, ellOver = 0;
+	std::vector<int2> hrowSlot;
 	{
 		int maxRow = 0;
 		for (int i = 0; i < Pf; i++) maxRow = std::max(maxRow, adjPtr[i + 1] - adjPtr[i]);
@@ -507,6 +508,8 @@
 			for (int e = 0; e < n; e++) ell[(size_t)i * M * 20 + e] = int2{ adjBlk[adjPtr[i] + e], adjCol[adjPtr[i] + e] };
 		}
 		d_ell.upload(ell, stream);
+		buildHrowSlotHost(ell, M, nblk, hrowSlot);
+		d_hrowSlot.upload(hrowSlot, stream); hrowSlotChecked = true;
 	}
 	d_blkrow.upload(blkRow, stream); d_odBlocks.upload(odBlocks, stream); d_prodPtr.upload(prodPtr, stream);
 	d_prodEa.upload(prodEa, stream); d_prodEb.upload(prodEb, stream); d_pePtr.upload(wholeGraph ? peAllPtr : pePtr, stream); d_peEdge.upload(wholeGraph ? peAll : peEdge, stream);
@@ -552,6 +555,34 @@
 	hostPatternValid = true;
 	const double dt = std::chrono::duration<double>(Clock::now() - t0).count();
 	prof[1] += 0.5 * dt; prof[5] += 0.5 * dt;
+}
+
+void cuba_hip_solver::buildHrowSlotHost(const std::vector<int2>& ell, int ellM, int nblk, std::vector<int2>& map) const
+{
+	map.assign((size_t)nblk, int2{ -1, -1 });
+	const size_t W = (size_t)20 * ellM;
+	if (ell.size() > (size_t)INT_MAX) { map.clear(); return; }
+	for (size_t x = 0; x < ell.size(); x++)
+	{
+		const int2 en = ell[x];
+		if (en.y < 0 || en.y == (int)(x / W)) continue;
+		const int blk = en.x & 0x7fffffff;
+		if (blk >= nblk) throw StateError{ "structure: an adjacency entry names a block that does not exist" };
+		(en.x < 0 ? map[blk].y : map[blk].x) = (int)x;
+	}
+	checkHrowSlot(map, ell.size());
+}
+
+void cuba_hip_solver::checkHrowSlot(const std::vector<int2>& map, size_t nSlots) const
+{
+	std::vector<char> seen(nSlots, 0);
+	for (const int2& m : map)
+		for (const int v : { m.x, m.y })
+		{
+			if (v == -1) continue;
+			if (v < 0 || (size_t)v >= nSlots || seen[v]) throw StateError{ "structure: the map of the row-ordered copy is inconsistent" };
+			seen[v] = 1;
+		}
 }
 
 cuba_hip_solver::CoarseCfg cuba_hip_solver::coarseConfig() const
@@ -718,7 +749,7 @@
 	sys.upper = agg > 0 && agg <= pcg_rows_max_aggregate() && (spmvUpper < 0 ? spmvRows == 4 : spmvUpper != 0) ? 1 : 0;
 	if (sys.upper)
 	{
-		d_tq.resize((size_t)6 * nblk); sys.tq = d_tq.data(); d_hrow.release(); sys.hrow = nullptr;
+		d_tq.resize((size_t)6 * nblk); sys.tq = d_tq.data(); d_hrow.release(); sys.hrow = nullptr; d_hrowSlot.release();
 		d_lowpos.resize((size_t)nblk); sys.lowpos = d_lowpos.data();
 		DeviceGraph gg; gg.Pf = Pf;
 		launch_build_lowpos(gg, st, d_lowpos.data(), stream);
@@ -1147,6 +1178,9 @@
 	const int ellM = std::min(3, (maxRow + 19) / 20), ellOver = maxRow > 20 * ellM;
 	d_ell.resize((size_t)Pf * ellM * 20);
 	topo::launch_ell(d_adjPtr.data(), d_adjBlk.data(), d_adjCol.data(), Pf, ellM, d_ell.data(), stream);
+	if (d_ell.size() <= (size_t)INT_MAX) { d_hrowSlot.resize((size_t)nblk); topo::launch_hrow_slot(d_ell.data(), Pf, ellM, nblk, d_hrowSlot.data(), stream); }
+	else d_hrowSlot.resize(0);
+	hrowSlotChecked = false;
 	if (!reorderActive && !reorderTried && tryReorder(nblk, hc[topo::CNT_FARBLOCKS]))
 	{
 		reorderTried = true;
diff --git a/cuda-bundle-adjustment_amd/csrc/ba_solver.hip b/cuda-bundle-adjustment_amd/csrc/ba_solver.hip
--- a/cuda-bundle-adjustment_amd/csrc/ba_solver.hip
+++ b/cuda-bundle-adjustment_amd/csrc/ba_solver.hip
@@ -148,6 +148,13 @@
 		else if (k == "spmv_upper") { s->spmvUpper = (int)value; s->haveStructure = false; s->dropPcgGraph(); }
 		else if (k == "pcg_graph") { s->useGraph = value != 0; s->dropPcgGraph(); }
 		else if (k == "profile") s->profile = value != 0;
+		else if (k == "fold_setup")
+		{
+			if (value != 0 && value != 1 && value != 2) throw ArgError{ "fold_setup: 0 = set-up, expand pass and first preconditioner application as three launches, 1 = folded (default), 2 = only the row-ordered copy stored by the Schur launch" };
+			s->foldSetup = (int)value;
+		}
+		else if (k == "fold_stage_calls") s->foldStageCalls = value != 0;
+		else if (k == "debug_solve_setup_only") s->debugSetupOnly = value != 0;
 		else throw ArgError{ "unknown option: " + k };
 	});
 }
@@ -391,6 +398,10 @@
 		else if (k == "value_bytes_uploaded") *value = s->cntValueBytes;
 		else if (k == "edge_sorts") *value = s->cntEdgeSorts;
 		else if (k == "late_decision_records") *value = s->cntLateRecords;
+		else if (k == "folded_schur_launches") *value = s->cntFoldRows;
+		else if (k == "folded_setup_launches") *value = s->cntFoldFirst;
+		else if (k == "schur_heavy_blocks") { s->need(); *value = s->st.nHeavy; }
+		else if (k == "schur_diagonal_product_blocks") { s->need(); *value = s->st.nDiagProd; }
 		else if (k == "covariance_ns") *value = (int64_t)(1e9 * s->covSeconds);
 		else if (k == "covariance_pairs_ns") *value = (int64_t)(1e9 * s->covPairsSeconds);
 		else if (k == "covariance_pairs_chunks") *value = s->covPairChunks;
@@ -444,9 +455,27 @@
 		case CUBA_HIP_ARRAY_XL: src = s->sys.xl; n = (size_t)3 * s->Lf; break;
 		case CUBA_HIP_ARRAY_LM_SYS: src = s->sys.lm_sys; n = (size_t)9 * s->Lf; break;
 		case CUBA_HIP_ARRAY_HSC: src = s->sys.hsc; n = (size_t)36 * s->st.nblk; break;
+		case CUBA_HIP_ARRAY_HROW: src = s->sys.hrow; n = src ? (size_t)36 * 20 * s->st.ell_m * s->Pf : 0; break;
+		case CUBA_HIP_ARRAY_MINV: src = s->sys.minv; n = (size_t)36 * s->Pf; break;
+		case CUBA_HIP_ARRAY_Z: src = s->sys.z; n = (size_t)6 * s->Pf; break;
+		case CUBA_HIP_ARRAY_R: src = s->sys.r; n = (size_t)6 * s->Pf; break;
+		case CUBA_HIP_ARRAY_RC: src = s->sys.rc; n = s->sys.agg > 0 ? (size_t)6 * s->sys.cl * s->sys.nc : 0; break;
+		case CUBA_HIP_ARRAY_RZ: src = s->sys.rz; n = (size_t)s->sys.nrz0; break;
+		case CUBA_HIP_ARRAY_HROW_SLOT: n = 2 * s->d_hrowSlot.size(); break;
 		default: throw ArgError{ "unknown array id" };
 		}
 		if (count) *count = n;
+		if (which == CUBA_HIP_ARRAY_HROW_SLOT)
+		{
+			if (out && n)
+			{
+				std::vector<int2> map(s->d_hrowSlot.size());
+				HIP_TRY(hipMemcpyAsync(map.data(), s->d_hrowSlot.data(), sizeof(int2) * map.size(), hipMemcpyDeviceToHost, s->stream));
+				s->sync();
+				for (size_t k = 0; k < map.size(); k++) { out[2 * k] = map[k].x; out[2 * k + 1] = map[k].y; }
+			}
+			return;
+		}
 		if (out && n)
 		{
 			if (which == CUBA_HIP_ARRAY_XL) src = s->landmarkRowsForCaller(src, s->Lf, 3);
diff --git a/cuda-bundle-adjustment_amd/csrc/ba_solver.hpp b/cuda-bundle-adjustment_amd/csrc/ba_solver.hpp
--- a/cuda-bundle-adjustment_amd/csrc/ba_solver.hpp
+++ b/cuda-bundle-adjustment_amd/csrc/ba_solver.hpp
@@ -2,6 +2,7 @@
 
 #include <algorithm>
 #include <chrono>
+#include <climits>
 #include <cmath>
 #include <cstdarg>
 #include <cstdio>
@@ -670,6 +671,18 @@
 	void enqueueCoarseSide(int first);
 	void enqueueInversionTail(hipStream_t side, bool firstInvCopy);
 	bool coarseSideLater = false;
+	int foldSetup = foldSetupByDefault();
+	static int foldSetupByDefault() { const char* e = std::getenv("CUBA_HIP_FOLD_SETUP"); return e && (e[0] == '0' || e[0] == '2') && !e[1] ? e[0] - '0' : 1; }
+	bool foldStageCalls = false;
+	bool foldChain = false;
+	bool hrowFromSchur = false;
+	bool debugSetupOnly = false;
+	DevBuf<int2> d_hrowSlot;
+	bool hrowSlotChecked = false;
+	int64_t cntFoldRows = 0, cntFoldFirst = 0;
+	void buildHrowSlotHost(const std::vector<int2>& ell, int ellM, int nblk, std::vector<int2>& map) const;
+	void checkHrowSlot(const std::vector<int2>& map, size_t nSlots) const;
+	bool foldUsable();
 	bool solveBrokeDown(SolveCtx& sc);
 	bool solveEnd(SolveCtx& sc);
 	bool solveReducedOnce();
diff --git a/cuda-bundle-adjustment_amd/csrc/ba_structure.hip b/cuda-bundle-adjustment_amd/csrc/ba_structure.hip
--- a/cuda-bundle-adjustment_amd/csrc/ba_structure.hip
+++ b/cuda-bundle-adjustment_amd/csrc/ba_structure.hip
@@ -307,6 +307,17 @@
 	const int i = (int)(x / W), e = (int)(x - (size_t)i * W);
 	const int a0 = adjPtr[i], n = adjPtr[i + 1] - a0;
 	ell[x] = e < n ? int2{ adjBlk[a0 + e], adjCol[a0 + e] } : int2{ 0, -1 };
+}
+
+__global__ __launch_bounds__(T) void hrow_slot_kernel(const int2* ell, int Pf, int M, int nblk, int2* map)
+{
+	const size_t x = (size_t)blockIdx.x * T + threadIdx.x;
+	const int W = 20 * M;
+	if (x >= (size_t)Pf * W) return;
+	const int2 en = ell[x];
+	const int blk = en.x & 0x7fffffff;
+	if (en.y < 0 || en.y == (int)(x / W) || blk >= nblk) return;
+	reinterpret_cast<int*>(map)[2 * (size_t)blk + (en.x < 0 ? 1 : 0)] = (int)x;
 }
 
 __global__ __launch_bounds__(T) void coarse_keys_kernel(const int* adjRow, const int* adjCol, int nAdj, int agg, int nc, uint32_t* keys, uint32_t* vals)
@@ -592,6 +603,13 @@
 	if (n > 0) hipLaunchKernelGGL(ell_kernel, grid_for(n), dim3(T), 0, s, adjPtr, adjBlk, adjCol, Pf, M, ell);
 }
 
+void launch_hrow_slot(const int2* ell, int Pf, int M, int nblk, int2* map, hipStream_t s)
+{
+	const size_t n = (size_t)Pf * 20 * M;
+	if (nblk > 0) (void)hipMemsetAsync(map, 0xff, sizeof(int2) * (size_t)nblk, s);
+	if (n > 0 && nblk > 0) hipLaunchKernelGGL(hrow_slot_kernel, grid_for(n), dim3(T), 0, s, ell, Pf, M, nblk, map);
+}
+
 void launch_coarse_keys(const int* adjRow, const int* adjCol, int nAdj, int agg, int nc, uint32_t* keys, uint32_t* vals, hipStream_t s)
 {
 	if (nAdj > 0) hipLaunchKernelGGL(coarse_keys_kernel, grid_for(nAdj), dim3(T), 0, s, adjRow, adjCol, nAdj, agg, nc, keys, vals);
diff --git a/cuda-bundle-adjustment_amd/csrc/ba_structure.hpp b/cuda-bundle-adjustment_amd/csrc/ba_structure.hpp
--- a/cuda-bundle-adjustment_amd/csrc/ba_structure.hpp
+++ b/cuda-bundle-adjustment_amd/csrc/ba_structure.hpp
@@ -48,6 +48,7 @@
 void launch_adj_fill(const int* rowptr, const int* colind, const int* blkrow, const int* lowerPtr, const uint64_t* tKeys, const uint32_t* tBlk, int nblk,
 	const int* adjPtr, int* adjBlk, int* adjCol, int* adjRow, hipStream_t s);
 void launch_ell(const int* adjPtr, const int* adjBlk, const int* adjCol, int Pf, int M, int2* ell, hipStream_t s);
+void launch_hrow_slot(const int2* ell, int Pf, int M, int nblk, int2* map, hipStream_t s);
 void launch_coarse_keys(const int* adjRow, const int* adjCol, int nAdj, int agg, int nc, uint32_t* keys, uint32_t* vals, hipStream_t s);
 void launch_heads_u32(const uint32_t* keys, int n, int* head, hipStream_t s);
 void launch_coarse_lists(const uint32_t* keys, const uint32_t* order, const int* cbOfEntry, const int* adjBlk, const int* adjRow, const int* adjCol,
diff --git a/include/cuba_hip.h b/include/cuba_hip.h
--- a/include/cuba_hip.h
+++ b/include/cuba_hip.h
@@ -33,7 +33,14 @@
 	CUBA_HIP_ARRAY_XL = 3,
 	CUBA_HIP_ARRAY_LM_SYS = 4,
 	CUBA_HIP_ARRAY_HSC = 5,
-	CUBA_HIP_ARRAY_STATE = 6
+	CUBA_HIP_ARRAY_STATE = 6,
+	CUBA_HIP_ARRAY_HROW = 7,
+	CUBA_HIP_ARRAY_MINV = 8,
+	CUBA_HIP_ARRAY_Z = 9,
+	CUBA_HIP_ARRAY_R = 10,
+	CUBA_HIP_ARRAY_RC = 11,
+	CUBA_HIP_ARRAY_RZ = 12,
+	CUBA_HIP_ARRAY_HROW_SLOT = 13
 };
 
 
```

Measured after the change: 821.2 million. 2.0% lower.
